# ndrwmlnk/critic-guided-segmentation-of-rewarding-objects-in-first-person-views

Measured on AMD Instinct MI355X. Metric: Hourglass+critic train images/sec, 64x64x3 batch=512, higher is better.
Workload: dtype f32

## Files before the change

critic-guided-segmentation-of-rewarding-objects-in-first-person-views_amd/_lib.py:

```python
import ctypes as C
import os

HERE = os.path.dirname(os.path.abspath(__file__))
LIB_PATH = os.environ.get("CGS_LIB_PATH") or os.path.join(HERE, "libcgs_hip.so")

OK, ERR_UNSUPPORTED, ERR_BADARG = 0, -1, -2
SRC_F32, SRC_U8, SRC_MIX = 0, 1, 2
ACT_NONE, ACT_RELU, ACT_LRELU, ACT_SIGMOID = 0, 1, 2, 3
H5_ENC1_FWD, H5_ENC1_BWD_DATA, H5_DEC0_FWD, H5_DEC0_BWD_SKIP, H5_DEC0_BWD_LOW = 1, 2, 3, 4, 5
H5_ENC1_BWD_DATA_POOLED = 6
H5_ENC2_FWD, H5_ENC2_BWD_DATA_POOLED, H5_DEC1_FWD, H5_DEC1_BWD_SKIP, H5_DEC1_BWD_LOW, H5_DEC1_FWD_F32B = 7, 8, 9, 10, 11, 12

vp = C.c_void_p
i32 = C.c_int32
i64 = C.c_int64
f32 = C.c_float


class Dropout(C.Structure):
    _fields_ = [("p", C.c_float), ("site", C.c_uint32), ("seed", C.c_uint64), ("step", C.c_void_p),
                ("base", C.c_uint32), ("reserved", C.c_uint32)]


class ConvDesc(C.Structure):
# ... 36 lines not shown
OBJ_TRACK_FIELDS, OBJ_TRACK_MAX_FRAMES = 8, 1 << 17
SALIENCY_SIDE, SALIENCY_MAX_T = 64, 1024
BOUNDARY_MAX_TOL, BOUNDARY_MAX_TOL_PX = 16, 128
FIT_SIDE, FIT_MAX_SIDE, FIT_RADIUS, FIT_MAP_F32, FIT_MAP_U8 = 64, 4096, 2, 0, 1
TEMPORAL_SIDE, TEMPORAL_MAX_RADIUS = 64, 8
OVERLAY_ONLY, OVERLAY_SIDE, OVERLAY_TRIPLE, OVERLAY_MAX_OUTLINE, OVERLAY_NONTEMPORAL = 1, 2, 3, 4, 1


class ReduceJob(C.Structure):
    _fields_ = [("slab", C.c_void_p), ("dst", C.c_void_p), ("nslab", i32), ("stride", i32), ("count", i32),
                ("accumulate", i32)]


SIGNATURES = {
    "cgs_conv3x3_fwd": (i32, [C.POINTER(ConvDesc), vp, vp, vp, vp, vp, vp, vp]),
    "cgs_conv3x3_bwd_data": (i32, [C.POINTER(ConvDesc), vp, vp, vp, vp, i32, vp, i32, vp, vp, vp]),
    "cgs_mask_infer_fwd": (i32, [i32, i32, vp, vp, vp, vp, vp, vp, vp, vp]),
    "cgs_mask_infer_fwd_packed": (i32, [i32, i32, vp, vp, vp, vp, vp, vp, vp, vp, vp]),
    "cgs_mask_infer_fwd_tile": (i32, [i32, i32, vp, vp, vp, vp, vp, vp, vp, vp]),
    "cgs_mask_infer_fwd_f16": (i32, [i32, i32, vp, vp, vp, vp, vp, vp, vp, vp]),
    "cgs_mask_infer_fwd_f16o": (i32, [i32, i32, vp, vp, vp, vp, vp, vp, vp, vp]),
    "cgs_f16_enc0_fwd": (i32, [i32, vp, vp, vp, vp, vp]),
    "cgs_f16_enc1_fwd": (i32, [i32, vp, vp, vp, vp, vp]),
    "cgs_f16_dec0_fwd": (i32, [i32, vp, vp, vp, vp, vp, vp]),
    "cgs_bf16_enc0_fwd": (i32, [i32, vp, i32, vp, vp, vp, vp, vp]),
    "cgs_bf16_mask0_fwd": (i32, [i32, vp, vp, vp, vp, vp, vp]),
    "cgs_bf16_mask2_fwd": (i32, [i32, vp, vp, vp, vp, vp]),
    "cgs_bf16_enc0_bwd_data": (i32, [i32, vp, vp, vp, vp]),
    "cgs_bf16_mask2_bwd_data": (i32, [i32, vp, vp, vp, vp, vp]),
    "cgs_bf16_enc0_bwd_data_pooled": (i32, [i32, vp, vp, vp, vp, vp, vp]),
    "cgs_bf16_enc0_bwd_mix": (i32, [i32, vp, vp, vp, vp, vp, vp, f32, f32, vp, vp]),
    "cgs_bf16_enc0_fwd_mix": (i32, [i32, vp, vp, vp, vp, vp, vp, vp, vp]),
    "cgs_bf16_hwgrad_pooled_mix": (i32, [i32, vp, vp, vp, vp, vp, vp, vp]),
    "cgs_bf16_mask0_bwd_data": (i32, [i32, vp, vp, vp, vp]),
    "cgs_bf16_h5conv": (i32, [i32, i32, vp, vp, vp, vp, vp, vp, vp]),
    "cgs_gen_enc0_fwd": (i32, [i32, i32, i32, vp, vp, vp, vp, vp, vp]),
    "cgs_gen_enc0_bwd_data": (i32, [i32, i32, vp, vp, vp, vp, vp]),
    "cgs_gen_enc0_bwd_weight_slabs": (i32, [i32, i32]),
    "cgs_gen_enc0_bwd_weight": (i32, [i32, i32, i32, vp, vp, vp, vp, vp]),
    "cgs_bn_rows": (i32, [i64, i32]),
    "cgs_bn_act_fwd": (i32, [i64, i32, vp, vp, vp, f32, i32, f32, i32, vp, vp, vp, vp, vp, f32, vp]),
    "cgs_bn_act_bwd": (i32, [i64, i32, vp, vp, vp, vp, i32, f32, i32, vp, vp, vp, vp, vp]),
    "cgs_bf16_hwgrad_slabs": (i32, [i32, i32, i32, i32, i32]),
    "cgs_bf16_hwgrad": (i32, [i32, i32, i32, i32, i32, i32, vp, vp, vp, vp, vp]),
    "cgs_bf16_hwgrad_pooled": (i32, [i32, i32, i32, i32, vp, vp, vp, vp, vp, vp]),
    "cgs_mask_train_fwd_partials": (i32, [i32]),
    "cgs_mask_train_fwd": (i32, [i32, i32, vp, vp, vp, vp, vp, vp, vp, vp, vp, vp]),
    "cgs_mask_train_fwd_packed": (i32, [i32, i32, vp, vp, vp, vp, vp, vp, vp, vp, vp, vp, vp]),
    "cgs_mask_head_bwd_slabs": (i32, [i32]),
    "cgs_mask_head_bwd": (i32, [i32, i32, vp, vp, vp, vp, vp, vp, vp, vp, vp, vp, vp]),
    "cgs_tail_enc_fwd": (i32, [i32, C.POINTER(TailEncWeights), vp, vp, vp, vp, vp, vp, vp, vp, vp, Dropout, Dropout, Dropout, vp]),
    "cgs_enc1_tail_fwd": (i32, [i32, C.POINTER(TailEncWeights), vp, vp, vp, vp, vp, vp, vp, vp, vp, vp, vp, vp, vp, Dropout, Dropout, Dropout, vp]),
    "cgs_critic_fwd_fused": (i32, [i32, C.POINTER(TailEncWeights), vp, i32] + [vp] * 16 + [Dropout, Dropout, Dropout, vp]),
    "cgs_tail_dec_fwd": (i32, [i32, C.POINTER(TailDecWeights), vp, vp, vp, vp, vp, vp, vp, vp]),
    "cgs_tail_enc_fwd_h16": (i32, [i32, C.POINTER(TailEncWeights), vp, vp, vp, vp, vp, vp, vp, vp, vp, vp]),
    "cgs_tail_dec_fwd_h16": (i32, [i32, C.POINTER(TailDecWeights), vp, vp, vp, vp, vp, vp, vp, vp]),
    "cgs_tail_infer_h16": (i32, [i32, C.POINTER(TailEncWeights), C.POINTER(TailDecWeights), vp, vp, vp, vp]),
    "cgs_f16_enc1_tail_infer": (i32, [i32, vp, vp, vp, C.POINTER(TailEncWeights), C.POINTER(TailDecWeights), vp, vp, vp]),
    "cgs_tail_dec_fwd_pack": (i32, [i32, C.POINTER(TailDecWeights), vp, vp, vp, vp, vp, vp, vp, vp, vp, vp]),
    "cgs_tail_enc_bwd_slabs": (i32, [i32]),
    "cgs_tail_enc_bwd": (i32, [i32, C.POINTER(TailEncWeights)] + [vp] * 10 + [f32, i32] + [vp] * 4 + [i32] + [vp] * 4 + [Dropout, Dropout, Dropout, vp]),
    "cgs_tail_enc_bwd_rider": (i32, [i32, C.POINTER(TailEncWeights)] + [vp] * 10 + [f32, i32] + [vp] * 4 + [i32] + [vp] * 4 + [Dropout, Dropout, Dropout, i32, vp, vp, vp, vp, i32, vp]),
    "cgs_tail_enc_bwd_enc1": (i32, [i32, C.POINTER(TailEncWeights)] + [vp] * 10 + [f32, i32] + [vp] * 4 + [i32] + [vp] * 4 + [Dropout, Dropout, Dropout, i32, vp, vp, vp, vp, i32, vp, vp, vp, i32, vp, vp, vp, i32, vp, vp, vp, vp]),
    "cgs_enc1_wgrad_rider_slabs": (i32, [i32]),
    "cgs_enc0_wgrad_u8_with_head_enc1": (i32, [i32, vp, vp, vp, vp, i32, vp, vp, vp, i32, i32, vp, vp, vp, i32, vp, vp, i32, vp, vp, vp, vp, i32, vp]),
    "cgs_enc0_bwd_mix_enc1": (i32, [i32, i32, vp, vp, vp, vp, vp, vp, vp, C.c_float, C.c_float, vp, vp, vp, vp, vp, vp, vp, vp]),
    "cgs_tail_head_wgrad_slabs": (i32, [i32]),
    "cgs_tail_head_wgrad": (i32, [i32, vp, vp, vp, i32, i32, vp, vp, vp, i32, vp, vp, vp]),
    "cgs_enc0_wgrad_u8_with_head": (i32, [i32, vp, vp, vp, vp, i32, vp, vp, vp, i32, i32, vp, vp, vp, i32, vp, vp, vp]),
    "cgs_reduce_adam": (i32, [vp, i32, i32, vp, vp, vp, vp, vp, f32, f32, f32, f32, vp, i32, vp, vp, vp, i32, f32, f32, f32, i32, i64, vp, vp]),
    "cgs_tail_dec_bwd_slabs": (i32, [i32]),
    "cgs_tail_dec_bwd": (i32, [i32, C.POINTER(TailDecWeights)] + [vp] * 14 + [vp]),
    "cgs_dec0_tail_dec_bwd": (i32, [i32, C.POINTER(TailDecWeights)] + [vp] * 17 + [vp]),
    "cgs_dec0_tail_dec_bwd_do3": (i32, [i32, C.POINTER(TailDecWeights)] + [vp] * 18 + [vp]),
    "cgs_dec3_wgrad_rider_slabs": (i32, [i32]),
    "cgs_enc0_wgrad_u8_with_head_riders": (i32, [i32, vp, vp, vp, vp, i32, vp, vp, vp, i32, i32, vp, vp, vp, i32, vp, vp, i32, vp, vp, vp, vp, i32, i32, vp, vp, vp, vp, vp]),
    "cgs_tail_dec_fwd_dec0": (i32, [i32, C.POINTER(TailDecWeights)] + [vp] * 13 + [vp]),
    "cgs_conv3x3_bwd_weight_slabs": (i32, [C.POINTER(ConvDesc)]),
    "cgs_conv3x3_bwd_weight": (i32, [C.POINTER(ConvDesc), vp, vp, vp, vp, vp, vp]),
    "cgs_conv3x3_bwd_both_slabs": (i32, [C.POINTER(ConvDesc)]),
    "cgs_conv3x3_bwd_both": (i32, [C.POINTER(ConvDesc), vp, vp, vp, vp, vp, vp, i32, vp, vp, vp, vp]),
    "cgs_reduce_slabs": (i32, [vp, i32, i32, vp, vp]),
    "cgs_head_fwd": (i32, [i32, vp, vp, vp, vp, vp, vp, vp, Dropout, Dropout, vp, vp, vp, vp, vp, vp, vp]),
    "cgs_enc0_bwd_mix_slabs": (i32, [i32]),
    "cgs_enc0_bwd_mix": (i32, [i32, i32, vp, vp, vp, vp, vp, vp, vp, C.c_float, C.c_float, vp, vp, vp, vp]),
    "cgs_head_bwd_slabs": (i32, [i32]),
    "cgs_head_bwd": (i32, [i32, vp, vp, vp, vp, vp, vp, vp, i32, vp, vp, vp, Dropout, Dropout, vp, vp, vp, vp, vp, vp]),
    "cgs_pointwise_fwd": (i32, [i32, i32, i32, vp, vp, vp, vp, vp]),
    "cgs_pointwise_bwd_slabs": (i32, [i32]),
    "cgs_pointwise_bwd": (i32, [i32, i32, i32, vp, vp, vp, vp, vp, vp]),
    "cgs_mix_fwd": (i32, [i32, i32, vp, vp, vp, i32, vp, vp, vp]),
    "cgs_mix_bwd": (i32, [i32, i32, vp, vp, vp, vp, i32, f32, f32, vp, vp]),
    "cgs_mix_bwd_weighted": (i32, [i32, i32, vp, vp, vp, vp, i32, f32, f32, vp, vp, vp]),
    "cgs_mix_fwd_partials": (i32, [i32, i32]),
    "cgs_phase2_losses": (i32, [i32, vp, vp, vp, i32, f32, f32, f32, i32, i64, vp, vp, vp]),
    "cgs_phase1_loss": (i32, [i32, vp, vp, i32, vp, vp, vp]),
    "cgs_adam_flat": (i32, [i64, vp, vp, vp, vp, vp, f32, f32, f32, f32, f32, vp]),
    "cgs_nchw_to_nhwc": (i32, [i32, i32, i32, vp, vp, vp]),
    "cgs_nhwc_to_nchw": (i32, [i32, i32, i32, vp, vp, vp]),
    "cgs_gen_conv_packed_floats": (i64, [i32, i32, i32]),
    "cgs_gen_conv_packed_floats_folded": (i64, [i32, i32, i32]),
    "cgs_gen_conv_packed_floats_up2": (i64, [i32, i32]),
    "cgs_gen_conv_pack_weights_up2": (i32, [i32, i32, i32, i32, vp, vp, vp]),
    "cgs_gen_conv3x3_bwd_data_up2": (i32, [i32, i32, i32, i32, vp, vp, vp, vp]),
    "cgs_gen_conv_pack_weights": (i32, [i32, i32, i32, i32, vp, vp, vp]),
    "cgs_gen_conv_pack_weights_window": (i32, [i32, i32, i32, i32, vp, vp, vp]),
    "cgs_gen_conv_pack_batch": (i32, [vp, i32, vp]),
    "cgs_gen_conv3x3_fwd": (i32, [i32, i32, i32, i32, i32, i32, i32, i32, f32, i32, vp, vp, vp, vp, vp, vp, vp]),
    "cgs_gen_conv3x3_fwd_folded": (i32, [i32, i32, i32, i32, i32, i32, i32, f32, vp, vp, vp, vp, vp, vp]),
    "cgs_gen_gemm": (i32, [i32, i32, i32, i32, f32, vp, vp, vp, vp, vp]),
    "cgs_gen_flip_weights": (i32, [i32, i32, vp, vp, vp]),
    "cgs_gen_conv3x3_bwd_data": (i32, [i32, i32, i32, i32, vp, vp, vp, vp, i32, vp, vp]),
    "cgs_gen_conv3x3_bwd_data_split": (i32, [i32, i32, i32, i32, i32, i32, vp, vp, vp, vp, vp]),
    "cgs_gen_conv3x3_bwd_weight_slabs": (i32, [i32, i32, i32, i32]),
    "cgs_gen_conv3x3_bwd_weight_folded_slabs": (i32, [i32, i32, i32, i32, i32]),
    "cgs_gen_conv3x3_bwd_weight_folded": (i32, [i32, i32, i32, i32, i32, i32, vp, vp, vp, vp, vp]),
    "cgs_gen_conv3x3_bwd_weight": (i32, [i32, i32, i32, i32, i32, i32, i32, vp, vp, vp, vp, vp, vp]),
    "cgs_gen_cat_split": (i32, [i32, i32, i32, i32, i32, vp, vp, vp, vp]),
    "cgs_gen_grad_fix": (i32, [i64, vp, vp, i32, f32, vp, i64, Dropout, vp]),
    "cgs_gen_dropout_fwd": (i32, [i64, vp, vp, Dropout, vp]),
    "cgs_gen_gemm_ex": (i32, [i32, i32, i32, vp, i64, i64, vp, i64, i64, vp, i32, f32, i32, vp, vp]),
    "cgs_gen_gemm_ex_splitk": (i32, [i32, i32, i32, vp, i64, i64, vp, i64, i64, i32, vp, vp]),
    "cgs_gen_u8_to_f32": (i32, [i64, vp, vp, vp]),
    "cgs_gen16_packed_weight_halves": (i64, [i32, i32, i32]),
    "cgs_gen16_pack_weights": (i32, [i32, i32, i32, vp, vp, vp]),
    "cgs_gen16_conv3x3_fwd": (i32, [i32, i32, i32, i32, i32, i32, i32, i32, f32, i32, i32, vp, vp, vp, vp, vp, vp]),
    "cgs_gen16_gemm": (i32, [i32, i32, i32, i32, f32, i32, i32, vp, vp, vp, vp, vp]),
    "cgs_genbf16_pack_weights": (i32, [i32, i32, i32, vp, vp, vp]),
    "cgs_genbf16_conv3x3_fwd": (i32, [i32, i32, i32, i32, i32, i32, i32, i32, f32, i32, i32, vp, vp, vp, vp, vp, vp]),
    "cgs_genbf16_gemm": (i32, [i32, i32, i32, i32, f32, i32, i32, vp, vp, vp, vp, vp]),
# ... 74 lines not shown
```

critic-guided-segmentation-of-rewarding-objects-in-first-person-views_amd/build.py:

```python
import os
import subprocess
import sys
from concurrent.futures import ThreadPoolExecutor

HERE = os.path.dirname(os.path.abspath(__file__))
REPO = os.path.dirname(HERE)
CSRC = os.path.join(HERE, "csrc")
LIB = os.path.join(HERE, "libcgs_hip.so")
SOURCES = ["conv_fwd.hip", "conv_wgrad.hip", "wgrad_dec0.hip", "conv_bwd_both.hip", "mconv.hip", "mask_head.hip", "mask_fwd.hip", "head.hip", "elementwise.hip", "tail.hip", "tail_infer.hip", "gen.hip", "gen4.hip", "gen_train.hip", "gen_f16.hip", "gen_bf16_train.hip", "hconv.hip", "hwgrad.hip", "bn.hip", "gen_enc0.hip", "crf.hip", "video.hip", "vis.hip", "sheet.hip", "metrics.hip", "objects.hip", "objects_match.hip", "objects_track.hip", "saliency.hip", "boundary.hip", "fit.hip", "temporal.hip", "overlay.hip"]
HEADERS = ["cgs_common.h", "head_wgrad.h", "conv_tile.h", "conv_body.h", "wgrad_body.h", "head_body.h", "tail_common.h", "tail4.h", "tail_h16.h", "gen_common.h", "gen4_common.h", "gen_wgrad_rows.h", "gen_wgrad_fold.h", "wgrad_dec0.h", "wgrad_sparse.h", os.path.join(REPO, "include", "cgs_hip.h")]
ARCH = "gfx950"
EXTRA_FLAGS = {"conv_fwd.hip": ["-fno-slp-vectorize"], "conv_bwd_both.hip": ["-fno-slp-vectorize"], "saliency.hip": ["-ffp-contract=off"]}


def _hipcc():
    for cand in (os.environ.get("HIPCC"), "/opt/rocm/bin/hipcc", "hipcc"):
        if cand and (os.path.isabs(cand) and os.path.exists(cand) or not os.path.isabs(cand)):
            return cand
    raise RuntimeError("hipcc not found")


def _stale():
    if not os.path.exists(LIB):
        return True
    t = os.path.getmtime(LIB)
    deps = [os.path.join(CSRC, s) for s in SOURCES] + [h if os.path.isabs(h) else os.path.join(CSRC, h) for h in HEADERS]
    return any(os.path.getmtime(d) > t for d in deps)


def build_library(force=False, verbose=True):
    if not force and not _stale():
        return LIB
    objdir = os.path.join(HERE, "build")
    os.makedirs(objdir, exist_ok=True)
    cc = _hipcc()
    flags = ["-O3", f"--offload-arch={ARCH}", "-std=c++17", "-fPIC", "-I", os.path.join(REPO, "include"), "-I", CSRC]

    def one(src):
        obj = os.path.join(objdir, src.replace(".hip", ".o"))
        extra = EXTRA_FLAGS.get(src, [])
        cmd = [cc] + flags + extra + ["-c", os.path.join(CSRC, src), "-o", obj]
        r = subprocess.run(cmd, capture_output=True, text=True)
        if r.returncode != 0:
            raise RuntimeError(f"hipcc failed for {src}:\n{r.stderr}")
        return obj

    with ThreadPoolExecutor(max_workers=6) as ex:
        objs = list(ex.map(one, SOURCES))
    r = subprocess.run([cc, "-shared", "-fPIC", f"--offload-arch={ARCH}", "-o", LIB] + objs, capture_output=True, text=True)
    if r.returncode != 0:
        raise RuntimeError(f"link failed:\n{r.stderr}")
    if verbose:
        print(f"built {LIB} ({os.path.getsize(LIB) // 1024} KiB) for {ARCH}", file=sys.stderr)
    return LIB


if __name__ == "__main__":
    build_library(force="--force" in sys.argv)
```

critic-guided-segmentation-of-rewarding-objects-in-first-person-views_amd/csrc/conv_body.h:

```cpp
#pragma once
#include "conv_tile.h"

#ifndef CGS_WHATIF_NO_POOL_EPI
#define CGS_WHATIF_NO_POOL_EPI 0
#endif
#ifndef CGS_POOL_EPI_MAX3
#define CGS_POOL_EPI_MAX3 2
#endif
#ifndef CGS_CONV_MFMA4
#define CGS_CONV_MFMA4 1
#endif

struct ConvParams {
    const void* src_a;
    const float* src_b;
    const uint32_t* amask_in;
    const float* w;
    const float* bias;
    float* out;
    float* out2;
    uint32_t* amask_out;
    const float* addend;
    const float* a_post;
    const float* w2;
// ... 521 lines not shown
    zero_halo_cols<G, PA>(ldsA, tid);
    auto pos = [&](int t, int& n0, int& row0) { const int b = bid0 + t; n0 = b / G::STRIPS; row0 = (b % G::STRIPS) * G::TH; };
    using RA = std::conditional_t<C::SRC == SRC_F32, FetchF32<G, PA>,
               std::conditional_t<C::SRC == SRC_U8C3, FetchU8<G>,
               std::conditional_t<C::SRC == SRC_MIXC3, FetchMix<G>,
               std::conditional_t<C::SRC == SRC_POOLEXP, FetchPool<G, PA, false>, FetchPool<G, PA, true>>>>>;
    RA ra;
    [[maybe_unused]] FetchBHalf<G, PB == 0 ? 1 : PB> rb;
    auto fetch = [&](int t) {
        int n0, row0;
        pos(t, n0, row0);
        if constexpr (C::SRC == SRC_F32) fetch_a_f32<G, PA>(ra, (const float4*)P.src_a, n0, row0, N, tid);
        else if constexpr (C::SRC == SRC_U8C3) fetch_a_u8c3<G>(ra, (const uint32_t*)P.src_a, n0, row0, N, tid);
        else if constexpr (C::SRC == SRC_MIXC3) fetch_a_mix<G>(ra, (const uint32_t*)P.mix_a, (const uint32_t*)P.mix_b, (const float4*)P.mix_z, P.mix_n_a, n0, row0, N, tid);
        else if constexpr (C::SRC == SRC_POOLEXP) fetch_poolexp<G, PA, false>(ra, (const float4*)P.src_a, P.amask_in, n0, 0, false, row0, N, tid);
        else fetch_poolexp<G, PA, true>(ra, (const float4*)P.src_a, P.amask_in, n0, P.mix_n_a, P.mix_inject != 0, row0, N, tid);
        if constexpr (PB > 0) fetch_b_half<G, PB>(rb, (const float4*)P.src_b, n0, row0, N, tid);
    };
    auto commit = [&](int t) {
        int n0, row0;
        pos(t, n0, row0);
        auto idx = [](int p, int img, int r, int x) { return ldsA_idx<G, PA>(p, img, r, x + 1); };
        if constexpr (C::SRC == SRC_F32) commit_a_f32<G, PA>(ra, ldsA, n0, row0, N, tid);
        else if constexpr (C::SRC == SRC_U8C3) commit_a_u8c3<G>(ra, ldsA, n0, row0, N, tid);
        else if constexpr (C::SRC == SRC_MIXC3) commit_a_mix<G>(ra, ldsA, P.mix_n_a, n0, row0, N, tid);
        else if constexpr (C::SRC == SRC_POOLEXP) commit_poolexp<G, PA, false>(ra, ldsA, n0, false, row0, N, tid, idx, L::DUMP);
        else commit_poolexp<G, PA, true>(ra, ldsA, n0, P.mix_inject != 0, row0, N, tid, idx, L::DUMP);
        if constexpr (PB > 0) commit_b_half<G, PB>(rb, ldsB, n0, row0, N, tid);
    };
    fetch(0);
#pragma unroll
    for (int t = 0; t < TPW; ++t) {
        commit(t);
        __syncthreads();
        if (t + 1 < TPW) fetch(t + 1);
        conv_compute<C, true>(P, bid0 + t, tid, smem, pool_lds);
        if (t + 1 < TPW) __syncthreads();
    }
}

template <class C>
__global__ void __launch_bounds__(C::THREADS * C::CW) conv3x3_pipe_kernel(ConvParams P) {
    extern __shared__ __attribute__((aligned(16))) float4 smem[];
    conv3x3_body_pipe<C>(P, blockIdx.x * tpw_of<C>::value, smem);
}

template <class C>
__global__ void __launch_bounds__(C::THREADS * C::CW) conv3x3_kernel(ConvParams P) {
    extern __shared__ __attribute__((aligned(16))) float4 smem[];
    conv3x3_body<C, false>(P, blockIdx.x, smem);
}

template <class C>
static size_t conv_lds_bytes() {
    using G = Geo<C::H, C::W, C::THREADS, C::CW>;
    constexpr int PA = (C::SRC == SRC_SCALAR) ? 1 : (C::CA + 3) / 4;
    constexpr int PB = C::CB / 4;
    size_t a = (C::SRC == SRC_SCALAR) ? (size_t)((G::IMGS * G::TRA * (G::W + 2) + 3) / 4) : (size_t)PA * G::IMGS * G::TRA * G::PWA;
    size_t b = PB == 0 ? 0 : (C::UPS == 2 ? (size_t)PB * G::IMGS * G::TRB * G::PWB : (size_t)PB * G::IMGS);
    size_t w = (size_t)(9 * C::WCI * C::WCO + 3) / 4;
    size_t dz = (C::SRC == SRC_DH) ? (size_t)((G::TRA + 2) * (G::W + 4) + 3) / 4 : 0;
    return (a + b + 1 + w + dz) * sizeof(float4);
}

#define CGS_FWD_CFG(NAME, HW, THR, SRC_, CA_, CB_, UPS_, CO_, EPI_, ACT_, OCB_, CW_)                   \
    struct NAME {                                                                                      \
        static constexpr int H = HW, W = HW, THREADS = THR, SRC = SRC_, CA = CA_, CB = CB_, UPS = UPS_; \
        static constexpr int WT = 0, WCI = CA_ + CB_, WCO = CO_, OC0 = 0, OC = CO_, OCB = OCB_, CW = CW_; \
        static constexpr int EPI = EPI_, ACT = ACT_, OUT_A = 0, POST_ACT = CGS_ACT_NONE;                \
        static constexpr bool DROP = (HW == 8 && CB_ == 0);   \
    };
#define CGS_DG_CFG(NAME, HW, THR, SRC_, DYC, LCI, LCO, UPS_, OC0_, OC_, OCB_, OUTA, PACT, CW_)         \
    struct NAME {                                                                                      \
        static constexpr int H = HW, W = HW, THREADS = THR, SRC = SRC_, CA = DYC, CB = 0, UPS = UPS_;   \
        static constexpr int WT = 1, WCI = LCI, WCO = LCO, OC0 = OC0_, OC = OC_, OCB = OCB_, CW = CW_;  \
        static constexpr int EPI = EPI_DGRAD, ACT = CGS_ACT_NONE, OUT_A = OUTA, POST_ACT = PACT;        \
        static constexpr bool DROP = (HW == 8 && SRC_ == SRC_POOLEXP);                                   \
    };

CGS_FWD_CFG(FEnc0U8, 64, 256, SRC_U8C3, 3, 0, 2, 8, EPI_POOL, CGS_ACT_RELU, 8, 1)
CGS_FWD_CFG(FEnc0F32, 64, 256, SRC_F32C3, 3, 0, 2, 8, EPI_POOL, CGS_ACT_RELU, 8, 1)
CGS_FWD_CFG(FEnc0Mix, 64, 256, SRC_MIXC3, 3, 0, 2, 8, EPI_POOL, CGS_ACT_RELU, 8, 1)
CGS_FWD_CFG(FEnc1, 32, 128, SRC_F32, 8, 0, 2, 8, EPI_POOL, CGS_ACT_RELU, 4, 2)
CGS_FWD_CFG(FEnc2, 16, 128, SRC_F32, 8, 0, 2, 8, EPI_POOL, CGS_ACT_RELU, 4, 2)
CGS_FWD_CFG(FEnc3, 8, 64, SRC_F32, 8, 0, 2, 16, EPI_POOL, CGS_ACT_RELU, 4, 4)
CGS_FWD_CFG(FDec3, 4, 64, SRC_F32, 16, 32, 4, 16, EPI_PLAIN, CGS_ACT_NONE, 4, 4)
CGS_FWD_CFG(FDec2, 8, 64, SRC_F32, 8, 16, 2, 8, EPI_PLAIN, CGS_ACT_NONE, 2, 4)
CGS_FWD_CFG(FDec1, 16, 64, SRC_F32, 8, 8, 2, 8, EPI_PLAIN, CGS_ACT_NONE, 4, 2)
CGS_FWD_CFG(FDec0, 32, 128, SRC_F32, 8, 8, 2, 8, EPI_PLAIN, CGS_ACT_NONE, 4, 2)
CGS_FWD_CFG(FMask0U8, 64, 128, SRC_U8C3, 3, 8, 2, 16, EPI_PLAIN, CGS_ACT_LRELU, 8, 2)
CGS_FWD_CFG(FMask0F32, 64, 128, SRC_F32C3, 3, 8, 2, 16, EPI_PLAIN, CGS_ACT_LRELU, 8, 2)
CGS_FWD_CFG(FMask2, 64, 256, SRC_F32, 16, 0, 2, 1, EPI_PLAIN, CGS_ACT_SIGMOID, 1, 1)

CGS_DG_CFG(DEnc0, 64, 256, SRC_POOLEXP, 8, 3, 8, 2, 0, 3, 3, 3, CGS_ACT_NONE, 1)
CGS_DG_CFG(DEnc1, 32, 128, SRC_POOLEXP, 8, 8, 8, 2, 0, 8, 4, 8, CGS_ACT_NONE, 2)
CGS_DG_CFG(DEnc2, 16, 128, SRC_POOLEXP, 8, 8, 8, 2, 0, 8, 4, 8, CGS_ACT_NONE, 2)
CGS_DG_CFG(DEnc3, 8, 64, SRC_POOLEXP, 16, 8, 16, 2, 0, 8, 4, 8, CGS_ACT_NONE, 2)
CGS_DG_CFG(DDec3, 4, 64, SRC_F32, 16, 48, 16, 4, 0, 48, 8, 16, CGS_ACT_NONE, 6)
CGS_DG_CFG(DDec2, 8, 64, SRC_F32, 8, 24, 8, 2, 0, 24, 8, 8, CGS_ACT_NONE, 3)
CGS_DG_CFG(DDec1, 16, 64, SRC_F32, 8, 16, 8, 2, 0, 16, 4, 8, CGS_ACT_NONE, 4)
CGS_DG_CFG(DDec0, 32, 128, SRC_F32, 8, 16, 8, 2, 0, 16, 8, 8, CGS_ACT_NONE, 2)
CGS_DG_CFG(DMask0, 64, 128, SRC_F32, 16, 11, 16, 2, 3, 8, 4, 3, CGS_ACT_NONE, 2)
CGS_DG_CFG(DMask2, 64, 128, SRC_SCALAR, 1, 16, 1, 2, 0, 16, 8, 16, CGS_ACT_LRELU, 2)
CGS_DG_CFG(DMaskHead, 64, 128, SRC_DH, 16, 11, 16, 2, 3, 8, 4, 3, CGS_ACT_NONE, 2)

#ifndef CGS_CONV_PIPE
#define CGS_CONV_PIPE 1
// ... 8 lines not shown
```

critic-guided-segmentation-of-rewarding-objects-in-first-person-views_amd/csrc/mask_fwd.hip:

```cpp
#include "conv_tile.h"

struct MaskFwdParams {
    const void* img; const float* o0;
    const float* w0; const float* b0; const float* w2; const float* b2;
    float* h; float* z; float* zpart;
    int n;
    unsigned long long* dbg;
    const float* w0_pack;
};

namespace {
using MG = Geo<64, 64, 256, 1>;
constexpr int kPSlots = 9;
constexpr int kWinPitch = 33;
unsigned long long* g_maskfwd_stamps = nullptr;
}

#define MF_STAMP(k) do { if (CGS_STAMP_PTR(P.dbg) && tid == 0) CGS_STAMP_PTR(P.dbg)[(size_t)blockIdx.x * 64 + (k)] = __builtin_amdgcn_s_memtime(); } while (0)
#ifdef CGS_DEBUG_STAMPS
extern "C" int dbg_maskfwd_stamps(unsigned long long* stamps) { g_maskfwd_stamps = stamps; return CGS_OK; }
#endif

template <int SRC>
__global__ void __launch_bounds__(256, SRC == SRC_U8C3 ? 2 : 1) mask_fwd_kernel(MaskFwdParams P) {
    if (CGS_KARG_PREFETCH) cgs_kernarg_prefetch<sizeof(MaskFwdParams)>();
    using G = MG;
    constexpr int A4 = (G::TRA * G::PWA + 1 + 3) / 4 * 4, B4 = 2 * G::TRB * G::PWB;
    static_assert(A4 + B4 <= 2048, "tiles fit the 32 KB staging area");
    __shared__ __attribute__((aligned(16))) float4 stage4[2048];
    float4* const ldsA = stage4;
    float4* const ldsB = stage4 + A4;
    __shared__ float win[kPSlots * 16 * kWinPitch];
    __shared__ float zred[8];
    const int tid = threadIdx.x, lane = tid & 63, wave = tid >> 6;
    const int n = blockIdx.x, N = P.n;
    const int lb = lane >> 2, li = lane & 3;
    MF_STAMP(0);

    constexpr int GW = G::W / 4, EA = G::TRA * GW, ITA = (EA + 255) / 256;
    constexpr int EB = G::TRB * G::PWB * 2, ITB = (EB + 255) / 256;
    uint32_t ra[ITA][(SRC == SRC_U8C3) ? 3 : 12];
    float4 rb[ITB];
    auto fetch = [&](int row0) {
#pragma unroll
        for (int it = 0; it < ITA; ++it) {
            int e = tid + 256 * it; e = e < EA ? e : EA - 1;
            const int g = e % GW, r = e / GW, y = row0 + r - 1;
            const bool in = y >= 0 && y < G::H;
            const int gi = in ? ((n * G::H + y) * G::W + g * 4) * 3 / 4 : 0;
            if constexpr (SRC == SRC_U8C3) {
                const uint32_t* src = (const uint32_t*)P.img;
                ra[it][0] = src[gi]; ra[it][1] = src[gi + 1]; ra[it][2] = src[gi + 2];
            } else {
                const float4* src = (const float4*)P.img;
#pragma unroll
                for (int k = 0; k < 3; ++k) {
                    const float4 v = src[gi + k];
                    ra[it][4 * k] = __float_as_uint(v.x); ra[it][4 * k + 1] = __float_as_uint(v.y);
                    ra[it][4 * k + 2] = __float_as_uint(v.z); ra[it][4 * k + 3] = __float_as_uint(v.w);
                }
            }
        }
        const int sy0 = row0 / 2;
#pragma unroll
        for (int it = 0; it < ITB; ++it) {
            int e = tid + 256 * it; e = e < EB ? e : EB - 1;
            const int p = e % 2, c = (e / 2) % G::PWB, r = e / (2 * G::PWB);
            const int sy = sy0 + r - 1, sx = c - 1;
            const bool in = sy >= 0 && sy < G::QH && sx >= 0 && sx < G::QW;
            rb[it] = ((const float4*)P.o0)[in ? ((n * G::QH + sy) * G::QW + sx) * 2 + p : 0];
        }
    };
    auto commit = [&](int row0) {
        const float sc = 1.f / 255.f;
#pragma unroll
        for (int it = 0; it < ITA; ++it) {
            int e = tid + 256 * it; e = e < EA ? e : EA - 1;
            const int g = e % GW, r = e / GW, y = row0 + r - 1;
            const bool in = y >= 0 && y < G::H;
            float4 p0, p1, p2, p3;
            if constexpr (SRC == SRC_U8C3) {
                const uint32_t d0 = ra[it][0], d1 = ra[it][1], d2 = ra[it][2];
                p0 = make_float4((d0 & 255) * sc, ((d0 >> 8) & 255) * sc, ((d0 >> 16) & 255) * sc, 0.f);
                p1 = make_float4((d0 >> 24) * sc, (d1 & 255) * sc, ((d1 >> 8) & 255) * sc, 0.f);
                p2 = make_float4(((d1 >> 16) & 255) * sc, (d1 >> 24) * sc, (d2 & 255) * sc, 0.f);
                p3 = make_float4(((d2 >> 8) & 255) * sc, ((d2 >> 16) & 255) * sc, (d2 >> 24) * sc, 0.f);
            } else {
                auto f = [&](int k) { return __uint_as_float(ra[it][k]); };
                p0 = make_float4(f(0), f(1), f(2), 0.f); p1 = make_float4(f(3), f(4), f(5), 0.f);
                p2 = make_float4(f(6), f(7), f(8), 0.f); p3 = make_float4(f(9), f(10), f(11), 0.f);
            }
            const int base = r * G::PWA;
            ldsA[base + G::pc(g * 4 + 1)] = in ? p0 : f4zero();
            ldsA[base + G::pc(g * 4 + 2)] = in ? p1 : f4zero();
            ldsA[base + G::pc(g * 4 + 3)] = in ? p2 : f4zero();
            ldsA[base + G::pc(g * 4 + 4)] = in ? p3 : f4zero();
        }
        zero_halo_cols<G, 1>(ldsA, tid);
        const int sy0 = row0 / 2;
#pragma unroll
        for (int it = 0; it < ITB; ++it) {
            int e = tid + 256 * it; e = e < EB ? e : EB - 1;
            const int p = e % 2, c = (e / 2) % G::PWB, r = e / (2 * G::PWB);
            const int sy = sy0 + r - 1, sx = c - 1;
            const bool in = sy >= 0 && sy < G::QH && sx >= 0 && sx < G::QW;
            ldsB[(p * G::TRB + r) * G::PWB + c] = in ? rb[it] : f4zero();
        }
    };
    fetch(0);
    float wimg[4][2];
    float wups[4][4][2];
    if (P.w0_pack) {
        const float* wp = P.w0_pack + lane;
#pragma unroll
        for (int g = 0; g < 4; ++g) {
#pragma unroll
            for (int k = 0; k < 2; ++k) wimg[g][k] = wp[(g * 2 + k) * 64];
#pragma unroll
            for (int pos = 0; pos < 4; ++pos)
#pragma unroll
                for (int ry = 0; ry < 2; ++ry) wups[pos][g][ry] = wp[(8 + (pos * 4 + g) * 2 + ry) * 64];
        }
    } else {
    float* wst = (float*)ldsA;
    for (int e = tid; e < 9 * 11 * 16; e += 256) wst[e] = P.w0[e];
    __syncthreads();
#pragma unroll
    for (int g = 0; g < 4; ++g) {
#pragma unroll
        for (int k = 0; k < 2; ++k) {
            const int step = 16 * k + lb;
            wimg[g][k] = step < 27 ? wst[((step / 3) * 11 + step % 3) * 16 + 4 * g + li] : 0.f;
        }
#pragma unroll
        for (int pos = 0; pos < 4; ++pos) {
            const int oy = pos >> 1, ox = pos & 1;
#pragma unroll
            for (int ry = 0; ry < 2; ++ry) {
                const int rx = lb >> 3, ci = lb & 7;
                const int ky0 = (oy == 0) ? (ry == 0 ? 0 : 1) : (ry == 0 ? 0 : 2), ky1 = (oy == 0) ? (ry == 0 ? 0 : 2) : (ry == 0 ? 1 : 2);
                const int kx0 = (ox == 0) ? (rx == 0 ? 0 : 1) : (rx == 0 ? 0 : 2), kx1 = (ox == 0) ? (rx == 0 ? 0 : 2) : (rx == 0 ? 1 : 2);
                auto wv = [&](int ky, int kx) { return wst[((ky * 3 + kx) * 11 + 3 + ci) * 16 + 4 * g + li]; };
                const float w00 = wv(ky0, kx0), w01 = wv(ky0, kx1), w10 = wv(ky1, kx0), w11 = wv(ky1, kx1);
                const bool my = ky1 > ky0, mx = kx1 > kx0;
                float s = w00;
                s += mx ? w01 : 0.f;
                s += my ? w10 : 0.f;
                s += (mx && my) ? w11 : 0.f;
                wups[pos][g][ry] = s;
            }
            __builtin_amdgcn_sched_barrier(0);
        }
    }
    }
    float w2r[3];
#pragma unroll
    for (int g = 0; g < 3; ++g) w2r[g] = (4 * g + li < 9) ? P.w2[(4 * g + li) * 16 + lb] : 0.f;
    const cgs_cptr b0c = cgs_to_const(P.b0);
    const float b2v = cgs_to_const(P.b2)[0];
    __syncthreads();

    MF_STAMP(1);
    const QuadPos q0 = quad_pos<G>(tid, 0);
    const int qy_l = q0.qy_l, qx = q0.qx;
    int pcx[4];
#pragma unroll
    for (int dx = 0; dx < 4; ++dx) pcx[dx] = G::pc(2 * qx + dx);
    float zs1 = 0.f, zs2 = 0.f;

#pragma unroll 1
    for (int strip = 0; strip < G::STRIPS; ++strip) {
        const int row0 = strip * G::TH;
        QuadPos q = q0;
        q.n = n; q.row0 = row0;
        MF_STAMP(2 + 10 * strip);
        commit(row0);
        __syncthreads();
        MF_STAMP(3 + 10 * strip);
        if (strip + 1 < G::STRIPS) fetch(row0 + G::TH);

        frag4 acc[4][4];
#pragma unroll
        for (int i = 0; i < 4; ++i)
#pragma unroll
            for (int g = 0; g < 4; ++g) acc[i][g] = frag4{b0c[4 * g], b0c[4 * g + 1], b0c[4 * g + 2], b0c[4 * g + 3]};
        {
            float4 pt[4][4];
            read_patch_a<G>(pt, ldsA, 0, q, pcx);
            mfma_plane<4, 3, 3, 0, 2>(acc, pt, wimg);
        }
        MF_STAMP(4 + 10 * strip);
        static_for<2>([&](auto PL) {
            constexpr int p = decltype(PL)::value;
            float4 s[3][3];
            const int base = (p * G::TRB + qy_l) * G::PWB + qx;
#pragma unroll
            for (int j = 0; j < 3; ++j)
#pragma unroll
                for (int i = 0; i < 3; ++i) s[j][i] = ldsB[base + j * G::PWB + i];
            static_for<16>([&](auto T) {
                constexpr int t = decltype(T)::value, ry = t >> 3, rx = (t >> 2) & 1, c = t & 3;
                constexpr int abid = rx * 8 + 4 * p + c;
#pragma unroll
                for (int pos = 0; pos < 4; ++pos) {
                    const float x = f4get(s[(pos >> 1) + ry][(pos & 1) + rx], c);
#pragma unroll
                    for (int g = 0; g < 4; ++g)
                        acc[pos][g] = __builtin_amdgcn_mfma_f32_4x4x1f32(wups[pos][g][ry], x, acc[pos][g], 4, abid, 0);
                }
            });
        });

        float hv[4][16];
        const int y0 = row0 + 2 * qy_l, x0 = 2 * qx;
#pragma unroll
        for (int pos = 0; pos < 4; ++pos)
#pragma unroll
            for (int c = 0; c < 16; ++c) { const float v = acc[pos][c >> 2][c & 3]; hv[pos][c] = fmaxf(v, 0.01f * v); }
        MF_STAMP(5 + 10 * strip);
        __syncthreads();
        MF_STAMP(6 + 10 * strip);
        if (P.h) {
            float4* sw4 = stage4 + wave * 512;
            const int pp = lane;
#pragma unroll
            for (int oy = 0; oy < 2; ++oy) {
#pragma unroll
                for (int j = 0; j < 8; ++j) {
                    const int pos = oy * 2 + (j >> 2), c0 = 4 * (j & 3);
                    sw4[pp * 8 + (j ^ (pp & 7))] = make_float4(hv[pos][c0], hv[pos][c0 + 1], hv[pos][c0 + 2], hv[pos][c0 + 3]);
                }
#pragma unroll
                for (int k = 0; k < 8; ++k) {
                    const int i = lane + 64 * k, rp = i >> 3, j = i & 7;
                    const float4 v = sw4[rp * 8 + (j ^ (rp & 7))];
                    const int y = row0 + 2 * (2 * wave + (k >> 2)) + oy;
                    ((float4*)P.h)[((size_t)(n * 64 + y) * 64) * 4 + (rp & 31) * 8 + j] = v;
                }
            }
        }
        MF_STAMP(7 + 10 * strip);
        frag4 c2[4][3];
#pragma unroll
        for (int i = 0; i < 4; ++i)
#pragma unroll
            for (int g = 0; g < 3; ++g) c2[i][g] = frag4{0.f, 0.f, 0.f, 0.f};
        static_for<16>([&](auto CH) {
            constexpr int ch = decltype(CH)::value;
#pragma unroll
            for (int pos = 0; pos < 4; ++pos)
#pragma unroll
                for (int g = 0; g < 3; ++g)
                    c2[pos][g] = __builtin_amdgcn_mfma_f32_4x4x1f32(w2r[g], hv[pos][ch], c2[pos][g], 4, ch, 0);
        });
        MF_STAMP(8 + 10 * strip);
        float sw[4][4];
#pragma unroll
        for (int wy = -1; wy <= 2; ++wy)
#pragma unroll
            for (int wx = -1; wx <= 2; ++wx) {
                float s = 0.f;
#pragma unroll
                for (int oy = 0; oy < 2; ++oy)
#pragma unroll
                    for (int ox = 0; ox < 2; ++ox) {
                        const int ky = oy - wy + 1, kx = ox - wx + 1;
                        if (ky >= 0 && ky <= 2 && kx >= 0 && kx <= 2) {
                            const int tap = ky * 3 + kx;
                            s += c2[oy * 2 + ox][tap >> 2][tap & 3];
                        }
                    }
                sw[wy + 1][wx + 1] = s;
            }
        float* wown = win + (qy_l + 1) * 16 * kWinPitch + qx;
#pragma unroll
        for (int e = 0; e < 16; ++e) wown[e * kWinPitch] = sw[e >> 2][e & 3];
        __syncthreads();
        MF_STAMP(9 + 10 * strip);
        const bool has_top = strip > 0 || qy_l > 0;
        const float* wtop = win + qy_l * 16 * kWinPitch + qx;
        float zz[3][2];
#pragma unroll
        for (int wy = -1; wy <= 1; ++wy) {
#pragma unroll
            for (int wx = 0; wx <= 1; ++wx) {
                const bool has_side = wx == 0 ? qx > 0 : qx < 31;
                const int side = has_side ? (wx == 0 ? -1 : 1) : 0;
                const int wxs = wx == 0 ? 2 : -1;
                float s = sw[wy + 1][wx + 1];
                const float a = wown[((wy + 1) * 4 + wxs + 1) * kWinPitch + side];
                s += has_side ? a : 0.f;
                if (wy <= 0) {
                    const float b = wtop[((wy + 3) * 4 + wx + 1) * kWinPitch];
                    const float c = wtop[((wy + 3) * 4 + wxs + 1) * kWinPitch + side];
                    s += has_top ? b : 0.f;
                    s += (has_top && has_side) ? c : 0.f;
                }
                zz[wy + 1][wx] = act_fwd<CGS_ACT_SIGMOID>(s + b2v);
            }
        }
        const bool last_row = strip == G::STRIPS - 1 && qy_l == 7;
#pragma unroll
        for (int wy = -1; wy <= 1; ++wy) {
            const int y = y0 + wy;
            if (wy == 1 ? last_row : y >= 0) {
                *(float2*)(P.z + (size_t)(n * 64 + y) * 64 + x0) = make_float2(zz[wy + 1][0], zz[wy + 1][1]);
                zs1 += fabsf(zz[wy + 1][0]) + fabsf(zz[wy + 1][1]);
                zs2 += zz[wy + 1][0] * zz[wy + 1][0] + zz[wy + 1][1] * zz[wy + 1][1];
            }
        }
        MF_STAMP(10 + 10 * strip);
        __syncthreads();
        MF_STAMP(11 + 10 * strip);
        if (qy_l == 7) {
#pragma unroll
            for (int e = 0; e < 16; ++e) win[e * kWinPitch + qx] = sw[e >> 2][e & 3];
        }
    }
    if (P.zpart) {
        zs1 = wave_sum(zs1); zs2 = wave_sum(zs2);
        if (lane == 0) { zred[2 * wave] = zs1; zred[2 * wave + 1] = zs2; }
        __syncthreads();
        if (tid == 0) {
            P.zpart[2 * n] = (zred[0] + zred[2]) + (zred[4] + zred[6]);
            P.zpart[2 * n + 1] = (zred[1] + zred[3]) + (zred[5] + zred[7]);
        }
    }
}

int mask_train_partials(int n) { return n; }
int mask_train_launch(int n, int img_kind, const void* img, const float* o0, const float* w0, const float* b0, const float* w2,
                      const float* b2, float* h, float* z, float* zpart, const float* w0_pack, hipStream_t st) {
    if (n <= 0) return CGS_OK;
    MaskFwdParams P{img, o0, w0, b0, w2, b2, h, z, zpart, n, g_maskfwd_stamps, w0_pack};
    if (img_kind == CGS_SRC_U8) hipLaunchKernelGGL(mask_fwd_kernel<SRC_U8C3>, dim3(n), dim3(256), 0, st, P);
    else hipLaunchKernelGGL(mask_fwd_kernel<SRC_F32C3>, dim3(n), dim3(256), 0, st, P);
    CGS_HIP_CHECK_LAUNCH();
    return CGS_OK;
}
```

critic-guided-segmentation-of-rewarding-objects-in-first-person-views_amd/csrc/tail.hip:

```cpp
#include "tail4.h"
#include "tail_h16.h"
#include "head_wgrad.h"
#include "wgrad_dec0.h"
#include "conv_body.h"
#include "wgrad_sparse.h"

namespace {

using T16x8 = Tile<16, 16, 8>;
using T8x8 = Tile<8, 8, 8>;
using T8x16 = Tile<8, 8, 16>;
using T16x16 = Tile<16, 16, 16>;
using T8x24 = Tile<8, 8, 24>;
using T4x48 = Tile<4, 4, 48>;
using T4x16 = Tile<4, 4, 20>;

__device__ __forceinline__ float4 nib_select4(const float4& v, uint32_t nib16, uint32_t pos) {
    float4 r;
    r.x = ((nib16 & 15u) == pos) ? v.x : 0.f;
    r.y = (((nib16 >> 4) & 15u) == pos) ? v.y : 0.f;
    r.z = (((nib16 >> 8) & 15u) == pos) ? v.z : 0.f;
    r.w = (((nib16 >> 12) & 15u) == pos) ? v.w : 0.f;
    return r;
}

__device__ __forceinline__ float drop1(const DropCtx& dc, uint32_t i) {
    return dc.on ? f4get(drop_mult4(dc, i >> 2), i & 3) : 1.f;
}

int tail_blocks(int n, int cap) { return n < cap ? n : cap; }
int tail_fwd_cap() { return 1024; }
#ifndef CGS_TAIL_DEC_FWD_CAP
#define CGS_TAIL_DEC_FWD_CAP 768
#endif
int tail_dec_fwd_cap() { return CGS_TAIL_DEC_FWD_CAP; }
int tail_bwd_cap() { return 512; }
#ifndef CGS_TAIL_ENC_BWD_CAP
#define CGS_TAIL_ENC_BWD_CAP 768
#endif
int tail_enc_bwd_cap() { return CGS_TAIL_ENC_BWD_CAP; }

unsigned long long* g_tail_stamps = nullptr;

}

#ifdef CGS_DEBUG_STAMPS
extern "C" int dbg_tail_stamps(unsigned long long* stamps) { g_tail_stamps = stamps; return CGS_OK; }
#endif
#define TAIL_STAMP(k)                                                                                     \
    do {                                                                                                  \
        if (CGS_STAMP_PTR(P.dbg) && tid == 0 && img == (int)blockIdx.x) CGS_STAMP_PTR(P.dbg)[(size_t)blockIdx.x * 16 + (k)] = __builtin_amdgcn_s_memtime(); \
    } while (0)

#ifndef CGS_TAIL_STAGGER
#define CGS_TAIL_STAGGER 0
#endif
#ifndef CGS_STAGGER_ENC_FWD
#define CGS_STAGGER_ENC_FWD CGS_TAIL_STAGGER
#endif
#ifndef CGS_STAGGER_DEC_FWD
#define CGS_STAGGER_DEC_FWD CGS_TAIL_STAGGER
#endif
#ifndef CGS_STAGGER_DEC_BWD
#define CGS_STAGGER_DEC_BWD CGS_TAIL_STAGGER
#endif
struct TailEncFwdParams {
    cgs_tail_enc_weights w;
    const float* e1;
    float* e2; uint32_t* am2; float* e3; uint32_t* am3; float* e4; float* h1; float* pred; float* o4;
    cgs_dropout drop_e2, drop_e3, drop_h1;
    int n;
    int nblocks;
    unsigned long long* dbg;
};

using X1P = TileP<16, 16, 8, 8, 148>;
using X2P = TileP<8, 8, 8, 8, 84>;

template <bool FUSED, int ENC0 = 0, bool H16 = false>
__global__ void __launch_bounds__(256) __attribute__((amdgpu_waves_per_eu(H16 ? 3 : 4, H16 ? 3 : 4))) tail_enc_fwd_kernel(TailEncFwdParams P, ConvParams PC, ConvParams PC0) {
    static_assert(!H16 || (!FUSED && ENC0 == 0), "fp16 operands: the stand-alone inference form");
    extern __shared__ __attribute__((aligned(16))) float4 conv_smem[];
    __shared__ __attribute__((aligned(16))) float x1[X1P::FLOATS];
    __shared__ __attribute__((aligned(16))) float x2[X2P::FLOATS];
    __shared__ __attribute__((aligned(16))) float xs[256];
    __shared__ __attribute__((aligned(16))) float red[8][32];
    __shared__ float es[32], hs[32];
    if (CGS_KARG_PREFETCH) cgs_kernarg_prefetch<sizeof(TailEncFwdParams) + 2 * sizeof(ConvParams)>();
    const int tid = threadIdx.x, lane = tid & 63, wave = tid >> 6;
    if (CGS_STAMP_PTR(P.dbg) && tid == 0) CGS_STAMP_PTR(P.dbg)[(size_t)blockIdx.x * 16] = __builtin_amdgcn_s_memtime();
    const int o = tid & 31, kg = tid >> 5;
    int img = blockIdx.x;
    float4 pe[2] = {f4zero(), f4zero()};
    if constexpr (!FUSED) {
        if (img < P.n) { pe[0] = ((const float4*)P.e1)[(size_t)img * 512 + tid]; pe[1] = ((const float4*)P.e1)[(size_t)img * 512 + tid + 256]; }
    }
#if CGS_DROPCTX3
    DropCtx d2, d3, dh;
    drop_ctx3(P.drop_e2, P.drop_e3, P.drop_h1, P.w.b6, d2, d3, dh);
#else
    const DropCtx d2 = drop_ctx(P.drop_e2, P.w.b6), d3 = drop_ctx(P.drop_e3, P.w.b6), dh = drop_ctx(P.drop_h1, P.w.b6);
#endif

    tilep_zero<X1P>(x1, tid);
    tilep_zero<X2P>(x2, tid);
    if constexpr (FUSED) {
        cgs_stagger<8, CGS_STAGGER_ENC_FWD>();
        if constexpr (ENC0 == 1) { conv3x3_body_pipe<FEnc0U8P>(PC0, 4 * (int)blockIdx.x, conv_smem); __syncthreads(); }
        if constexpr (ENC0 == 2) { conv3x3_body_pipe<FEnc0MixP>(PC0, 4 * (int)blockIdx.x, conv_smem); __syncthreads(); }
        conv3x3_body_pipe<FEnc1P>(PC, 2 * (int)blockIdx.x, conv_smem, PoolLds{x1, X1P::PITCH, X1P::PS});
    }
    if (CGS_STAMP_PTR(P.dbg) && tid == 0) CGS_STAMP_PTR(P.dbg)[(size_t)blockIdx.x * 16 + 12] = __builtin_amdgcn_s_memtime();
    [[maybe_unused]] float wr6[H16 ? 1 : 2][5], wr10[1][5];
    [[maybe_unused]] th4_t w6h[5], w10h[5];
    [[maybe_unused]] int off6[5], off10[5];
    if constexpr (H16) {
        const int l15w = lane & 15;
        h16_fill_w<8, 5, 1>(w6h, lane, 0, l15w < 8, [&](int tap, int c) { return P.w.w6[(tap * 8 + c) * 8 + (l15w & 7)]; });
        h16_fill_w<8, 5, 1>(w10h, lane, 0, true, [&](int tap, int c) { return P.w.w10[(tap * 8 + c) * 16 + l15w]; });
        h16_fill_off<X1P, 8, 5, 1>(off6, lane, 0);
        h16_fill_off<X2P, 8, 5, 1>(off10, lane, 0);
    } else {
        fill_wreg<2, 5, 72>(wr6, lane, [&](int step, int co) { return P.w.w6[step * 8 + co]; });
        fill_wreg<1, 5, 72>(wr10, lane, [&](int step, int co) { return P.w.w10[step * 16 + 4 * wave + co]; });
    }
    if (CGS_STAMP_PTR(P.dbg) && tid == 0) CGS_STAMP_PTR(P.dbg)[(size_t)blockIdx.x * 16 + 13] = __builtin_amdgcn_s_memtime();
    float w1r[4], wpr[4];
#pragma unroll
    for (int j = 0; j < 4; ++j) {
        w1r[j] = P.w.wl1[(kg * 4 + j) * 32 + o];
        wpr[j] = P.o4 ? P.w.wpw[(kg * 4 + j) * 32 + o] : 0.f;
    }
    const cgs_cptr b6c = cgs_to_const(P.w.b6), b10c = cgs_to_const(P.w.b10);
    const float b14 = P.w.b14[o], bl1 = P.w.bl1[o], wl2 = P.w.wl2[o], bl2 = P.w.bl2[0], bpw = P.o4 ? P.w.bpw[o] : 0.f;
    const PxPos pa = px16(wave, lane), pb = px8(lane);
    if (CGS_STAMP_PTR(P.dbg) && tid == 0) CGS_STAMP_PTR(P.dbg)[(size_t)blockIdx.x * 16 + 14] = __builtin_amdgcn_s_memtime();
    __syncthreads();

    for (; img < P.n; img += P.nblocks) {
        TAIL_STAMP(1);
        if constexpr (!FUSED) {
#pragma unroll
// ... 152 lines not shown
                for (int m = 16; m >= 1; m >>= 1) t += __shfl_xor(t, m, 64);
                if (o == 0) P.pred[img] = 1.f / (1.f + expf(-(t + bl2)));
            }
        }
        __syncthreads();
        TAIL_STAMP(11);
    }
    if (CGS_STAMP_PTR(P.dbg) && tid == 0) CGS_STAMP_PTR(P.dbg)[(size_t)blockIdx.x * 16 + 15] = __builtin_amdgcn_s_memtime();
}

extern "C" int cgs_tail_enc_fwd(int32_t n, const cgs_tail_enc_weights* w, const float* e1, float* e2, uint32_t* am2, float* e3,
                                uint32_t* am3, float* e4, float* h1, float* pred, float* o4, cgs_dropout drop_e2,
                                cgs_dropout drop_e3, cgs_dropout drop_h1, cgs_stream_t stream) {
    if (n < 0 || !w || !e1 || !e2 || !am2 || !e3 || !am3 || !e4 || !h1 || !pred) return CGS_ERR_BADARG;
    if (!w->w6 || !w->b6 || !w->w10 || !w->b10 || !w->w14 || !w->b14 || !w->wl1 || !w->bl1 || !w->wl2 || !w->bl2) return CGS_ERR_BADARG;
    if (o4 && (!w->wpw || !w->bpw)) return CGS_ERR_BADARG;
    if (n == 0) return CGS_OK;
    TailEncFwdParams P{*w, e1, e2, am2, e3, am3, e4, h1, pred, o4, drop_e2, drop_e3, drop_h1, n, tail_blocks(n, tail_fwd_cap()), g_tail_stamps ? g_tail_stamps + 0 * 2048 * 16 : nullptr};
    const int blocks = P.nblocks;
    hipLaunchKernelGGL((tail_enc_fwd_kernel<false, 0>), dim3(blocks), dim3(256), 0, (hipStream_t)stream, P, ConvParams{}, ConvParams{});
    CGS_HIP_CHECK_LAUNCH();
    return CGS_OK;
}

extern "C" int cgs_tail_enc_fwd_h16(int32_t n, const cgs_tail_enc_weights* w, const float* e1, float* e2, uint32_t* am2, float* e3,
                                    uint32_t* am3, float* e4, float* h1, float* pred, float* o4, cgs_stream_t stream) {
    if (n < 0 || !w || !e1 || !e2 || !am2 || !e3 || !am3 || !e4 || !h1 || !pred) return CGS_ERR_BADARG;
    if (!w->w6 || !w->b6 || !w->w10 || !w->b10 || !w->w14 || !w->b14 || !w->wl1 || !w->bl1 || !w->wl2 || !w->bl2) return CGS_ERR_BADARG;
    if (o4 && (!w->wpw || !w->bpw)) return CGS_ERR_BADARG;
    if (n == 0) return CGS_OK;
    const cgs_dropout nd{};
    TailEncFwdParams P{*w, e1, e2, am2, e3, am3, e4, h1, pred, o4, nd, nd, nd, n, tail_blocks(n, 768), nullptr};
    hipLaunchKernelGGL((tail_enc_fwd_kernel<false, 0, true>), dim3(P.nblocks), dim3(256), 0, (hipStream_t)stream, P, ConvParams{}, ConvParams{});
    CGS_HIP_CHECK_LAUNCH();
    return CGS_OK;
}

extern "C" int cgs_enc1_tail_fwd(int32_t n, const cgs_tail_enc_weights* w, const float* e0, const float* w3, const float* b3, float* e1,
                                 uint32_t* am1, float* e2, uint32_t* am2, float* e3, uint32_t* am3, float* e4, float* h1, float* pred, float* o4,
                                 cgs_dropout drop_e2, cgs_dropout drop_e3, cgs_dropout drop_h1, cgs_stream_t stream) {
    if (n < 0 || !w || !e0 || !w3 || !b3 || !e1 || !am1 || !e2 || !am2 || !e3 || !am3 || !e4 || !h1 || !pred) return CGS_ERR_BADARG;
    if (!w->w6 || !w->b6 || !w->w10 || !w->b10 || !w->w14 || !w->b14 || !w->wl1 || !w->bl1 || !w->wl2 || !w->bl2) return CGS_ERR_BADARG;
    if (o4 && (!w->wpw || !w->bpw)) return CGS_ERR_BADARG;
    if (n == 0) return CGS_OK;
    TailEncFwdParams P{*w, e1, e2, am2, e3, am3, e4, h1, pred, o4, drop_e2, drop_e3, drop_h1, n, n, g_tail_stamps ? g_tail_stamps + 0 * 2048 * 16 : nullptr};
    ConvParams PC{};
    PC.src_a = e0; PC.w = w3; PC.bias = b3; PC.out = e1; PC.amask_out = am1; PC.n = n;
    const size_t lds = conv_lds_bytes<FEnc1P>();
    hipLaunchKernelGGL((tail_enc_fwd_kernel<true, 0>), dim3(n), dim3(256), lds, (hipStream_t)stream, P, PC, ConvParams{});
    CGS_HIP_CHECK_LAUNCH();
    return CGS_OK;
}

extern "C" int cgs_critic_fwd_fused(int32_t n, const cgs_tail_enc_weights* w, const void* x, int32_t x_is_mix, const float* w0, const float* b0,
                                    float* e0, uint32_t* am0, const float* w3, const float* b3, float* e1, uint32_t* am1, float* e2, uint32_t* am2,
                                    float* e3, uint32_t* am3, float* e4, float* h1, float* pred, float* o4, cgs_dropout drop_e2,
                                    cgs_dropout drop_e3, cgs_dropout drop_h1, cgs_stream_t stream) {
    if (n < 0 || !w || !x || !w0 || !b0 || !e0 || !am0 || !w3 || !b3 || !e1 || !am1 || !e2 || !am2 || !e3 || !am3 || !e4 || !h1 || !pred) return CGS_ERR_BADARG;
    if (!w->w6 || !w->b6 || !w->w10 || !w->b10 || !w->w14 || !w->b14 || !w->wl1 || !w->bl1 || !w->wl2 || !w->bl2) return CGS_ERR_BADARG;
    if (o4 && (!w->wpw || !w->bpw)) return CGS_ERR_BADARG;
    if (n == 0) return CGS_OK;
    TailEncFwdParams P{*w, e1, e2, am2, e3, am3, e4, h1, pred, o4, drop_e2, drop_e3, drop_h1, n, n, g_tail_stamps ? g_tail_stamps + 0 * 2048 * 16 : nullptr};
    ConvParams PC{}, PC0{};
    PC.src_a = e0; PC.w = w3; PC.bias = b3; PC.out = e1; PC.amask_out = am1; PC.n = n;
    PC0.w = w0; PC0.bias = b0; PC0.out = e0; PC0.amask_out = am0; PC0.n = n;
    size_t lds = conv_lds_bytes<FEnc1P>();
    if (x_is_mix) {
        const cgs_mix_src* m = (const cgs_mix_src*)x;
        if (!m->a || !m->b || !m->z || m->n_a <= 0 || n > 2 * m->n_a) return CGS_ERR_BADARG;
        PC0.mix_a = m->a; PC0.mix_b = m->b; PC0.mix_z = m->z; PC0.mix_n_a = m->n_a;
        if (conv_lds_bytes<FEnc0MixP>() > lds) lds = conv_lds_bytes<FEnc0MixP>();
        hipLaunchKernelGGL((tail_enc_fwd_kernel<true, 2>), dim3(n), dim3(256), lds, (hipStream_t)stream, P, PC, PC0);
    } else {
        PC0.src_a = x;
        if (conv_lds_bytes<FEnc0U8P>() > lds) lds = conv_lds_bytes<FEnc0U8P>();
        hipLaunchKernelGGL((tail_enc_fwd_kernel<true, 1>), dim3(n), dim3(256), lds, (hipStream_t)stream, P, PC, PC0);
    }
    CGS_HIP_CHECK_LAUNCH();
    return CGS_OK;
}

struct TailDecFwdParams {
    cgs_tail_dec_weights w;
    const float* e1; const float* e2; const float* e3; const float* o4;
    float* o3; float* o2; float* o1;
    int n;
    int nblocks;
    unsigned long long* dbg;
    const float* m0_w; float* m0_pack;
};

__device__ __forceinline__ void mask0_pack_weights(const float* __restrict__ w0, float* __restrict__ pack, int lane) {
    const int lb = lane >> 2, li = lane & 3;
#pragma unroll
    for (int g = 0; g < 4; ++g) {
#pragma unroll
        for (int k = 0; k < 2; ++k) {
            const int step = 16 * k + lb;
            pack[(g * 2 + k) * 64 + lane] = step < 27 ? w0[((step / 3) * 11 + step % 3) * 16 + 4 * g + li] : 0.f;
        }
#pragma unroll
        for (int pos = 0; pos < 4; ++pos) {
            const int oy = pos >> 1, ox = pos & 1;
#pragma unroll
            for (int ry = 0; ry < 2; ++ry) {
                const int rx = lb >> 3, ci = lb & 7;
                const int ky0 = (oy == 0) ? (ry == 0 ? 0 : 1) : (ry == 0 ? 0 : 2), ky1 = (oy == 0) ? (ry == 0 ? 0 : 2) : (ry == 0 ? 1 : 2);
                const int kx0 = (ox == 0) ? (rx == 0 ? 0 : 1) : (rx == 0 ? 0 : 2), kx1 = (ox == 0) ? (rx == 0 ? 0 : 2) : (rx == 0 ? 1 : 2);
                auto wv = [&](int ky, int kx) { return w0[((ky * 3 + kx) * 11 + 3 + ci) * 16 + 4 * g + li]; };
                const float w00 = wv(ky0, kx0), w01 = wv(ky0, kx1), w10 = wv(ky1, kx0), w11 = wv(ky1, kx1);
                const bool my = ky1 > ky0, mx = kx1 > kx0;
                float sum = w00;
                sum += mx ? w01 : 0.f;
                sum += my ? w10 : 0.f;
                sum += (mx && my) ? w11 : 0.f;
                pack[(8 + (pos * 4 + g) * 2 + ry) * 64 + lane] = sum;
            }
        }
    }
}

using T1F = TileP<16, 16, 16, 16, 292>;

template <bool FUSED, bool H16 = false>
__global__ void __launch_bounds__(256) __attribute__((amdgpu_waves_per_eu(3, 3))) tail_dec_fwd_kernel(TailDecFwdParams P, ConvParams PC) {
    static_assert(!H16 || !FUSED, "fp16 operands: the stand-alone inference form");
    if (CGS_KARG_PREFETCH) cgs_kernarg_prefetch<sizeof(TailDecFwdParams) + sizeof(ConvParams)>();
    extern __shared__ __attribute__((aligned(16))) float4 dec_conv_smem[];
    __shared__ __attribute__((aligned(16))) float t1[T1F::FLOATS];
    __shared__ __attribute__((aligned(16))) float t2[T8x24::FLOATS];
    __shared__ __attribute__((aligned(16))) float t3[T4x48::FLOATS];
    __shared__ __attribute__((aligned(16))) float w2s[14 * 64 * 2];
    static_assert(14 * 64 * 2 >= 216 * 8, "either form fits");
    __shared__ float part[4][16][16];
    const int tid = threadIdx.x, lane = tid & 63, wave = tid >> 6;
    if ((int)blockIdx.x == P.nblocks) {
        if (wave == 0) mask0_pack_weights(P.m0_w, P.m0_pack, lane);
        return;
    }
    if constexpr (FUSED) cgs_stagger<8, CGS_STAGGER_DEC_FWD>();
    if (CGS_STAMP_PTR(P.dbg) && tid == 0) CGS_STAMP_PTR(P.dbg)[(size_t)blockIdx.x * 16] = __builtin_amdgcn_s_memtime();
    const int l15 = lane & 15, kq = lane >> 4;
    int img = blockIdx.x;
    float4 pe1a = f4zero(), pe1b = f4zero(), pe2 = f4zero(), pe3 = f4zero(), po4 = f4zero();
#define DEC_FWD_FETCH(im)                                                                                         \
    do {                                                                                                          \
        pe1a = ((const float4*)P.e1)[(size_t)(im) * 512 + tid]; pe1b = ((const float4*)P.e1)[(size_t)(im) * 512 + tid + 256]; \
        pe2 = ((const float4*)P.e2)[(size_t)(im) * 128 + (tid & 127)];                                            \
        pe3 = ((const float4*)P.e3)[(size_t)(im) * 64 + (tid & 63)];                                              \
        po4 = ((const float4*)P.o4)[(size_t)(im) * 8 + (tid & 7)];                                                \
    } while (0)
    if (img < P.n) DEC_FWD_FETCH(img);

    const float4 w2a = ((const float4*)P.w.w2)[tid], w2b = ((const float4*)P.w.w2)[tid + 256 < 216 * 8 / 4 ? tid + 256 : 0];
    [[maybe_unused]] float wr1[2][H16 ? 1 : 9];
    [[maybe_unused]] th4_t w3h[7], w1h[9];
    [[maybe_unused]] int off2[14];
    [[maybe_unused]] th4_t w2t[H16 ? 4 : 1];
    if constexpr (H16) {
        h16_fill_w<48, 7, 4>(w3h, lane, wave, true, [&](int tap, int c) { return P.w.w3[(tap * 48 + c) * 16 + l15]; });
        h16_fill_w<16, 9, 1>(w1h, lane, 0, l15 < 8, [&](int tap, int c) { return P.w.w1[(tap * 16 + c) * 8 + (l15 & 7)]; });
#pragma unroll
        for (int r = 0; r < 4; ++r) {
            const int e = tid + 256 * r, i = e >> 6, ln = e & 63;
            w2t[r] = h16_w1<24>(i, ln >> 4, (ln & 15) < 8, [&](int tap, int c) { return P.w.w2[(tap * 24 + c) * 8 + (ln & 7)]; });
        }
        h16_fill_off<T8x24, 24, 14, 1>(off2, lane, 0);
    } else {
        fill_wreg<2, 9, 144>(wr1, lane, [&](int step, int co) { return P.w.w1[step * 8 + co]; });
    }
    const float b2 = P.w.b2[l15 & 7];
    [[maybe_unused]] const float b1v = P.w.b1[l15 & 7];
    __builtin_amdgcn_sched_barrier(0);
    tilep_zero<T1F>(t1, tid);
    tile_zero<T8x24>(t2, tid);
    tile_zero<T4x48>(t3, tid);
    if constexpr (H16) {
#pragma unroll
        for (int r = 0; r < 4; ++r)
            if (tid + 256 * r < 14 * 64) ((th4_t*)w2s)[tid + 256 * r] = w2t[r];
    } else {
        ((float4*)w2s)[tid] = w2a;
        if (tid + 256 < 216 * 8 / 4) ((float4*)w2s)[tid + 256] = w2b;
    }
    const PxPos pa = px16(wave, lane);
    const cgs_cptr b1c = cgs_to_const(P.w.b1);
    __syncthreads();

    for (; img < P.n; img += P.nblocks) {
        TAIL_STAMP(1);
        int lz = 0;
        asm volatile("" : "+v"(lz));
        const int lane_i = lane + lz;
// ... 53 lines not shown
        auto epi2 = [&](int q, const frag4 (&acc)[1]) {
            if (l15 < 8) {
                const int qy = q >> 2, qx = q & 3;
#pragma unroll
                for (int j = 0; j < 4; ++j) {
                    const int y = 2 * qy + (j >> 1), x = 2 * qx + (j & 1);
                    const float v = acc[0][j] + b2;
                    P.o2[((size_t)img * 64 + y * 8 + x) * 8 + l15] = v;
#pragma unroll
                    for (int d = 0; d < 4; ++d) t1[T1F::at(2 * y + (d >> 1), 2 * x + (d & 1)) + 8 + l15] = v;
                }
            }
        };
        if constexpr (H16) {
            int y, x;
            h16_tile_px<8>(wave, l15, y, x);
            const frag4 acc[1] = {h16_conv_f<14>(t2 + T8x24::at(y - 1, x - 1), [&](int n) { return off2[n]; },
                                               [&](int n) { return ((const th4_t*)w2s)[n * 64 + lane_i]; }, frag4{0.f, 0.f, 0.f, 0.f})};
            epi2(4 * wave + kq, acc);
        } else {
            conv_tiles<T8x24, 0, 24, 1>(t2, [&](int tap, int c, int) { return w2s[(tap * 24 + c) * 8 + (l15 & 7)]; }, epi2, wave, lane_i);
        }
        __syncthreads();
        TAIL_STAMP(5);
        if constexpr (H16) {
#pragma unroll 1
            for (int u = 0; u < 4; ++u) {
                const int t = wave + 4 * u;
                int y, x;
                h16_tile_px<16>(t, l15, y, x);
                const frag4 acc = h16_conv_f<9>(t1 + T1F::at(y - 1, x - 1) + 4 * kq, [&](int n) { return h16_off<T1F, 16>(n, 0); },
                                                 [&](int n) { return w1h[n]; }, frag4{b1v, b1v, b1v, b1v});
                if (l15 < 8) {
                    const int q = 4 * t + kq, qy = q >> 3, qx = q & 7;
#pragma unroll
                    for (int j = 0; j < 4; ++j)
                        P.o1[((size_t)img * 256 + (2 * qy + (j >> 1)) * 16 + 2 * qx + (j & 1)) * 8 + l15] = acc[j];
                }
            }
        } else {
            frag4 a[2] = {frag4{b1c[0], b1c[1], b1c[2], b1c[3]}, frag4{b1c[4], b1c[5], b1c[6], b1c[7]}};
            conv_px<T1F, 0, 16, 16, 0, 2, 9, false, true>(a, t1, pa.y, pa.x, wr1);
            float4* dst = (float4*)(P.o1 + ((size_t)img * 256 + pa.y * 16 + pa.x) * 8);
            dst[0] = make_float4(a[0][0], a[0][1], a[0][2], a[0][3]);
            dst[1] = make_float4(a[1][0], a[1][1], a[1][2], a[1][3]);
        }
        __syncthreads();
        TAIL_STAMP(6);
    }
    if constexpr (FUSED) {
        conv3x3_body_pipe<FDec0P>(PC, 2 * (int)blockIdx.x, dec_conv_smem);
    }
    if (CGS_STAMP_PTR(P.dbg) && tid == 0) CGS_STAMP_PTR(P.dbg)[(size_t)blockIdx.x * 16 + 15] = __builtin_amdgcn_s_memtime();
}

extern "C" int cgs_tail_dec_fwd_pack(int32_t n, const cgs_tail_dec_weights* w, const float* e1, const float* e2, const float* e3,
                                     const float* o4, float* o3, float* o2, float* o1, const float* w_m0, float* m0_pack,
                                     cgs_stream_t stream) {
    if (n < 0 || !w || !e1 || !e2 || !e3 || !o4 || !o3 || !o2 || !o1 || (m0_pack && !w_m0)) return CGS_ERR_BADARG;
    if (!w->w3 || !w->b3 || !w->w2 || !w->b2 || !w->w1 || !w->b1) return CGS_ERR_BADARG;
    if (n == 0) return CGS_OK;
    TailDecFwdParams P{*w, e1, e2, e3, o4, o3, o2, o1, n, tail_blocks(n, tail_dec_fwd_cap()), g_tail_stamps ? g_tail_stamps + 1 * 2048 * 16 : nullptr,
                       w_m0, m0_pack};
    const int blocks = tail_blocks(n, tail_dec_fwd_cap());
    hipLaunchKernelGGL(tail_dec_fwd_kernel<false>, dim3(blocks + (m0_pack ? 1 : 0)), dim3(256), 0, (hipStream_t)stream, P, ConvParams{});
    CGS_HIP_CHECK_LAUNCH();
    return CGS_OK;
}

extern "C" int cgs_tail_dec_fwd_dec0(int32_t n, const cgs_tail_dec_weights* w, const float* e0, const float* e1, const float* e2, const float* e3,
                                     const float* o4, float* o3, float* o2, float* o1, const float* w0, const float* b0, float* o0,
                                     const float* w_m0, float* m0_pack, cgs_stream_t stream) {
    if (n < 0 || !w || !e0 || !e1 || !e2 || !e3 || !o4 || !o3 || !o2 || !o1 || !w0 || !b0 || !o0 || (m0_pack && !w_m0)) return CGS_ERR_BADARG;
    if (!w->w3 || !w->b3 || !w->w2 || !w->b2 || !w->w1 || !w->b1) return CGS_ERR_BADARG;
    if (n == 0) return CGS_OK;
    if (n > tail_fwd_cap()) return CGS_ERR_UNSUPPORTED;
    TailDecFwdParams P{*w, e1, e2, e3, o4, o3, o2, o1, n, n, g_tail_stamps ? g_tail_stamps + 1 * 2048 * 16 : nullptr, w_m0, m0_pack};
    ConvParams PC{};
    PC.src_a = e0; PC.src_b = o1; PC.w = w0; PC.bias = b0; PC.out = o0; PC.n = n;
    const size_t lds = conv_lds_bytes<FDec0P>();
    static hipError_t attr = hipFuncSetAttribute(reinterpret_cast<const void*>(&tail_dec_fwd_kernel<true>),
                                                 hipFuncAttributeMaxDynamicSharedMemorySize, (int)(conv_lds_bytes<FDec0P>()));
    if (attr != hipSuccess) return (int)attr;
    hipLaunchKernelGGL(tail_dec_fwd_kernel<true>, dim3(n + (m0_pack ? 1 : 0)), dim3(256), lds, (hipStream_t)stream, P, PC);
    CGS_HIP_CHECK_LAUNCH();
    return CGS_OK;
}

extern "C" int cgs_tail_dec_fwd_h16(int32_t n, const cgs_tail_dec_weights* w, const float* e1, const float* e2, const float* e3,
                                    const float* o4, float* o3, float* o2, float* o1, cgs_stream_t stream) {
    if (n < 0 || !w || !e1 || !e2 || !e3 || !o4 || !o3 || !o2 || !o1) return CGS_ERR_BADARG;
    if (!w->w3 || !w->b3 || !w->w2 || !w->b2 || !w->w1 || !w->b1) return CGS_ERR_BADARG;
    if (n == 0) return CGS_OK;
    const int blocks = tail_blocks(n, tail_dec_fwd_cap());
    TailDecFwdParams P{*w, e1, e2, e3, o4, o3, o2, o1, n, blocks, nullptr, nullptr, nullptr};
    hipLaunchKernelGGL((tail_dec_fwd_kernel<false, true>), dim3(blocks), dim3(256), 0, (hipStream_t)stream, P, ConvParams{});
    CGS_HIP_CHECK_LAUNCH();
    return CGS_OK;
}

extern "C" int cgs_tail_dec_fwd(int32_t n, const cgs_tail_dec_weights* w, const float* e1, const float* e2, const float* e3,
                                const float* o4, float* o3, float* o2, float* o1, cgs_stream_t stream) {
    return cgs_tail_dec_fwd_pack(n, w, e1, e2, e3, o4, o3, o2, o1, nullptr, nullptr, stream);
}

static constexpr int kTailSlab10 = 1168, kTailSlab6 = 584;
using DY2P = TileP<16, 16, 8, 8, 148>;
using DY3P = TileP<8, 8, 16, 16, 164>;
static constexpr int kTailEncBwdTileFloats = T16x8::FLOATS + T8x8::FLOATS + DY2P::FLOATS + DY3P::FLOATS;
static constexpr int kTailEncBwdOwnFloats = ((kTailEncBwdTileFloats + 3) & ~3) + 72 * 8 + 72 * 16 + 256 + 512 + 512 + 2048 + 64 + 32;
static constexpr int kTailEncBwdLdsFloats = kTailEncBwdOwnFloats > kWD0LdsFloats ? kTailEncBwdOwnFloats : kWD0LdsFloats;

struct TailEncBwdParams {
    cgs_tail_enc_weights w;
    const float* e1; const float* e2; const uint32_t* am2; const float* e3; const uint32_t* am3;
    const float* e4; const float* h1; const float* pred; const float* dpred;
    const float* target; float loss_scale; int bce;
    const float* dE1; const float* dE2; const float* dE3; const float* d_o4; int n_add;
    float* de1;
    float* hvec; float* slab10; float* slab6;
    cgs_dropout drop_e2, drop_e3, drop_h1;
    int n;
    int nblocks;
    unsigned long long* dbg;
    WDec0Params rider;
};

#ifndef CGS_ENC1_STAGGER
#define CGS_ENC1_STAGGER 64
#endif
#ifndef CGS_DROPCTX_SPLIT
#define CGS_DROPCTX_SPLIT 0
#endif
#ifndef CGS_ENC1_WGRAD_STAGES
#define CGS_ENC1_WGRAD_STAGES 1
#endif
template <int MODE>
// ... 609 lines not shown
```

critic-guided-segmentation-of-rewarding-objects-in-first-person-views_amd/engine.py:

```python
import os
import ctypes as C
from typing import Dict, Optional

import torch

from . import _lib
from . import hourglass as hg
from . import parallel
from .spec import ENC_LAYERS, critic_layout, masker_layout

_P = hg._p
_S = hg._stream


def _align4(x):
    return (x + 3) // 4 * 4


GATHER_ONE_LAUNCH = os.environ.get("CGS_GATHER_ONE_LAUNCH", "1") != "0"
PHASE1_FUSED_TAIL = os.environ.get("CGS_PHASE1_FUSED_TAIL", "1") != "0"
F16_TAILS = os.environ.get("CGS_F16_TAILS", "fused")


class HourglassEngine:
# ... 108 lines not shown
        return {k: t[a:b] for k, t in self.cbuf.items()}

    def _slab_views(self, tag: str, n_first: int, n_second: int):
        lib = _lib.load()
        out1, out2 = {}, {}
        nd = _lib.Dropout(0.0, 0, 0, None, 0, 0)
        tail = hg.TAIL_BWD
        specs = [] if tail else [("slab_head", lambda n, first: lib.cgs_head_bwd_slabs(n), hg.HEAD_SLAB)]
        for i, (key, hw, ca, cb, co, ups, act, pool, site) in enumerate(ENC_LAYERS):
            def f(n, first, i=i, hw=hw, ca=ca, cb=cb, co=co, ups=ups, act=act, pool=pool):
                d = hg.conv_desc(n, hw, ca, cb, co, False, ups, act, pool, nd)
                in_tail1 = hg.enc1_tail_bwd_fused(n) and hg.ENC1_WGRAD_IN_TAIL and 1 in hg.BOTH_ENC
                if tail and (i >= 2 or (i == 1 and in_tail1) or (i == 0 and in_tail1 and tag == "p2" and hg.enc0_in_tail(first, not first, None))):
                    return lib.cgs_tail_enc_bwd_slabs(n)
                if i in hg.BOTH_ENC and (i > 0 or first):
                    return lib.cgs_conv3x3_bwd_both_slabs(C.byref(d))
                return lib.cgs_conv3x3_bwd_weight_slabs(C.byref(d))
            specs.append((f"slab_enc{i}", f, 9 * ca * co + co))
        for name, fn, cnt in specs:
            a, b = (fn(n_first, True) if n_first else 0), (fn(n_second, False) if n_second else 0)
            big = torch.zeros((a + b, cnt), device=self.dev)
            self._ws.setdefault("slabs_" + tag, []).append(big)
            out1[name], out2[name] = big[:a], big[a:]
        return out1, out2

    def _opt_range(self):
        return (0, self.total) if self.live else (self.off_m, self.total - self.off_m)

    def _adam(self, tag="p2"):
        if self.fused_tail and not self.dp and tag == "p2":
            return
        lo, cnt = self._opt_range()
        _lib.call("cgs_adam_flat", cnt, C.c_void_p(self.flat.data_ptr() + 4 * lo), C.c_void_p(self.grad.data_ptr() + 4 * lo),
                  C.c_void_p(self.m.data_ptr() + 4 * lo), C.c_void_p(self.v.data_ptr() + 4 * lo), _P(self.step_t),
                  self.lr, self.b1, self.b2, self.eps, 1.0 / self.world, _S())

    def _allreduce(self):
        if self.dp:
            lo, cnt = self._opt_range()
            parallel.allreduce_sum_(self.grad[lo:lo + cnt], self.pg)

    def _phase2_fwd_bwd(self):
        n = self.n
        nmix = 2 * n if self.inject else n
        drop = self.drop
        A = self.ab[n:]
        B = self.ab[:n]
        if getattr(self, "_o4_full", None) is None:
            self._o4_full = torch.empty((2 * n, 32), device=self.dev, dtype=torch.float32)
            self.mbuf["o4"] = self._o4_full[n:]
        fm_ptr = self.fm.data_ptr()
        pw = (C.c_void_p(fm_ptr + 4 * self.lm.off("dec_model.4.weight")), C.c_void_p(fm_ptr + 4 * self.lm.off("dec_model.4.bias")),
              self._o4_full)
        hg.critic_forward(self.fc, self.lc, self.ab, 2 * n, drop.shifted(0), out=self._cview(0, 2 * n),
                          pw=None if self.separate else pw)
        sa = self._cview(n, 2 * n)
        if self.separate:
            pws = (pw[0], pw[1], self.mbuf["o4"])
            hg.critic_forward(self.fs, self.lc, A, n, drop.shifted(4 * n), out=self.sbuf, pw=pws)
            embeds = [self.sbuf[f"e{i}"] for i in range(5)]
        else:
            embeds = [sa[f"e{i}"] for i in range(5)]
        hg.masker_forward(self.fm, self.lm, A, embeds, n, out=self.mbuf, o4_done=True,
                          zpart=self.zsum if hg.ENC0_MIX_FUSED else None)
        if hg.ENC0_MIX_FUSED:
            mixsrc = hg.MixInput(A, B, self.mbuf["Z"])
            hg.critic_forward(self.fc, self.lc, mixsrc, nmix, drop.shifted(2 * n), out=self._cview(2 * n, 2 * n + nmix))
        else:
            mixsrc = self.mixed[:nmix]
            _lib.call("cgs_mix_fwd", n, 4096, _P(A), _P(B), _P(self.mbuf["Z"]), int(self.inject), _P(self.mixed), _P(self.zsum), _S())
            hg.critic_forward(self.fc, self.lc, mixsrc, nmix, drop.shifted(2 * n), out=self._cview(2 * n, 2 * n + nmix))
        flags = (1 if self.live else 0) | (2 if self.inject else 0) | (4 if self.bce else 0) | (0 if self.staticnorm else 8)
        ft = self.fused_tail
        if not ft:
            _lib.call("cgs_phase2_losses", n, _P(self.cbuf["pred"]), _P(self.y), _P(self.zsum), self.nzpart, self.lfak, self.L1, self.L2,
                      flags, n * 4096, _P(self.losses), _P(self.dpred), _S())
        loss_mix = (self.cbuf["pred"][:nmix], 1.0 / n, False) if ft else None
        loss_a = (self.y, self.lfak / n, self.bce) if ft else None
        plan = self._plans.get("p2")
        first = plan is None
        if first:
            plan = hg.SlabPlan()
            self._sl_mix, self._sl_a = self._slab_views("p2", nmix, n if self.live else 0)
            self._ws["cb_mix"].update(self._sl_mix)
            self._ws["cb_a"].update(self._sl_a)
        pc = plan if first else hg.SlabPlan()
        sink_c = [] if hg.TAIL_BWD else None
        nz = float(n * 4096)
        if hg.ENC0_MIX_FUSED:
            hg.critic_backward(self.fc, self.lc, mixsrc, nmix, self._cview(2 * n, 2 * n + nmix),
                               None if ft else self.dpred[2 * n:2 * n + nmix], pc, drop.shifted(2 * n), dx=None, dx_from=0,
                               ws=self._ws["cb_mix"], side=self.side, need_wgrad=self.live, loss=loss_mix, head_sink=sink_c,
                               mix_bwd=(A, B, self.mbuf["Z"], self.inject, self.L1 / nz, self.L2 / nz, self.dzpre,
                                        None if self.staticnorm else sa["pred"]))
        else:
            hg.critic_backward(self.fc, self.lc, self.mixed[:nmix], nmix, self._cview(2 * n, 2 * n + nmix),
                               self.dpred[2 * n:2 * n + nmix], pc, drop.shifted(2 * n), dx=self.dmixed[:nmix], dx_from=0,
                               ws=self._ws["cb_mix"], side=self.side, need_wgrad=self.live)
            _lib.call("cgs_mix_bwd", n, 4096, _P(A), _P(B), _P(self.mbuf["Z"]), _P(self.dmixed), int(self.inject),
                      self.L1 / nz, self.L2 / nz, _P(self.dzpre), _S())
        pm = hg.SlabPlan()
        defer = [] if (self.live and not self.separate and hg.TAIL_BWD) else None
        d_emb = hg.masker_backward(self.fm, self.lm, A, embeds, n, self.mbuf, self.dzpre, pm, ws=self._ws["mb"], side=self.side,
                                   pw_in_head=self.live or self.separate, defer_dec0=defer)
        rider = next((d for d in (defer or []) if not isinstance(d, dict)), None)
        dec3 = next((d["dec3"] for d in (defer or []) if isinstance(d, dict)), None)
        ps = hg.SlabPlan()
        if self.separate:
            d_o4, d_emb[4] = d_emb[4], None
            hg.critic_backward(self.fs, self.lc, A, n, self.sbuf, None if ft else self._zero_dpred, ps, drop.shifted(4 * n), d_embeds=d_emb,
                               n_add=n, ws=self._ws["cb_sep"], side=self.side,
                               pw_bwd=(d_o4, pw[0], pm, self.lm.off("dec_model.4.weight")))
            if self.live:
                hg.critic_backward(self.fc, self.lc, A, n, sa, None if ft else self.dpred[n:2 * n], pc, drop.shifted(n),
                                   ws=self._ws["cb_a"], side=self.side, loss=loss_a, head_sink=sink_c)
        elif self.live:
            d_o4, d_emb[4] = d_emb[4], None
# ... 296 lines not shown
```

critic-guided-segmentation-of-rewarding-objects-in-first-person-views_amd/hourglass.py:

```python
import os
import ctypes as C
from typing import Dict, List, Optional

import torch

from . import _lib
from .spec import (DEC_LAYERS, DROP_SITE_E2, DROP_SITE_E3, DROP_SITE_H1, ENC_LAYERS, Layout)

_ACT = {"none": _lib.ACT_NONE, "relu": _lib.ACT_RELU, "lrelu": _lib.ACT_LRELU, "sigmoid": _lib.ACT_SIGMOID}
HEAD_SLAB = 8192 + 32 + 1024 + 32 + 32 + 1
BWD_BOTH = True
MASK_INFER_FUSED = True
ENC0_MIX_FUSED = True
MASK_HEAD_FUSED = True
MASK_TRAIN_FUSED = True
MASK_TRAIN_FUSED_MIN_N = int(os.environ.get("CGS_MASK_TRAIN_FUSED_MIN_N", "160"))
TAIL_FWD = True
TAIL_BWD = True
ENC1_TAIL_FUSED = True
CRITIC_FWD_FUSED = True
DEC0_TAIL_BWD_FUSED = True
DEC_TAIL_DEC0_FUSED = True
ENC1_TAIL_BWD_FUSED = os.environ.get("CGS_ENC1_TAIL_BWD_FUSED", "1") != "0"
ENC1_TAIL_BWD_FUSED_MIN_N = int(os.environ.get("CGS_ENC1_TAIL_BWD_FUSED_MIN_N", "224"))


def mask_train_fused(n: int) -> bool:
    return MASK_TRAIN_FUSED and n >= MASK_TRAIN_FUSED_MIN_N


def enc1_tail_bwd_fused(n: int) -> bool:
    return ENC1_TAIL_BWD_FUSED and n >= ENC1_TAIL_BWD_FUSED_MIN_N
ENC1_WGRAD_IN_TAIL = os.environ.get("CGS_ENC1_WGRAD_IN_TAIL", "1") != "0"
ENC0_WGRAD_IN_TAIL = os.environ.get("CGS_ENC0_WGRAD_IN_TAIL", "")
DEC0_WGRAD_RIDER = True
DEC0_RIDERS = 256
DEC3_WGRAD_RIDER = os.environ.get("CGS_DEC3_WGRAD_RIDER", "0") != "0"
_both = "c3,c2,c1,c0,d3,d2,d1"
BOTH_ENC = {int(t[1]) for t in _both.split(",") if t.startswith("c")} if BWD_BOTH else set()
BOTH_DEC = {t for t in _both.split(",") if t[0] in "dm"} if BWD_BOTH else set()
_DEC_TAG = {0: "d3", 1: "d2", 2: "d1", 3: "d0", 4: "m0", 5: "m2"}
PW_SLAB = 32 * 32 + 32


def _stream():
    return C.c_void_p(torch.cuda.current_stream().cuda_stream)


def _p(t: Optional[torch.Tensor]):
    return C.c_void_p(t.data_ptr()) if t is not None else C.c_void_p(0)


def _chk(t: torch.Tensor, dtype, what: str):
    if not t.is_cuda:
        raise _lib.CgsError(f"{what}: HIP kernels need a device tensor (got {t.device}); there is no CPU fallback")
    if t.dtype != dtype or not t.is_contiguous():
        raise _lib.CgsError(f"{what}: expected contiguous {dtype}, got {t.dtype} contiguous={t.is_contiguous()}")
    return t


def _chk_img(x, n: int, what: str):
    shp = tuple(x.shape) if not isinstance(x, MixInput) else (x.n_a, 64, 64, 3)
    if len(shp) != 4 or shp[1:] != (64, 64, 3) or (not isinstance(x, MixInput) and shp[0] < n):
        raise _lib.CgsError(f"{what}: expected an NHWC image batch [>={n},64,64,3], got {shp}")


class DropState:

    def __init__(self, p: float, seed: int, step: Optional[torch.Tensor], img_off: int = 0):
        self.p, self.seed, self.step, self.img_off = float(p), int(seed), step, int(img_off)

    def shifted(self, img_off: int) -> "DropState":
        return DropState(self.p, self.seed, self.step, img_off)

    def desc(self, site: int, active: bool = True, per_img4: int = 0) -> _lib.Dropout:
        if not active or self.p <= 0.0:
            return _lib.Dropout(0.0, 0, 0, None, 0, 0)
        return _lib.Dropout(self.p, site, self.seed, self.step.data_ptr(), self.img_off * per_img4, 0)


NO_DROP = DropState(0.0, 0, None)
# ... 49 lines not shown
        self.device = A_u8.device
        self.dtype = torch.float32
        self.src = _lib.MixSrc(A_u8.data_ptr(), B_u8.data_ptr(), Z.data_ptr(), self.n_a, 0)

    def ptr(self):
        return C.cast(C.pointer(self.src), C.c_void_p)


class SlabPlan:

    def __init__(self):
        self.jobs = []
        self._table = None
        self._keep = None
        self._extra = []

    def add(self, slab: torch.Tensor, nslab: int, count: int, dst_off: int):
        for i, (s0, n0, c0, o0) in enumerate(self.jobs):
            if o0 == dst_off and c0 == count:
                if slab.data_ptr() != s0.data_ptr() + 4 * n0 * c0:
                    raise _lib.CgsError("slabs of passes that share a destination must be adjacent in memory")
                self.jobs[i] = (s0, n0 + nslab, c0, o0)
                self._extra.append(slab)
                return
        self.jobs.append((slab, nslab, count, dst_off))

    def build(self, grad_flat: torch.Tensor, accumulate: bool = False):
        CH = 1024
        rows = []
        for slab, nslab, count, off in self.jobs:
            for c0 in range(0, count, CH):
                rows.append((slab.data_ptr() + 4 * c0, grad_flat.data_ptr() + 4 * (off + c0), nslab, count, min(CH, count - c0)))
        arr = (_lib.ReduceJob * len(rows))()
        for i, (sp, dp, nslab, stride, cnt) in enumerate(rows):
            arr[i] = _lib.ReduceJob(sp, dp, nslab, stride, cnt, int(accumulate))
        host = torch.frombuffer(bytearray(bytes(arr)), dtype=torch.uint8)
        self._table = host.to(grad_flat.device)
        self._keep = grad_flat
        self._njobs = len(rows)
        self._max = max(r[4] for r in rows)
        return self

    def run(self, step: Optional[torch.Tensor] = None):
        _lib.call("cgs_reduce_slabs", _p(self._table), self._njobs, self._max, _p(step), _stream())

    def run_adam(self, step, param, grad, m, v, lr, b1, b2, eps, ticket, loss=None):
        ls = loss if loss is not None else (0, None, None, None, 0, 0.0, 0.0, 0.0, 0, 0, None)
        _lib.call("cgs_reduce_adam", _p(self._table), self._njobs, self._max, _p(step), _p(param), _p(grad), _p(m), _p(v),
                  float(lr), float(b1), float(b2), float(eps), _p(ticket), int(ls[0]), _p(ls[1]), _p(ls[2]), _p(ls[3]), int(ls[4]),
                  float(ls[5]), float(ls[6]), float(ls[7]), int(ls[8]), int(ls[9]), _p(ls[10]), _stream())


def critic_forward(flat: torch.Tensor, lay: Layout, x: torch.Tensor, n: int, drop: DropState = NO_DROP,
                   out: Optional[Dict[str, torch.Tensor]] = None, pw=None) -> Dict[str, torch.Tensor]:
    mixin = isinstance(x, MixInput)
    u8 = (not mixin) and x.dtype == torch.uint8
    if not mixin:
        _chk(x, torch.uint8 if u8 else torch.float32, "critic input")
    _chk_img(x, n, "critic input")
    dev = x.device
    o = out if out is not None else {}
    src = x
    whole = TAIL_FWD and ENC1_TAIL_FUSED and CRITIC_FWD_FUSED and (mixin or u8)
    for i, (key, hw, ca, cb, co, ups, act, pool, site) in enumerate(ENC_LAYERS):
        e = o.get(f"e{i}")
        if e is None:
            e = o[f"e{i}"] = torch.empty((n, hw // 2, hw // 2, co), device=dev, dtype=torch.float32)
        am = o.get(f"am{i}")
        if am is None:
            am = o[f"am{i}"] = torch.empty((n, hw // 2, hw // 2, co // 8), device=dev, dtype=torch.int32)
        if TAIL_FWD and (i >= 2 or (i == 1 and ENC1_TAIL_FUSED) or (i == 0 and whole)):
            src = e
            continue
        d = conv_desc(n, hw, ca, cb, co, u8 and i == 0, ups, act, pool, drop.desc(DROP_SITE_E2, site is not None, 128))
        if mixin and i == 0:
            d.src_a = _lib.SRC_MIX
        _lib.call("cgs_conv3x3_fwd", C.byref(d), src.ptr() if (mixin and i == 0) else _p(src), None,
                  C.c_void_p(flat.data_ptr() + 4 * lay.off(key + ".weight")),
                  C.c_void_p(flat.data_ptr() + 4 * lay.off(key + ".bias")), _p(e), _p(am), _stream())
        src = e
    for k, shape in (("e4", (n, 32)), ("h1", (n, 32)), ("pred", (n,))):
        if o.get(k) is None:
            o[k] = torch.empty(shape, device=dev, dtype=torch.float32)
    if TAIL_FWD:
        pwp = (pw[0], pw[1]) if pw else None
        tw = tail_enc_weights(flat, lay, (pwp[0].value, pwp[1].value) if pwp else None)
        if whole:
            k0, k3 = ENC_LAYERS[0][0], ENC_LAYERS[1][0]
            wp_ = lambda k: C.c_void_p(flat.data_ptr() + 4 * lay.off(k))
            _lib.call("cgs_critic_fwd_fused", n, C.byref(tw), x.ptr() if mixin else _p(x), int(mixin), wp_(k0 + ".weight"), wp_(k0 + ".bias"),
                      _p(o["e0"]), _p(o["am0"]), wp_(k3 + ".weight"), wp_(k3 + ".bias"), _p(o["e1"]), _p(o["am1"]), _p(o["e2"]), _p(o["am2"]),
                      _p(o["e3"]), _p(o["am3"]), _p(o["e4"]), _p(o["h1"]), _p(o["pred"]), _p(pw[2]) if pw else None,
                      drop.desc(DROP_SITE_E2, True, 128), drop.desc(DROP_SITE_E3, True, 64), drop.desc(DROP_SITE_H1, True, 8), _stream())
            return o
        if ENC1_TAIL_FUSED:
            k3 = ENC_LAYERS[1][0]
            _lib.call("cgs_enc1_tail_fwd", n, C.byref(tw), _p(o["e0"]), C.c_void_p(flat.data_ptr() + 4 * lay.off(k3 + ".weight")),
                      C.c_void_p(flat.data_ptr() + 4 * lay.off(k3 + ".bias")), _p(o["e1"]), _p(o["am1"]), _p(o["e2"]), _p(o["am2"]), _p(o["e3"]),
                      _p(o["am3"]), _p(o["e4"]), _p(o["h1"]), _p(o["pred"]), _p(pw[2]) if pw else None, drop.desc(DROP_SITE_E2, True, 128),
                      drop.desc(DROP_SITE_E3, True, 64), drop.desc(DROP_SITE_H1, True, 8), _stream())
            return o
        _lib.call("cgs_tail_enc_fwd", n, C.byref(tw), _p(o["e1"]), _p(o["e2"]), _p(o["am2"]), _p(o["e3"]), _p(o["am3"]),
                  _p(o["e4"]), _p(o["h1"]), _p(o["pred"]), _p(pw[2]) if pw else None, drop.desc(DROP_SITE_E2, True, 128),
                  drop.desc(DROP_SITE_E3, True, 64), drop.desc(DROP_SITE_H1, True, 8), _stream())
        return o
    fp = flat.data_ptr()
    _lib.call("cgs_head_fwd", n, _p(o["e3"]), C.c_void_p(fp + 4 * lay.off("features.14.weight")),
              C.c_void_p(fp + 4 * lay.off("features.14.bias")), C.c_void_p(fp + 4 * lay.off("crit.1.weight")),
              C.c_void_p(fp + 4 * lay.off("crit.1.bias")), C.c_void_p(fp + 4 * lay.off("crit.4.weight")),
              C.c_void_p(fp + 4 * lay.off("crit.4.bias")), drop.desc(DROP_SITE_E3, True, 64), drop.desc(DROP_SITE_H1, True, 8),
              _p(o["e4"]), _p(o["h1"]), _p(o["pred"]), pw[0] if pw else None, pw[1] if pw else None,
              _p(pw[2]) if pw else None, _stream())
    return o


def enc0_in_tail(mixin: bool, u8: bool, dx) -> bool:
    if mixin:
        return ENC0_WGRAD_IN_TAIL in ("both", "mix")
    return u8 and dx is None and ENC0_WGRAD_IN_TAIL in ("both", "A")


def head_wgrad(ranges, plan: "SlabPlan", lay: Layout, ws: Dict[str, torch.Tensor]):
    enc0 = next((r["enc0"] for r in ranges if isinstance(r, dict)), None)
    ranges = [r for r in ranges if not isinstance(r, dict)]
    if not ranges:
        if enc0 is not None:
            raise _lib.CgsError("head_wgrad: a deferred features.0 weight gradient needs a head range to ride with")
        return
    assert len(ranges) <= 2
    lib = _lib.load()
    total = sum(r[3] for r in ranges)
    nsl = lib.cgs_tail_head_wgrad_slabs(total)
    dev = ranges[0][0].device
    key = f"slab_head_{total}"
    if ws.get(key) is None:
        ws[key] = torch.empty((nsl, HEAD_SLAB), device=dev, dtype=torch.float32)
    pwb = next((r[5] for r in ranges if r[5] is not None), None)
    if pwb is not None and ws.get(key + "_pw") is None:
        ws[key + "_pw"] = torch.empty((nsl, PW_SLAB), device=dev, dtype=torch.float32)
    sl, slpw = ws[key], (ws[key + "_pw"] if pwb is not None else None)
    r0 = ranges[0]
    r1 = ranges[1] if len(ranges) > 1 else (None, None, None, 0, 0, None)
    if enc0 is not None:
        n_e, x_e, dy_e, am_e, slab_e = enc0[:5]
        e1w = enc0[5] if len(enc0) > 5 else None
        d3 = enc0[6] if len(enc0) > 6 else None
# ... 143 lines not shown
            if need_wgrad and not enc0_done:
                nsl = lib.cgs_enc0_bwd_mix_slabs(n)
                slab = buf("slab_enc0", (nsl, cnt))
                plan.add(slab, nsl, cnt, lay.off(key + ".weight"))
            e1w = enc1_wgrad if enc1_wgrad is not None else (0, None, None, None, None, 0)
            _lib.call("cgs_enc0_bwd_mix_enc1", A8.shape[0], int(bool(inj)), _p(src) if (need_wgrad and not mixin) else None, _p(d_cur),
                      _p(saved["am0"]), wptr, _p(A8), _p(B8), _p(Zm), float(l1s), float(l2s), _p(vfp), _p(dzp), _p(slab),
                      _p(e1w[1]), _p(e1w[2]), _p(e1w[3]), _p(e1w[4]), _stream())
            return None
        if need_wgrad and i in BOTH_ENC and (i > 0 or (dx is not None and dx_from == 0 and not u8)):
            nsl = lib.cgs_conv3x3_bwd_both_slabs(C.byref(d))
            if nsl < 0:
                _lib.check(nsl, "cgs_conv3x3_bwd_both_slabs")
            slab = buf(f"slab_enc{i}", (nsl, cnt))
            nxt = buf(f"de{i - 1}", (n, hw, hw, ca)) if i > 0 else dx
            _lib.call("cgs_conv3x3_bwd_both", C.byref(d), _p(src), None, _p(d_cur), _p(saved[f"am{i}"]), wptr,
                      _p(d_embeds[i - 1]) if (has_add and i > 0) else None, n_add if (has_add and i > 0) else 0, _p(nxt), None,
                      _p(slab), _stream())
            plan.add(slab, nsl, cnt, lay.off(key + ".weight"))
            d_cur = nxt
            continue
        nsl = lib.cgs_conv3x3_bwd_weight_slabs(C.byref(d))
        if nsl < 0:
            _lib.check(nsl, "cgs_conv3x3_bwd_weight_slabs")
        if need_wgrad and not (i == 0 and enc0_done):
            slab = buf(f"slab_enc{i}", (nsl, cnt))
            if i == 0 and head_sink is not None and u8:
                head_sink.append({"enc0": (n, src, d_cur, saved["am0"], slab, enc1_wgrad, dec3_rider)})
                enc1_wgrad, dec3_rider = None, None
            else:
                with side.fork():
                    _lib.call("cgs_conv3x3_bwd_weight", C.byref(d), _p(src), None, _p(d_cur), _p(saved[f"am{i}"]), _p(slab), _stream())
            plan.add(slab, nsl, cnt, lay.off(key + ".weight"))
        if i > 0:
            nxt = buf(f"de{i - 1}", (n, hw, hw, ca))
            _lib.call("cgs_conv3x3_bwd_data", C.byref(d), _p(d_cur), _p(saved[f"am{i}"]), wptr, None, _lib.ACT_NONE,
                      _p(d_embeds[i - 1]) if has_add else None, n_add if has_add else 0, _p(nxt), None, _stream())
            d_cur = nxt
        elif dx is not None and n - dx_from > 0:
            m = n - dx_from
            dd = conv_desc(m, hw, ca, cb, co, False, ups, act, pool, _lib.Dropout(0.0, 0, 0, None))
            _lib.call("cgs_conv3x3_bwd_data", C.byref(dd), _p(d_cur[dx_from:]), _p(saved["am0"][dx_from:]), wptr, None,
                      _lib.ACT_NONE, None, 0, _p(dx), None, _stream())
    if enc1_wgrad is not None:
        raise _lib.CgsError("critic_backward: features.3's deferred weight gradient found no features.0 launch to ride with")
    if dec3_rider is not None:
        raise _lib.CgsError("critic_backward: dec_model.3's deferred weight gradient found no features.0 launch to ride with")
    return dx


def masker_forward(flat: torch.Tensor, lay: Layout, x: torch.Tensor, embeds: List[torch.Tensor], n: int,
                   out: Optional[Dict[str, torch.Tensor]] = None, o4_done: bool = False,
                   keep_hm: bool = True, fp16_mask_head: bool = False,
                   zpart: Optional[torch.Tensor] = None) -> Dict[str, torch.Tensor]:
    u8 = x.dtype == torch.uint8
    _chk(x, torch.uint8 if u8 else torch.float32, "masker image input")
    _chk_img(x, n, "masker image input")
    dev = x.device
    fp = flat.data_ptr()
    o = out if out is not None else {}
    if o4_done:
        assert o.get("o4") is not None, "o4_done: the caller's head kernel already produced out['o4']"
    else:
        if o.get("o4") is None:
            o["o4"] = torch.empty((n, 32), device=dev, dtype=torch.float32)
        _lib.call("cgs_pointwise_fwd", n, 32, 32, _p(embeds[4]), C.c_void_p(fp + 4 * lay.off("dec_model.4.weight")),
                  C.c_void_p(fp + 4 * lay.off("dec_model.4.bias")), _p(o["o4"]), _stream())
    names = ("o3", "o2", "o1", "o0", "hm", "Z")
    srcs_a = (embeds[3], embeds[2], embeds[1], embeds[0], x, None)
    prev = o["o4"]
    if fp16_mask_head and (keep_hm or not MASK_INFER_FUSED):
        raise _lib.CgsError("fp16_mask_head is an inference-only option of the one-kernel mask head (keep_hm=False)")
    if TAIL_FWD:
        for nm, shp in (("o3", (n, 4, 4, 16)), ("o2", (n, 8, 8, 8)), ("o1", (n, 16, 16, 8))):
            if o.get(nm) is None:
                o[nm] = torch.empty(shp, device=dev, dtype=torch.float32)
        tw = tail_dec_weights(flat, lay)
        m0pack = None
        if (keep_hm and mask_train_fused(n) and zpart is not None) or (not keep_hm and MASK_INFER_FUSED and not fp16_mask_head):
            m0pack = o.get("m0pack")
            if m0pack is None:
                m0pack = o["m0pack"] = torch.empty(40 * 64, device=dev, dtype=torch.float32)
        dec0_done = False
        if DEC_TAIL_DEC0_FUSED:
            if o.get("o0") is None:
                o["o0"] = torch.empty((n, 32, 32, 8), device=dev, dtype=torch.float32)
            rc = _lib.load().cgs_tail_dec_fwd_dec0(n, C.byref(tw), _p(embeds[0]), _p(embeds[1]), _p(embeds[2]), _p(embeds[3]), _p(o["o4"]),
                                                   _p(o["o3"]), _p(o["o2"]), _p(o["o1"]), C.c_void_p(fp + 4 * lay.off("dec_model.0.weight")),
                                                   C.c_void_p(fp + 4 * lay.off("dec_model.0.bias")), _p(o["o0"]),
                                                   C.c_void_p(fp + 4 * lay.off("masker.0.weight")), _p(m0pack), _stream())
            if rc == 0:
                dec0_done = True
            elif rc != _lib.ERR_UNSUPPORTED:
                _lib.check(rc, "cgs_tail_dec_fwd_dec0")
        if not dec0_done:
            _lib.call("cgs_tail_dec_fwd_pack", n, C.byref(tw), _p(embeds[1]), _p(embeds[2]), _p(embeds[3]), _p(o["o4"]),
                      _p(o["o3"]), _p(o["o2"]), _p(o["o1"]), C.c_void_p(fp + 4 * lay.off("masker.0.weight")), _p(m0pack), _stream())
        prev = o["o0"] if dec0_done else o["o1"]
    for name, sa, (key, hw, ca, cb, co, ups, act, pool, _s) in zip(names, srcs_a, DEC_LAYERS):
        if TAIL_FWD and (name in ("o3", "o2", "o1") or (name == "o0" and dec0_done)):
            continue
        if name == "hm" and not keep_hm and MASK_INFER_FUSED:
            if o.get("Z") is None:
                o["Z"] = torch.empty((n, 64, 64), device=dev, dtype=torch.float32)
            margs = (n, _lib.SRC_U8 if u8 else _lib.SRC_F32, _p(x), _p(prev),
                     C.c_void_p(fp + 4 * lay.off("masker.0.weight")), C.c_void_p(fp + 4 * lay.off("masker.0.bias")),
                     C.c_void_p(fp + 4 * lay.off("masker.2.weight")), C.c_void_p(fp + 4 * lay.off("masker.2.bias")), _p(o["Z"]))
            if fp16_mask_head:
                rc = _lib.load().cgs_mask_infer_fwd_f16(*margs, _stream())
            else:
                rc = _lib.load().cgs_mask_infer_fwd_packed(*margs, _p(o.get("m0pack")) if TAIL_FWD else None, _stream())
            if rc == 0:
                return o
            if rc != _lib.ERR_UNSUPPORTED:
                _lib.check(rc, "cgs_mask_infer_fwd")
        if name == "hm" and keep_hm and mask_train_fused(n) and zpart is not None:
            for k, shp in (("hm", (n, 64, 64, 16)), ("Z", (n, 64, 64))):
                if o.get(k) is None:
                    o[k] = torch.empty(shp, device=dev, dtype=torch.float32)
            _lib.call("cgs_mask_train_fwd_packed", n, _lib.SRC_U8 if u8 else _lib.SRC_F32, _p(x), _p(prev),
                      C.c_void_p(fp + 4 * lay.off("masker.0.weight")), C.c_void_p(fp + 4 * lay.off("masker.0.bias")),
                      C.c_void_p(fp + 4 * lay.off("masker.2.weight")), C.c_void_p(fp + 4 * lay.off("masker.2.bias")),
                      _p(o["hm"]), _p(o["Z"]), _p(zpart), _p(o.get("m0pack")) if TAIL_FWD else None, _stream())
            return o
        shape = (n, hw, hw) if co == 1 else (n, hw, hw, co)
        if o.get(name) is None:
            o[name] = torch.empty(shape, device=dev, dtype=torch.float32)
        a = sa if sa is not None else prev
        b = prev if cb > 0 else None
        d = conv_desc(n, hw, ca, cb, co, u8 and name == "hm", ups, act, pool, _lib.Dropout(0.0, 0, 0, None))
        _lib.call("cgs_conv3x3_fwd", C.byref(d), _p(a), _p(b), C.c_void_p(fp + 4 * lay.off(key + ".weight")),
                  C.c_void_p(fp + 4 * lay.off(key + ".bias")), _p(o[name]), _p(zpart) if name == "Z" else None, _stream())
        prev = o[name]
    return o

# ... 151 lines not shown
```

include/cgs_hip.h:

```cpp
#ifndef CGS_HIP_H
#define CGS_HIP_H

#include <stdint.h>

#ifdef __cplusplus
extern "C" {
#endif

typedef void* cgs_stream_t;

enum { CGS_OK = 0, CGS_ERR_UNSUPPORTED = -1, CGS_ERR_BADARG = -2 };
enum { CGS_SRC_F32 = 0, CGS_SRC_U8 = 1, CGS_SRC_MIX = 2 };

typedef struct {
    const uint8_t* a;
    const uint8_t* b;
    const float* z;
    int32_t n_a;
    int32_t reserved;
} cgs_mix_src;
enum { CGS_ACT_NONE = 0, CGS_ACT_RELU = 1, CGS_ACT_LRELU = 2, CGS_ACT_SIGMOID = 3 };

typedef struct {
    float p;
// ... 59 lines not shown
int cgs_mask_infer_fwd_f16o(int32_t n, int32_t src_a, const void* x, const void* o0_f16, const float* w_m0_hwio, const float* b_m0,
                            const float* w_m2_hwio, const float* b_m2, float* z, cgs_stream_t stream);
int cgs_bf16_enc0_fwd(int32_t n, const void* x, int32_t x_is_f32, const float* w_hwio, const float* bias, void* e0_bf16, uint8_t* codes,
                      cgs_stream_t stream);
int cgs_bf16_mask0_fwd(int32_t n, const uint8_t* x_u8, const void* o0_bf16, const float* w_hwio, const float* bias, void* hm_bf16,
                       cgs_stream_t stream);
int cgs_bf16_mask2_fwd(int32_t n, const void* hm_bf16, const float* w_hwio, const float* bias, float* z, cgs_stream_t stream);
int cgs_bf16_enc0_bwd_data(int32_t n, const void* dy_bf16, const float* w_hwio, float* dx, cgs_stream_t stream);
int cgs_bf16_enc0_bwd_data_pooled(int32_t n, const void* dp_bf16, const void* addend_bf16, const uint8_t* codes, const float* w_hwio, float* dx,
                                  cgs_stream_t stream);
int cgs_bf16_enc0_fwd_mix(int32_t n, const uint8_t* a_u8, const uint8_t* b_u8, const float* z, const float* w_hwio, const float* bias, void* e0_bf16,
                          uint8_t* codes, cgs_stream_t stream);
int cgs_bf16_hwgrad_pooled_mix(int32_t n, const uint8_t* a_u8, const uint8_t* b_u8, const float* z, const void* dp, const uint8_t* codes, float* slab,
                               cgs_stream_t stream);
int cgs_bf16_enc0_bwd_mix(int32_t n, const void* dp_bf16, const uint8_t* codes, const float* w_hwio, const uint8_t* a_u8, const uint8_t* b_u8,
                          const float* z, float l1s, float l2s, float* dzpre, cgs_stream_t stream);
int cgs_bf16_mask2_bwd_data(int32_t n, const float* dz, const void* hm_bf16, const float* w_hwio, void* dhm_bf16, cgs_stream_t stream);
int cgs_bf16_mask0_bwd_data(int32_t n, const void* dhm_bf16, const float* w_hwio, void* do0_bf16, cgs_stream_t stream);
enum { CGS_H5_ENC1_FWD = 1, CGS_H5_ENC1_BWD_DATA = 2, CGS_H5_DEC0_FWD = 3, CGS_H5_DEC0_BWD_SKIP = 4, CGS_H5_DEC0_BWD_LOW = 5,
       CGS_H5_ENC1_BWD_DATA_POOLED = 6,
       CGS_H5_ENC2_FWD = 7, CGS_H5_ENC2_BWD_DATA_POOLED = 8, CGS_H5_DEC1_FWD = 9, CGS_H5_DEC1_BWD_SKIP = 10, CGS_H5_DEC1_BWD_LOW = 11,
       CGS_H5_DEC1_FWD_F32B = 12  };
int cgs_bf16_h5conv(int32_t which, int32_t n, const void* src_a, const void* src_b, const float* w_hwio, const float* bias, void* out,
                    uint8_t* codes, cgs_stream_t stream);
int cgs_bf16_hwgrad_slabs(int32_t n, int32_t hw, int32_t ca, int32_t cb, int32_t co);
int cgs_bf16_hwgrad(int32_t n, int32_t hw, int32_t ca, int32_t cb, int32_t co, int32_t a_kind, const void* src_a, const void* src_b,
                    const void* dy, float* slab, cgs_stream_t stream);
int cgs_bf16_hwgrad_pooled(int32_t n, int32_t hw, int32_t ca, int32_t a_kind, const void* src_a, const void* dp, const void* addend,
                           const uint8_t* codes, float* slab, cgs_stream_t stream);

typedef struct {
    const float *w6, *b6;
    const float *w10, *b10;
    const float *w14, *b14;
    const float *wl1, *bl1;
    const float *wl2, *bl2;
    const float *wpw, *bpw;
} cgs_tail_enc_weights;
typedef struct {
    const float *w3, *b3;
    const float *w2, *b2;
    const float *w1, *b1;
} cgs_tail_dec_weights;
int cgs_tail_enc_fwd(int32_t n, const cgs_tail_enc_weights* w, const float* e1, float* e2, uint32_t* am2, float* e3,
                     uint32_t* am3, float* e4, float* h1, float* pred, float* o4, cgs_dropout drop_e2,
                     cgs_dropout drop_e3, cgs_dropout drop_h1, cgs_stream_t stream);
int cgs_enc1_tail_fwd(int32_t n, const cgs_tail_enc_weights* w, const float* e0, const float* w3, const float* b3, float* e1,
                      uint32_t* am1, float* e2, uint32_t* am2, float* e3, uint32_t* am3, float* e4, float* h1, float* pred, float* o4,
                      cgs_dropout drop_e2, cgs_dropout drop_e3, cgs_dropout drop_h1, cgs_stream_t stream);
int cgs_critic_fwd_fused(int32_t n, const cgs_tail_enc_weights* w, const void* x, int32_t x_is_mix, const float* w0, const float* b0,
                         float* e0, uint32_t* am0, const float* w3, const float* b3, float* e1, uint32_t* am1, float* e2, uint32_t* am2,
                         float* e3, uint32_t* am3, float* e4, float* h1, float* pred, float* o4, cgs_dropout drop_e2, cgs_dropout drop_e3,
                         cgs_dropout drop_h1, cgs_stream_t stream);
int cgs_tail_dec_fwd(int32_t n, const cgs_tail_dec_weights* w, const float* e1, const float* e2, const float* e3,
                     const float* o4, float* o3, float* o2, float* o1, cgs_stream_t stream);
int cgs_tail_enc_fwd_h16(int32_t n, const cgs_tail_enc_weights* w, const float* e1, float* e2, uint32_t* am2, float* e3,
                         uint32_t* am3, float* e4, float* h1, float* pred, float* o4, cgs_stream_t stream);
int cgs_tail_dec_fwd_h16(int32_t n, const cgs_tail_dec_weights* w, const float* e1, const float* e2, const float* e3,
                         const float* o4, float* o3, float* o2, float* o1, cgs_stream_t stream);
int cgs_tail_infer_h16(int32_t n, const cgs_tail_enc_weights* we, const cgs_tail_dec_weights* wd, const float* e1, float* pred, float* o1,
                       cgs_stream_t stream);
int cgs_f16_enc1_tail_infer(int32_t n, const void* e0_f16, const float* w3, const float* b3, const cgs_tail_enc_weights* we,
                            const cgs_tail_dec_weights* wd, float* pred, float* o1, cgs_stream_t stream);
int cgs_tail_dec_fwd_pack(int32_t n, const cgs_tail_dec_weights* w, const float* e1, const float* e2, const float* e3,
                          const float* o4, float* o3, float* o2, float* o1, const float* w_m0, float* m0_pack, cgs_stream_t stream);

int cgs_tail_enc_bwd_slabs(int32_t n);
int cgs_tail_enc_bwd(int32_t n, const cgs_tail_enc_weights* w, const float* e1, const float* e2, const uint32_t* am2,
                     const float* e3, const uint32_t* am3, const float* e4, const float* h1, const float* pred,
                     const float* dpred, const float* target, float loss_scale, int32_t bce, const float* dE1, const float* dE2, const float* dE3, const float* d_o4,
                     int32_t n_add, float* de1, float* hvec, float* slab10, float* slab6,
                     cgs_dropout drop_e2, cgs_dropout drop_e3, cgs_dropout drop_h1, cgs_stream_t stream);
int cgs_tail_enc_bwd_rider(int32_t n, const cgs_tail_enc_weights* w, const float* e1, const float* e2, const uint32_t* am2,
                           const float* e3, const uint32_t* am3, const float* e4, const float* h1, const float* pred,
                           const float* dpred, const float* target, float loss_scale, int32_t bce, const float* dE1, const float* dE2,
                           const float* dE3, const float* d_o4, int32_t n_add, float* de1, float* hvec, float* slab10, float* slab6,
                           cgs_dropout drop_e2, cgs_dropout drop_e3, cgs_dropout drop_h1,
                           int32_t n_r, const float* e0_r, const float* o1_r, const float* dy_r, float* slab_r, int32_t nslab_r,
                           cgs_stream_t stream);
int cgs_tail_enc_bwd_enc1(int32_t n, const cgs_tail_enc_weights* w, const float* e1, const float* e2, const uint32_t* am2,
                          const float* e3, const uint32_t* am3, const float* e4, const float* h1, const float* pred,
                          const float* dpred, const float* target, float loss_scale, int32_t bce, const float* dE1, const float* dE2,
                          const float* dE3, const float* d_o4, int32_t n_add, float* de1, float* hvec, float* slab10, float* slab6,
                          cgs_dropout drop_e2, cgs_dropout drop_e3, cgs_dropout drop_h1,
                          int32_t n_r, const float* e0_r, const float* o1_r, const float* dy_r, float* slab_r, int32_t nslab_r,
                          const uint32_t* am1, const float* w_enc1, const float* addend0, int32_t n_addend, float* de0,
                          const float* e0, float* slab1,
                          int32_t x_kind, const void* x, const uint32_t* am0, float* slab0, cgs_stream_t stream);
int cgs_tail_head_wgrad_slabs(int32_t n_total);
int cgs_tail_head_wgrad(int32_t n0, const float* hvec0, const float* e4_0, const float* d_o4_0, int32_t n_o4_0, int32_t n1,
                        const float* hvec1, const float* e4_1, const float* d_o4_1, int32_t n_o4_1, float* slab_head,
                        float* slab_pw, cgs_stream_t stream);
int cgs_enc0_wgrad_u8_with_head(int32_t n, const uint8_t* x_u8, const float* dy, const uint32_t* amask, float* slab,
                                int32_t n0, const float* hvec0, const float* e4_0, const float* d_o4_0, int32_t n_o4_0,
                                int32_t n1, const float* hvec1, const float* e4_1, const float* d_o4_1, int32_t n_o4_1,
                                float* slab_head, float* slab_pw, cgs_stream_t stream);
int cgs_enc1_wgrad_rider_slabs(int32_t n);
int cgs_enc0_wgrad_u8_with_head_enc1(int32_t n, const uint8_t* x_u8, const float* dy, const uint32_t* amask, float* slab,
                                     int32_t n0, const float* hvec0, const float* e4_0, const float* d_o4_0, int32_t n_o4_0,
                                     int32_t n1, const float* hvec1, const float* e4_1, const float* d_o4_1, int32_t n_o4_1,
                                     float* slab_head, float* slab_pw,
                                     int32_t n1w, const float* e0_1, const float* dy1, const uint32_t* am1, float* slab1, int32_t nslab1,
                                     cgs_stream_t stream);
int cgs_dec3_wgrad_rider_slabs(int32_t n);
int cgs_enc0_wgrad_u8_with_head_riders(int32_t n, const uint8_t* x_u8, const float* dy, const uint32_t* amask, float* slab,
                                       int32_t n0, const float* hvec0, const float* e4_0, const float* d_o4_0, int32_t n_o4_0,
                                       int32_t n1, const float* hvec1, const float* e4_1, const float* d_o4_1, int32_t n_o4_1,
                                       float* slab_head, float* slab_pw,
                                       int32_t n1w, const float* e0_1, const float* dy1, const uint32_t* am1, float* slab1, int32_t nslab1,
                                       int32_t n3, const float* e3, const float* o4, const float* do3, float* slab3, cgs_stream_t stream);
int cgs_tail_dec_bwd_slabs(int32_t n);
int cgs_tail_dec_bwd(int32_t n, const cgs_tail_dec_weights* w, const float* e1, const float* e2, const float* e3,
                     const float* o4, const float* o3, const float* o2, const float* do1, float* dE1, float* dE2,
                     float* dE3, float* d_o4, float* slab3, float* slab2, float* slab1, cgs_stream_t stream);
int cgs_dec0_tail_dec_bwd(int32_t n, const cgs_tail_dec_weights* w, const float* dy_o0, const float* w0_hwio, float* dE0, const float* e1,
                          const float* e2, const float* e3, const float* o4, const float* o3, const float* o2, float* do1, float* dE1,
                          float* dE2, float* dE3, float* d_o4, float* slab3, float* slab2, float* slab1, cgs_stream_t stream);
int cgs_dec0_tail_dec_bwd_do3(int32_t n, const cgs_tail_dec_weights* w, const float* dy_o0, const float* w0, float* dE0, const float* e1,
                              const float* e2, const float* e3, const float* o4, const float* o3, const float* o2, float* do1,
                              float* dE1, float* dE2, float* dE3, float* d_o4, float* slab3, float* slab2, float* slab1, float* do3,
                              cgs_stream_t stream);
int cgs_tail_dec_fwd_dec0(int32_t n, const cgs_tail_dec_weights* w, const float* e0, const float* e1, const float* e2, const float* e3,
                          const float* o4, float* o3, float* o2, float* o1, const float* w0_hwio, const float* b0, float* o0,
                          const float* w_m0, float* m0_pack, cgs_stream_t stream);

int cgs_conv3x3_bwd_weight_slabs(const cgs_conv_desc* d);
int cgs_conv3x3_bwd_weight(const cgs_conv_desc* d, const void* src_a, const float* src_b,
                           const float* dy, const uint32_t* amask, float* slab,
                           cgs_stream_t stream);

int cgs_conv3x3_bwd_both_slabs(const cgs_conv_desc* d);
int cgs_conv3x3_bwd_both(const cgs_conv_desc* d, const void* src_a, const float* src_b, const float* dy,
                         const uint32_t* amask, const float* w_hwio, const float* addend, int32_t n_addend,
                         float* d_a, float* d_b, float* slab, cgs_stream_t stream);

typedef struct {
    const float* slab;
    float* dst;
    int32_t nslab, stride, count;
    int32_t accumulate;
} cgs_reduce_job;
int cgs_reduce_slabs(const cgs_reduce_job* jobs, int32_t njobs, int32_t max_count,
                     uint64_t* step, cgs_stream_t stream);

int cgs_reduce_adam(const cgs_reduce_job* jobs, int32_t njobs, int32_t max_count, uint64_t* step, float* param,
                    const float* grad_base, float* m, float* v, float lr, float beta1, float beta2, float eps,
                    uint32_t* ticket, int32_t n, const float* pred, const float* y, const float* zpart, int32_t nzpart,
                    float lfak, float l1, float l2, int32_t flags, int64_t nz, float* losses, cgs_stream_t stream);

int cgs_enc0_bwd_mix_slabs(int32_t n_mix);
int cgs_enc0_bwd_mix(int32_t n_a, int32_t inject, const float* mixed, const float* dy, const uint32_t* amask,
                     const float* w_hwio, const uint8_t* a, const uint8_t* b, const float* z, float l1_scale,
                     float l2_scale, const float* valuefak_pred, float* dzpre, float* slab, cgs_stream_t stream);
int cgs_enc0_bwd_mix_enc1(int32_t n_a, int32_t inject, const float* mixed, const float* dy, const uint32_t* amask,
                          const float* w_hwio, const uint8_t* a, const uint8_t* b, const float* z, float l1_scale,
                          float l2_scale, const float* valuefak_pred, float* dzpre, float* slab,
                          const float* e0_1, const float* dy1, const uint32_t* am1, float* slab1, cgs_stream_t stream);

int cgs_head_fwd(int32_t n, const float* e3, const float* w4, const float* b4, const float* w1,
                 const float* b1, const float* w2, const float* b2, cgs_dropout drop_in,
                 cgs_dropout drop_h, float* e4, float* h1, float* pred, const float* w_pw,
                 const float* b_pw, float* o4, cgs_stream_t stream);
int cgs_head_bwd_slabs(int32_t n);
int cgs_head_bwd(int32_t n, const float* e3, const float* e4, const float* h1, const float* pred,
                 const float* dpred, const float* d_e4_extra, const float* d_e3_extra, int32_t n_extra,
                 const float* w4,
                 const float* w1, const float* w2, cgs_dropout drop_in, cgs_dropout drop_h,
                 float* d_e3, float* slab, const float* d_o4, const float* w_pw, float* slab_pw,
                 cgs_stream_t stream);

int cgs_pointwise_fwd(int32_t n, int32_t ci, int32_t co, const float* x, const float* w,
                      const float* b, float* y, cgs_stream_t stream);
int cgs_pointwise_bwd_slabs(int32_t n);
int cgs_pointwise_bwd(int32_t n, int32_t ci, int32_t co, const float* x, const float* dy,
                      const float* w, float* dx, float* slab, cgs_stream_t stream);

int cgs_mix_fwd_partials(int32_t n, int32_t hw);
// ... 212 lines not shown
```

Baseline: 1.001 million.

## Fuse decoder tail and mask-head forward into one launch; pack mask weights in critic launch

Adds a combined kernel that runs the decoder tail, dec0 and the mask-head forward (h, Z, zpart) in one launch, and moves the mask-head weight packing into the critic's fused forward launch. The mask forward body is factored into a shared header so both kernels can reuse it. The aim is to cut kernel launches and the intermediate round trips between the decoder and mask stages. In exchange the fused kernel carries more registers and LDS, which may lower occupancy, and it falls back to the old path when it reports unsupported.

```diff
diff --git a/critic-guided-segmentation-of-rewarding-objects-in-first-person-views_amd/_lib.py b/critic-guided-segmentation-of-rewarding-objects-in-first-person-views_amd/_lib.py
--- a/critic-guided-segmentation-of-rewarding-objects-in-first-person-views_amd/_lib.py
+++ b/critic-guided-segmentation-of-rewarding-objects-in-first-person-views_amd/_lib.py
@@ -112,6 +112,7 @@
     "cgs_tail_enc_fwd": (i32, [i32, C.POINTER(TailEncWeights), vp, vp, vp, vp, vp, vp, vp, vp, vp, Dropout, Dropout, Dropout, vp]),
     "cgs_enc1_tail_fwd": (i32, [i32, C.POINTER(TailEncWeights), vp, vp, vp, vp, vp, vp, vp, vp, vp, vp, vp, vp, vp, Dropout, Dropout, Dropout, vp]),
     "cgs_critic_fwd_fused": (i32, [i32, C.POINTER(TailEncWeights), vp, i32] + [vp] * 16 + [Dropout, Dropout, Dropout, vp]),
+    "cgs_critic_fwd_fused_pack": (i32, [i32, C.POINTER(TailEncWeights), vp, i32] + [vp] * 16 + [Dropout, Dropout, Dropout, vp, vp, vp]),
     "cgs_tail_dec_fwd": (i32, [i32, C.POINTER(TailDecWeights), vp, vp, vp, vp, vp, vp, vp, vp]),
     "cgs_tail_enc_fwd_h16": (i32, [i32, C.POINTER(TailEncWeights), vp, vp, vp, vp, vp, vp, vp, vp, vp, vp]),
     "cgs_tail_dec_fwd_h16": (i32, [i32, C.POINTER(TailDecWeights), vp, vp, vp, vp, vp, vp, vp, vp]),
@@ -136,6 +137,7 @@
     "cgs_dec3_wgrad_rider_slabs": (i32, [i32]),
     "cgs_enc0_wgrad_u8_with_head_riders": (i32, [i32, vp, vp, vp, vp, i32, vp, vp, vp, i32, i32, vp, vp, vp, i32, vp, vp, i32, vp, vp, vp, vp, i32, i32, vp, vp, vp, vp, vp]),
     "cgs_tail_dec_fwd_dec0": (i32, [i32, C.POINTER(TailDecWeights)] + [vp] * 13 + [vp]),
+    "cgs_dec_mask_fwd": (i32, [i32, C.POINTER(TailDecWeights)] + [vp] * 11 + [i32] + [vp] * 8 + [vp]),
     "cgs_conv3x3_bwd_weight_slabs": (i32, [C.POINTER(ConvDesc)]),
     "cgs_conv3x3_bwd_weight": (i32, [C.POINTER(ConvDesc), vp, vp, vp, vp, vp, vp]),
     "cgs_conv3x3_bwd_both_slabs": (i32, [C.POINTER(ConvDesc)]),
diff --git a/critic-guided-segmentation-of-rewarding-objects-in-first-person-views_amd/build.py b/critic-guided-segmentation-of-rewarding-objects-in-first-person-views_amd/build.py
--- a/critic-guided-segmentation-of-rewarding-objects-in-first-person-views_amd/build.py
+++ b/critic-guided-segmentation-of-rewarding-objects-in-first-person-views_amd/build.py
@@ -8,7 +8,7 @@
 CSRC = os.path.join(HERE, "csrc")
 LIB = os.path.join(HERE, "libcgs_hip.so")
 SOURCES = ["conv_fwd.hip", "conv_wgrad.hip", "wgrad_dec0.hip", "conv_bwd_both.hip", "mconv.hip", "mask_head.hip", "mask_fwd.hip", "head.hip", "elementwise.hip", "tail.hip", "tail_infer.hip", "gen.hip", "gen4.hip", "gen_train.hip", "gen_f16.hip", "gen_bf16_train.hip", "hconv.hip", "hwgrad.hip", "bn.hip", "gen_enc0.hip", "crf.hip", "video.hip", "vis.hip", "sheet.hip", "metrics.hip", "objects.hip", "objects_match.hip", "objects_track.hip", "saliency.hip", "boundary.hip", "fit.hip", "temporal.hip", "overlay.hip"]
-HEADERS = ["cgs_common.h", "head_wgrad.h", "conv_tile.h", "conv_body.h", "wgrad_body.h", "head_body.h", "tail_common.h", "tail4.h", "tail_h16.h", "gen_common.h", "gen4_common.h", "gen_wgrad_rows.h", "gen_wgrad_fold.h", "wgrad_dec0.h", "wgrad_sparse.h", os.path.join(REPO, "include", "cgs_hip.h")]
+HEADERS = ["cgs_common.h", "head_wgrad.h", "conv_tile.h", "conv_body.h", "wgrad_body.h", "head_body.h", "mask_fwd_body.h", "tail_common.h", "tail4.h", "tail_h16.h", "gen_common.h", "gen4_common.h", "gen_wgrad_rows.h", "gen_wgrad_fold.h", "wgrad_dec0.h", "wgrad_sparse.h", os.path.join(REPO, "include", "cgs_hip.h")]
 ARCH = "gfx950"
 EXTRA_FLAGS = {"conv_fwd.hip": ["-fno-slp-vectorize"], "conv_bwd_both.hip": ["-fno-slp-vectorize"], "saliency.hip": ["-ffp-contract=off"]}
 
diff --git a/critic-guided-segmentation-of-rewarding-objects-in-first-person-views_amd/csrc/conv_body.h b/critic-guided-segmentation-of-rewarding-objects-in-first-person-views_amd/csrc/conv_body.h
--- a/critic-guided-segmentation-of-rewarding-objects-in-first-person-views_amd/csrc/conv_body.h
+++ b/critic-guided-segmentation-of-rewarding-objects-in-first-person-views_amd/csrc/conv_body.h
@@ -597,7 +597,7 @@
 }
 
 template <class C>
-static size_t conv_lds_bytes() {
+static constexpr size_t conv_lds_bytes() {
     using G = Geo<C::H, C::W, C::THREADS, C::CW>;
     constexpr int PA = (C::SRC == SRC_SCALAR) ? 1 : (C::CA + 3) / 4;
     constexpr int PB = C::CB / 4;
diff --git a/critic-guided-segmentation-of-rewarding-objects-in-first-person-views_amd/csrc/mask_fwd.hip b/critic-guided-segmentation-of-rewarding-objects-in-first-person-views_amd/csrc/mask_fwd.hip
--- a/critic-guided-segmentation-of-rewarding-objects-in-first-person-views_amd/csrc/mask_fwd.hip
+++ b/critic-guided-segmentation-of-rewarding-objects-in-first-person-views_amd/csrc/mask_fwd.hip
@@ -1,22 +1,9 @@
-#include "conv_tile.h"
-
-struct MaskFwdParams {
-    const void* img; const float* o0;
-    const float* w0; const float* b0; const float* w2; const float* b2;
-    float* h; float* z; float* zpart;
-    int n;
-    unsigned long long* dbg;
-    const float* w0_pack;
-};
+#include "mask_fwd_body.h"
 
 namespace {
-using MG = Geo<64, 64, 256, 1>;
-constexpr int kPSlots = 9;
-constexpr int kWinPitch = 33;
 unsigned long long* g_maskfwd_stamps = nullptr;
 }
 
-#define MF_STAMP(k) do { if (CGS_STAMP_PTR(P.dbg) && tid == 0) CGS_STAMP_PTR(P.dbg)[(size_t)blockIdx.x * 64 + (k)] = __builtin_amdgcn_s_memtime(); } while (0)
 #ifdef CGS_DEBUG_STAMPS
 extern "C" int dbg_maskfwd_stamps(unsigned long long* stamps) { g_maskfwd_stamps = stamps; return CGS_OK; }
 #endif
@@ -24,308 +11,10 @@
 template <int SRC>
 __global__ void __launch_bounds__(256, SRC == SRC_U8C3 ? 2 : 1) mask_fwd_kernel(MaskFwdParams P) {
     if (CGS_KARG_PREFETCH) cgs_kernarg_prefetch<sizeof(MaskFwdParams)>();
-    using G = MG;
-    constexpr int A4 = (G::TRA * G::PWA + 1 + 3) / 4 * 4, B4 = 2 * G::TRB * G::PWB;
-    static_assert(A4 + B4 <= 2048, "tiles fit the 32 KB staging area");
-    __shared__ __attribute__((aligned(16))) float4 stage4[2048];
-    float4* const ldsA = stage4;
-    float4* const ldsB = stage4 + A4;
-    __shared__ float win[kPSlots * 16 * kWinPitch];
+    __shared__ __attribute__((aligned(16))) float4 stage4[kMaskStageF4];
+    __shared__ float win[kMaskWinFloats];
     __shared__ float zred[8];
-    const int tid = threadIdx.x, lane = tid & 63, wave = tid >> 6;
-    const int n = blockIdx.x, N = P.n;
-    const int lb = lane >> 2, li = lane & 3;
-    MF_STAMP(0);
-
-    constexpr int GW = G::W / 4, EA = G::TRA * GW, ITA = (EA + 255) / 256;
-    constexpr int EB = G::TRB * G::PWB * 2, ITB = (EB + 255) / 256;
-    uint32_t ra[ITA][(SRC == SRC_U8C3) ? 3 : 12];
-    float4 rb[ITB];
-    auto fetch = [&](int row0) {
-#pragma unroll
-        for (int it = 0; it < ITA; ++it) {
-            int e = tid + 256 * it; e = e < EA ? e : EA - 1;
-            const int g = e % GW, r = e / GW, y = row0 + r - 1;
-            const bool in = y >= 0 && y < G::H;
-            const int gi = in ? ((n * G::H + y) * G::W + g * 4) * 3 / 4 : 0;
-            if constexpr (SRC == SRC_U8C3) {
-                const uint32_t* src = (const uint32_t*)P.img;
-                ra[it][0] = src[gi]; ra[it][1] = src[gi + 1]; ra[it][2] = src[gi + 2];
-            } else {
-                const float4* src = (const float4*)P.img;
-#pragma unroll
-                for (int k = 0; k < 3; ++k) {
-                    const float4 v = src[gi + k];
-                    ra[it][4 * k] = __float_as_uint(v.x); ra[it][4 * k + 1] = __float_as_uint(v.y);
-                    ra[it][4 * k + 2] = __float_as_uint(v.z); ra[it][4 * k + 3] = __float_as_uint(v.w);
-                }
-            }
-        }
-        const int sy0 = row0 / 2;
-#pragma unroll
-        for (int it = 0; it < ITB; ++it) {
-            int e = tid + 256 * it; e = e < EB ? e : EB - 1;
-            const int p = e % 2, c = (e / 2) % G::PWB, r = e / (2 * G::PWB);
-            const int sy = sy0 + r - 1, sx = c - 1;
-            const bool in = sy >= 0 && sy < G::QH && sx >= 0 && sx < G::QW;
-            rb[it] = ((const float4*)P.o0)[in ? ((n * G::QH + sy) * G::QW + sx) * 2 + p : 0];
-        }
-    };
-    auto commit = [&](int row0) {
-        const float sc = 1.f / 255.f;
-#pragma unroll
-        for (int it = 0; it < ITA; ++it) {
-            int e = tid + 256 * it; e = e < EA ? e : EA - 1;
-            const int g = e % GW, r = e / GW, y = row0 + r - 1;
-            const bool in = y >= 0 && y < G::H;
-            float4 p0, p1, p2, p3;
-            if constexpr (SRC == SRC_U8C3) {
-                const uint32_t d0 = ra[it][0], d1 = ra[it][1], d2 = ra[it][2];
-                p0 = make_float4((d0 & 255) * sc, ((d0 >> 8) & 255) * sc, ((d0 >> 16) & 255) * sc, 0.f);
-                p1 = make_float4((d0 >> 24) * sc, (d1 & 255) * sc, ((d1 >> 8) & 255) * sc, 0.f);
-                p2 = make_float4(((d1 >> 16) & 255) * sc, (d1 >> 24) * sc, (d2 & 255) * sc, 0.f);
-                p3 = make_float4(((d2 >> 8) & 255) * sc, ((d2 >> 16) & 255) * sc, (d2 >> 24) * sc, 0.f);
-            } else {
-                auto f = [&](int k) { return __uint_as_float(ra[it][k]); };
-                p0 = make_float4(f(0), f(1), f(2), 0.f); p1 = make_float4(f(3), f(4), f(5), 0.f);
-                p2 = make_float4(f(6), f(7), f(8), 0.f); p3 = make_float4(f(9), f(10), f(11), 0.f);
-            }
-            const int base = r * G::PWA;
-            ldsA[base + G::pc(g * 4 + 1)] = in ? p0 : f4zero();
-            ldsA[base + G::pc(g * 4 + 2)] = in ? p1 : f4zero();
-            ldsA[base + G::pc(g * 4 + 3)] = in ? p2 : f4zero();
-            ldsA[base + G::pc(g * 4 + 4)] = in ? p3 : f4zero();
-        }
-        zero_halo_cols<G, 1>(ldsA, tid);
-        const int sy0 = row0 / 2;
-#pragma unroll
-        for (int it = 0; it < ITB; ++it) {
-            int e = tid + 256 * it; e = e < EB ? e : EB - 1;
-            const int p = e % 2, c = (e / 2) % G::PWB, r = e / (2 * G::PWB);
-            const int sy = sy0 + r - 1, sx = c - 1;
-            const bool in = sy >= 0 && sy < G::QH && sx >= 0 && sx < G::QW;
-            ldsB[(p * G::TRB + r) * G::PWB + c] = in ? rb[it] : f4zero();
-        }
-    };
-    fetch(0);
-    float wimg[4][2];
-    float wups[4][4][2];
-    if (P.w0_pack) {
-        const float* wp = P.w0_pack + lane;
-#pragma unroll
-        for (int g = 0; g < 4; ++g) {
-#pragma unroll
-            for (int k = 0; k < 2; ++k) wimg[g][k] = wp[(g * 2 + k) * 64];
-#pragma unroll
-            for (int pos = 0; pos < 4; ++pos)
-#pragma unroll
-                for (int ry = 0; ry < 2; ++ry) wups[pos][g][ry] = wp[(8 + (pos * 4 + g) * 2 + ry) * 64];
-        }
-    } else {
-    float* wst = (float*)ldsA;
-    for (int e = tid; e < 9 * 11 * 16; e += 256) wst[e] = P.w0[e];
-    __syncthreads();
-#pragma unroll
-    for (int g = 0; g < 4; ++g) {
-#pragma unroll
-        for (int k = 0; k < 2; ++k) {
-            const int step = 16 * k + lb;
-            wimg[g][k] = step < 27 ? wst[((step / 3) * 11 + step % 3) * 16 + 4 * g + li] : 0.f;
-        }
-#pragma unroll
-        for (int pos = 0; pos < 4; ++pos) {
-            const int oy = pos >> 1, ox = pos & 1;
-#pragma unroll
-            for (int ry = 0; ry < 2; ++ry) {
-                const int rx = lb >> 3, ci = lb & 7;
-                const int ky0 = (oy == 0) ? (ry == 0 ? 0 : 1) : (ry == 0 ? 0 : 2), ky1 = (oy == 0) ? (ry == 0 ? 0 : 2) : (ry == 0 ? 1 : 2);
-                const int kx0 = (ox == 0) ? (rx == 0 ? 0 : 1) : (rx == 0 ? 0 : 2), kx1 = (ox == 0) ? (rx == 0 ? 0 : 2) : (rx == 0 ? 1 : 2);
-                auto wv = [&](int ky, int kx) { return wst[((ky * 3 + kx) * 11 + 3 + ci) * 16 + 4 * g + li]; };
-                const float w00 = wv(ky0, kx0), w01 = wv(ky0, kx1), w10 = wv(ky1, kx0), w11 = wv(ky1, kx1);
-                const bool my = ky1 > ky0, mx = kx1 > kx0;
-                float s = w00;
-                s += mx ? w01 : 0.f;
-                s += my ? w10 : 0.f;
-                s += (mx && my) ? w11 : 0.f;
-                wups[pos][g][ry] = s;
-            }
-            __builtin_amdgcn_sched_barrier(0);
-        }
-    }
-    }
-    float w2r[3];
-#pragma unroll
-    for (int g = 0; g < 3; ++g) w2r[g] = (4 * g + li < 9) ? P.w2[(4 * g + li) * 16 + lb] : 0.f;
-    const cgs_cptr b0c = cgs_to_const(P.b0);
-    const float b2v = cgs_to_const(P.b2)[0];
-    __syncthreads();
-
-    MF_STAMP(1);
-    const QuadPos q0 = quad_pos<G>(tid, 0);
-    const int qy_l = q0.qy_l, qx = q0.qx;
-    int pcx[4];
-#pragma unroll
-    for (int dx = 0; dx < 4; ++dx) pcx[dx] = G::pc(2 * qx + dx);
-    float zs1 = 0.f, zs2 = 0.f;
-
-#pragma unroll 1
-    for (int strip = 0; strip < G::STRIPS; ++strip) {
-        const int row0 = strip * G::TH;
-        QuadPos q = q0;
-        q.n = n; q.row0 = row0;
-        MF_STAMP(2 + 10 * strip);
-        commit(row0);
-        __syncthreads();
-        MF_STAMP(3 + 10 * strip);
-        if (strip + 1 < G::STRIPS) fetch(row0 + G::TH);
-
-        frag4 acc[4][4];
-#pragma unroll
-        for (int i = 0; i < 4; ++i)
-#pragma unroll
-            for (int g = 0; g < 4; ++g) acc[i][g] = frag4{b0c[4 * g], b0c[4 * g + 1], b0c[4 * g + 2], b0c[4 * g + 3]};
-        {
-            float4 pt[4][4];
-            read_patch_a<G>(pt, ldsA, 0, q, pcx);
-            mfma_plane<4, 3, 3, 0, 2>(acc, pt, wimg);
-        }
-        MF_STAMP(4 + 10 * strip);
-        static_for<2>([&](auto PL) {
-            constexpr int p = decltype(PL)::value;
-            float4 s[3][3];
-            const int base = (p * G::TRB + qy_l) * G::PWB + qx;
-#pragma unroll
-            for (int j = 0; j < 3; ++j)
-#pragma unroll
-                for (int i = 0; i < 3; ++i) s[j][i] = ldsB[base + j * G::PWB + i];
-            static_for<16>([&](auto T) {
-                constexpr int t = decltype(T)::value, ry = t >> 3, rx = (t >> 2) & 1, c = t & 3;
-                constexpr int abid = rx * 8 + 4 * p + c;
-#pragma unroll
-                for (int pos = 0; pos < 4; ++pos) {
-                    const float x = f4get(s[(pos >> 1) + ry][(pos & 1) + rx], c);
-#pragma unroll
-                    for (int g = 0; g < 4; ++g)
-                        acc[pos][g] = __builtin_amdgcn_mfma_f32_4x4x1f32(wups[pos][g][ry], x, acc[pos][g], 4, abid, 0);
-                }
-            });
-        });
-
-        float hv[4][16];
-        const int y0 = row0 + 2 * qy_l, x0 = 2 * qx;
-#pragma unroll
-        for (int pos = 0; pos < 4; ++pos)
-#pragma unroll
-            for (int c = 0; c < 16; ++c) { const float v = acc[pos][c >> 2][c & 3]; hv[pos][c] = fmaxf(v, 0.01f * v); }
-        MF_STAMP(5 + 10 * strip);
-        __syncthreads();
-        MF_STAMP(6 + 10 * strip);
-        if (P.h) {
-            float4* sw4 = stage4 + wave * 512;
-            const int pp = lane;
-#pragma unroll
-            for (int oy = 0; oy < 2; ++oy) {
-#pragma unroll
-                for (int j = 0; j < 8; ++j) {
-                    const int pos = oy * 2 + (j >> 2), c0 = 4 * (j & 3);
-                    sw4[pp * 8 + (j ^ (pp & 7))] = make_float4(hv[pos][c0], hv[pos][c0 + 1], hv[pos][c0 + 2], hv[pos][c0 + 3]);
-                }
-#pragma unroll
-                for (int k = 0; k < 8; ++k) {
-                    const int i = lane + 64 * k, rp = i >> 3, j = i & 7;
-                    const float4 v = sw4[rp * 8 + (j ^ (rp & 7))];
-                    const int y = row0 + 2 * (2 * wave + (k >> 2)) + oy;
-                    ((float4*)P.h)[((size_t)(n * 64 + y) * 64) * 4 + (rp & 31) * 8 + j] = v;
-                }
-            }
-        }
-        MF_STAMP(7 + 10 * strip);
-        frag4 c2[4][3];
-#pragma unroll
-        for (int i = 0; i < 4; ++i)
-#pragma unroll
-            for (int g = 0; g < 3; ++g) c2[i][g] = frag4{0.f, 0.f, 0.f, 0.f};
-        static_for<16>([&](auto CH) {
-            constexpr int ch = decltype(CH)::value;
-#pragma unroll
-            for (int pos = 0; pos < 4; ++pos)
-#pragma unroll
-                for (int g = 0; g < 3; ++g)
-                    c2[pos][g] = __builtin_amdgcn_mfma_f32_4x4x1f32(w2r[g], hv[pos][ch], c2[pos][g], 4, ch, 0);
-        });
-        MF_STAMP(8 + 10 * strip);
-        float sw[4][4];
-#pragma unroll
-        for (int wy = -1; wy <= 2; ++wy)
-#pragma unroll
-            for (int wx = -1; wx <= 2; ++wx) {
-                float s = 0.f;
-#pragma unroll
-                for (int oy = 0; oy < 2; ++oy)
-#pragma unroll
-                    for (int ox = 0; ox < 2; ++ox) {
-                        const int ky = oy - wy + 1, kx = ox - wx + 1;
-                        if (ky >= 0 && ky <= 2 && kx >= 0 && kx <= 2) {
-                            const int tap = ky * 3 + kx;
-                            s += c2[oy * 2 + ox][tap >> 2][tap & 3];
-                        }
-                    }
-                sw[wy + 1][wx + 1] = s;
-            }
-        float* wown = win + (qy_l + 1) * 16 * kWinPitch + qx;
-#pragma unroll
-        for (int e = 0; e < 16; ++e) wown[e * kWinPitch] = sw[e >> 2][e & 3];
-        __syncthreads();
-        MF_STAMP(9 + 10 * strip);
-        const bool has_top = strip > 0 || qy_l > 0;
-        const float* wtop = win + qy_l * 16 * kWinPitch + qx;
-        float zz[3][2];
-#pragma unroll
-        for (int wy = -1; wy <= 1; ++wy) {
-#pragma unroll
-            for (int wx = 0; wx <= 1; ++wx) {
-                const bool has_side = wx == 0 ? qx > 0 : qx < 31;
-                const int side = has_side ? (wx == 0 ? -1 : 1) : 0;
-                const int wxs = wx == 0 ? 2 : -1;
-                float s = sw[wy + 1][wx + 1];
-                const float a = wown[((wy + 1) * 4 + wxs + 1) * kWinPitch + side];
-                s += has_side ? a : 0.f;
-                if (wy <= 0) {
-                    const float b = wtop[((wy + 3) * 4 + wx + 1) * kWinPitch];
-                    const float c = wtop[((wy + 3) * 4 + wxs + 1) * kWinPitch + side];
-                    s += has_top ? b : 0.f;
-                    s += (has_top && has_side) ? c : 0.f;
-                }
-                zz[wy + 1][wx] = act_fwd<CGS_ACT_SIGMOID>(s + b2v);
-            }
-        }
-        const bool last_row = strip == G::STRIPS - 1 && qy_l == 7;
-#pragma unroll
-        for (int wy = -1; wy <= 1; ++wy) {
-            const int y = y0 + wy;
-            if (wy == 1 ? last_row : y >= 0) {
-                *(float2*)(P.z + (size_t)(n * 64 + y) * 64 + x0) = make_float2(zz[wy + 1][0], zz[wy + 1][1]);
-                zs1 += fabsf(zz[wy + 1][0]) + fabsf(zz[wy + 1][1]);
-                zs2 += zz[wy + 1][0] * zz[wy + 1][0] + zz[wy + 1][1] * zz[wy + 1][1];
-            }
-        }
-        MF_STAMP(10 + 10 * strip);
-        __syncthreads();
-        MF_STAMP(11 + 10 * strip);
-        if (qy_l == 7) {
-#pragma unroll
-            for (int e = 0; e < 16; ++e) win[e * kWinPitch + qx] = sw[e >> 2][e & 3];
-        }
-    }
-    if (P.zpart) {
-        zs1 = wave_sum(zs1); zs2 = wave_sum(zs2);
-        if (lane == 0) { zred[2 * wave] = zs1; zred[2 * wave + 1] = zs2; }
-        __syncthreads();
-        if (tid == 0) {
-            P.zpart[2 * n] = (zred[0] + zred[2]) + (zred[4] + zred[6]);
-            P.zpart[2 * n + 1] = (zred[1] + zred[3]) + (zred[5] + zred[7]);
-        }
-    }
+    mask_fwd_body<SRC, false, false>(P, stage4, win, zred, [] {});
 }
 
 int mask_train_partials(int n) { return n; }
diff --git a/critic-guided-segmentation-of-rewarding-objects-in-first-person-views_amd/csrc/mask_fwd_body.h b/critic-guided-segmentation-of-rewarding-objects-in-first-person-views_amd/csrc/mask_fwd_body.h
--- /dev/null
+++ b/critic-guided-segmentation-of-rewarding-objects-in-first-person-views_amd/csrc/mask_fwd_body.h
@@ -0,0 +1,332 @@
+#pragma once
+#include "conv_tile.h"
+
+struct MaskFwdParams {
+    const void* img; const float* o0;
+    const float* w0; const float* b0; const float* w2; const float* b2;
+    float* h; float* z; float* zpart;
+    int n;
+    unsigned long long* dbg;
+    const float* w0_pack;
+};
+
+namespace {
+using MG = Geo<64, 64, 256, 1>;
+constexpr int kPSlots = 9;
+constexpr int kWinPitch = 33;
+constexpr int kMaskStageF4 = 2048;
+constexpr int kMaskWinFloats = kPSlots * 16 * kWinPitch;
+}
+
+#define MF_STAMP(k) do { if (CGS_STAMP_PTR(P.dbg) && tid == 0) CGS_STAMP_PTR(P.dbg)[(size_t)blockIdx.x * 64 + (k)] = __builtin_amdgcn_s_memtime(); } while (0)
+
+template <int SRC, bool HOIST, bool PACKED, class Mid>
+__device__ __forceinline__ void mask_fwd_body(const MaskFwdParams& P, float4* const stage4, float* const win, float* const zred, Mid&& mid) {
+    using G = MG;
+    constexpr int A4 = (G::TRA * G::PWA + 1 + 3) / 4 * 4, B4 = 2 * G::TRB * G::PWB;
+    static_assert(A4 + B4 <= 2048, "tiles fit the 32 KB staging area");
+    float4* const ldsA = stage4;
+    float4* const ldsB = stage4 + A4;
+    const int tid = threadIdx.x, lane = tid & 63, wave = tid >> 6;
+    const int n = blockIdx.x, N = P.n;
+    const int lb = lane >> 2, li = lane & 3;
+    MF_STAMP(0);
+
+    constexpr int GW = G::W / 4, EA = G::TRA * GW, ITA = (EA + 255) / 256;
+    constexpr int EB = G::TRB * G::PWB * 2, ITB = (EB + 255) / 256;
+    uint32_t ra[ITA][(SRC == SRC_U8C3) ? 3 : 12];
+    float4 rb[ITB];
+    auto fetch_a = [&](int row0) {
+#pragma unroll
+        for (int it = 0; it < ITA; ++it) {
+            int e = tid + 256 * it; e = e < EA ? e : EA - 1;
+            const int g = e % GW, r = e / GW, y = row0 + r - 1;
+            const bool in = y >= 0 && y < G::H;
+            const int gi = in ? ((n * G::H + y) * G::W + g * 4) * 3 / 4 : 0;
+            if constexpr (SRC == SRC_U8C3) {
+                const uint32_t* src = (const uint32_t*)P.img;
+                ra[it][0] = src[gi]; ra[it][1] = src[gi + 1]; ra[it][2] = src[gi + 2];
+            } else {
+                const float4* src = (const float4*)P.img;
+#pragma unroll
+                for (int k = 0; k < 3; ++k) {
+                    const float4 v = src[gi + k];
+                    ra[it][4 * k] = __float_as_uint(v.x); ra[it][4 * k + 1] = __float_as_uint(v.y);
+                    ra[it][4 * k + 2] = __float_as_uint(v.z); ra[it][4 * k + 3] = __float_as_uint(v.w);
+                }
+            }
+        }
+    };
+    auto fetch_b = [&](int row0) {
+        const int sy0 = row0 / 2;
+#pragma unroll
+        for (int it = 0; it < ITB; ++it) {
+            int e = tid + 256 * it; e = e < EB ? e : EB - 1;
+            const int p = e % 2, c = (e / 2) % G::PWB, r = e / (2 * G::PWB);
+            const int sy = sy0 + r - 1, sx = c - 1;
+            const bool in = sy >= 0 && sy < G::QH && sx >= 0 && sx < G::QW;
+            rb[it] = ((const float4*)P.o0)[in ? ((n * G::QH + sy) * G::QW + sx) * 2 + p : 0];
+        }
+    };
+    auto fetch = [&](int row0) { fetch_a(row0); fetch_b(row0); };
+    auto commit = [&](int row0) {
+        const float sc = 1.f / 255.f;
+#pragma unroll
+        for (int it = 0; it < ITA; ++it) {
+            int e = tid + 256 * it; e = e < EA ? e : EA - 1;
+            const int g = e % GW, r = e / GW, y = row0 + r - 1;
+            const bool in = y >= 0 && y < G::H;
+            float4 p0, p1, p2, p3;
+            if constexpr (SRC == SRC_U8C3) {
+                const uint32_t d0 = ra[it][0], d1 = ra[it][1], d2 = ra[it][2];
+                p0 = make_float4((d0 & 255) * sc, ((d0 >> 8) & 255) * sc, ((d0 >> 16) & 255) * sc, 0.f);
+                p1 = make_float4((d0 >> 24) * sc, (d1 & 255) * sc, ((d1 >> 8) & 255) * sc, 0.f);
+                p2 = make_float4(((d1 >> 16) & 255) * sc, (d1 >> 24) * sc, (d2 & 255) * sc, 0.f);
+                p3 = make_float4(((d2 >> 8) & 255) * sc, ((d2 >> 16) & 255) * sc, (d2 >> 24) * sc, 0.f);
+            } else {
+                auto f = [&](int k) { return __uint_as_float(ra[it][k]); };
+                p0 = make_float4(f(0), f(1), f(2), 0.f); p1 = make_float4(f(3), f(4), f(5), 0.f);
+                p2 = make_float4(f(6), f(7), f(8), 0.f); p3 = make_float4(f(9), f(10), f(11), 0.f);
+            }
+            const int base = r * G::PWA;
+            ldsA[base + G::pc(g * 4 + 1)] = in ? p0 : f4zero();
+            ldsA[base + G::pc(g * 4 + 2)] = in ? p1 : f4zero();
+            ldsA[base + G::pc(g * 4 + 3)] = in ? p2 : f4zero();
+            ldsA[base + G::pc(g * 4 + 4)] = in ? p3 : f4zero();
+        }
+        zero_halo_cols<G, 1>(ldsA, tid);
+        const int sy0 = row0 / 2;
+#pragma unroll
+        for (int it = 0; it < ITB; ++it) {
+            int e = tid + 256 * it; e = e < EB ? e : EB - 1;
+            const int p = e % 2, c = (e / 2) % G::PWB, r = e / (2 * G::PWB);
+            const int sy = sy0 + r - 1, sx = c - 1;
+            const bool in = sy >= 0 && sy < G::QH && sx >= 0 && sx < G::QW;
+            ldsB[(p * G::TRB + r) * G::PWB + c] = in ? rb[it] : f4zero();
+        }
+    };
+    if constexpr (HOIST) fetch_a(0); else fetch(0);
+    float wimg[4][2];
+    float wups[4][4][2];
+    if (PACKED || P.w0_pack) {
+        const float* wp = P.w0_pack + lane;
+#pragma unroll
+        for (int g = 0; g < 4; ++g) {
+#pragma unroll
+            for (int k = 0; k < 2; ++k) wimg[g][k] = wp[(g * 2 + k) * 64];
+#pragma unroll
+            for (int pos = 0; pos < 4; ++pos)
+#pragma unroll
+                for (int ry = 0; ry < 2; ++ry) wups[pos][g][ry] = wp[(8 + (pos * 4 + g) * 2 + ry) * 64];
+        }
+    } else if constexpr (!PACKED) {
+    float* wst = (float*)ldsA;
+    for (int e = tid; e < 9 * 11 * 16; e += 256) wst[e] = P.w0[e];
+    __syncthreads();
+#pragma unroll
+    for (int g = 0; g < 4; ++g) {
+#pragma unroll
+        for (int k = 0; k < 2; ++k) {
+            const int step = 16 * k + lb;
+            wimg[g][k] = step < 27 ? wst[((step / 3) * 11 + step % 3) * 16 + 4 * g + li] : 0.f;
+        }
+#pragma unroll
+        for (int pos = 0; pos < 4; ++pos) {
+            const int oy = pos >> 1, ox = pos & 1;
+#pragma unroll
+            for (int ry = 0; ry < 2; ++ry) {
+                const int rx = lb >> 3, ci = lb & 7;
+                const int ky0 = (oy == 0) ? (ry == 0 ? 0 : 1) : (ry == 0 ? 0 : 2), ky1 = (oy == 0) ? (ry == 0 ? 0 : 2) : (ry == 0 ? 1 : 2);
+                const int kx0 = (ox == 0) ? (rx == 0 ? 0 : 1) : (rx == 0 ? 0 : 2), kx1 = (ox == 0) ? (rx == 0 ? 0 : 2) : (rx == 0 ? 1 : 2);
+                auto wv = [&](int ky, int kx) { return wst[((ky * 3 + kx) * 11 + 3 + ci) * 16 + 4 * g + li]; };
+                const float w00 = wv(ky0, kx0), w01 = wv(ky0, kx1), w10 = wv(ky1, kx0), w11 = wv(ky1, kx1);
+                const bool my = ky1 > ky0, mx = kx1 > kx0;
+                float s = w00;
+                s += mx ? w01 : 0.f;
+                s += my ? w10 : 0.f;
+                s += (mx && my) ? w11 : 0.f;
+                wups[pos][g][ry] = s;
+            }
+            __builtin_amdgcn_sched_barrier(0);
+        }
+    }
+    }
+    float w2r[3];
+#pragma unroll
+    for (int g = 0; g < 3; ++g) w2r[g] = (4 * g + li < 9) ? P.w2[(4 * g + li) * 16 + lb] : 0.f;
+    const cgs_cptr b0c = cgs_to_const(P.b0);
+    const float b2v = cgs_to_const(P.b2)[0];
+    if constexpr (HOIST) {
+        __builtin_amdgcn_sched_barrier(0);
+        mid();
+        fetch_b(0);
+    }
+    __syncthreads();
+
+    MF_STAMP(1);
+    const QuadPos q0 = quad_pos<G>(tid, 0);
+    const int qy_l = q0.qy_l, qx = q0.qx;
+    int pcx[4];
+#pragma unroll
+    for (int dx = 0; dx < 4; ++dx) pcx[dx] = G::pc(2 * qx + dx);
+    float zs1 = 0.f, zs2 = 0.f;
+
+#pragma unroll 1
+    for (int strip = 0; strip < G::STRIPS; ++strip) {
+        const int row0 = strip * G::TH;
+        QuadPos q = q0;
+        q.n = n; q.row0 = row0;
+        MF_STAMP(2 + 10 * strip);
+        commit(row0);
+        __syncthreads();
+        MF_STAMP(3 + 10 * strip);
+        if (strip + 1 < G::STRIPS) fetch(row0 + G::TH);
+
+        frag4 acc[4][4];
+#pragma unroll
+        for (int i = 0; i < 4; ++i)
+#pragma unroll
+            for (int g = 0; g < 4; ++g) acc[i][g] = frag4{b0c[4 * g], b0c[4 * g + 1], b0c[4 * g + 2], b0c[4 * g + 3]};
+        {
+            float4 pt[4][4];
+            read_patch_a<G>(pt, ldsA, 0, q, pcx);
+            mfma_plane<4, 3, 3, 0, 2>(acc, pt, wimg);
+        }
+        MF_STAMP(4 + 10 * strip);
+        static_for<2>([&](auto PL) {
+            constexpr int p = decltype(PL)::value;
+            float4 s[3][3];
+            const int base = (p * G::TRB + qy_l) * G::PWB + qx;
+#pragma unroll
+            for (int j = 0; j < 3; ++j)
+#pragma unroll
+                for (int i = 0; i < 3; ++i) s[j][i] = ldsB[base + j * G::PWB + i];
+            static_for<16>([&](auto T) {
+                constexpr int t = decltype(T)::value, ry = t >> 3, rx = (t >> 2) & 1, c = t & 3;
+                constexpr int abid = rx * 8 + 4 * p + c;
+#pragma unroll
+                for (int pos = 0; pos < 4; ++pos) {
+                    const float x = f4get(s[(pos >> 1) + ry][(pos & 1) + rx], c);
+#pragma unroll
+                    for (int g = 0; g < 4; ++g)
+                        acc[pos][g] = __builtin_amdgcn_mfma_f32_4x4x1f32(wups[pos][g][ry], x, acc[pos][g], 4, abid, 0);
+                }
+            });
+        });
+
+        float hv[4][16];
+        const int y0 = row0 + 2 * qy_l, x0 = 2 * qx;
+#pragma unroll
+        for (int pos = 0; pos < 4; ++pos)
+#pragma unroll
+            for (int c = 0; c < 16; ++c) { const float v = acc[pos][c >> 2][c & 3]; hv[pos][c] = fmaxf(v, 0.01f * v); }
+        MF_STAMP(5 + 10 * strip);
+        __syncthreads();
+        MF_STAMP(6 + 10 * strip);
+        if (P.h) {
+            float4* sw4 = stage4 + wave * 512;
+            const int pp = lane;
+#pragma unroll
+            for (int oy = 0; oy < 2; ++oy) {
+#pragma unroll
+                for (int j = 0; j < 8; ++j) {
+                    const int pos = oy * 2 + (j >> 2), c0 = 4 * (j & 3);
+                    sw4[pp * 8 + (j ^ (pp & 7))] = make_float4(hv[pos][c0], hv[pos][c0 + 1], hv[pos][c0 + 2], hv[pos][c0 + 3]);
+                }
+#pragma unroll
+                for (int k = 0; k < 8; ++k) {
+                    const int i = lane + 64 * k, rp = i >> 3, j = i & 7;
+                    const float4 v = sw4[rp * 8 + (j ^ (rp & 7))];
+                    const int y = row0 + 2 * (2 * wave + (k >> 2)) + oy;
+                    ((float4*)P.h)[((size_t)(n * 64 + y) * 64) * 4 + (rp & 31) * 8 + j] = v;
+                }
+            }
+        }
+        MF_STAMP(7 + 10 * strip);
+        frag4 c2[4][3];
+#pragma unroll
+        for (int i = 0; i < 4; ++i)
+#pragma unroll
+            for (int g = 0; g < 3; ++g) c2[i][g] = frag4{0.f, 0.f, 0.f, 0.f};
+        static_for<16>([&](auto CH) {
+            constexpr int ch = decltype(CH)::value;
+#pragma unroll
+            for (int pos = 0; pos < 4; ++pos)
+#pragma unroll
+                for (int g = 0; g < 3; ++g)
+                    c2[pos][g] = __builtin_amdgcn_mfma_f32_4x4x1f32(w2r[g], hv[pos][ch], c2[pos][g], 4, ch, 0);
+        });
+        MF_STAMP(8 + 10 * strip);
+        float sw[4][4];
+#pragma unroll
+        for (int wy = -1; wy <= 2; ++wy)
+#pragma unroll
+            for (int wx = -1; wx <= 2; ++wx) {
+                float s = 0.f;
+#pragma unroll
+                for (int oy = 0; oy < 2; ++oy)
+#pragma unroll
+                    for (int ox = 0; ox < 2; ++ox) {
+                        const int ky = oy - wy + 1, kx = ox - wx + 1;
+                        if (ky >= 0 && ky <= 2 && kx >= 0 && kx <= 2) {
+                            const int tap = ky * 3 + kx;
+                            s += c2[oy * 2 + ox][tap >> 2][tap & 3];
+                        }
+                    }
+                sw[wy + 1][wx + 1] = s;
+            }
+        float* wown = win + (qy_l + 1) * 16 * kWinPitch + qx;
+#pragma unroll
+        for (int e = 0; e < 16; ++e) wown[e * kWinPitch] = sw[e >> 2][e & 3];
+        __syncthreads();
+        MF_STAMP(9 + 10 * strip);
+        const bool has_top = strip > 0 || qy_l > 0;
+        const float* wtop = win + qy_l * 16 * kWinPitch + qx;
+        float zz[3][2];
+#pragma unroll
+        for (int wy = -1; wy <= 1; ++wy) {
+#pragma unroll
+            for (int wx = 0; wx <= 1; ++wx) {
+                const bool has_side = wx == 0 ? qx > 0 : qx < 31;
+                const int side = has_side ? (wx == 0 ? -1 : 1) : 0;
+                const int wxs = wx == 0 ? 2 : -1;
+                float s = sw[wy + 1][wx + 1];
+                const float a = wown[((wy + 1) * 4 + wxs + 1) * kWinPitch + side];
+                s += has_side ? a : 0.f;
+                if (wy <= 0) {
+                    const float b = wtop[((wy + 3) * 4 + wx + 1) * kWinPitch];
+                    const float c = wtop[((wy + 3) * 4 + wxs + 1) * kWinPitch + side];
+                    s += has_top ? b : 0.f;
+                    s += (has_top && has_side) ? c : 0.f;
+                }
+                zz[wy + 1][wx] = act_fwd<CGS_ACT_SIGMOID>(s + b2v);
+            }
+        }
+        const bool last_row = strip == G::STRIPS - 1 && qy_l == 7;
+#pragma unroll
+        for (int wy = -1; wy <= 1; ++wy) {
+            const int y = y0 + wy;
+            if (wy == 1 ? last_row : y >= 0) {
+                *(float2*)(P.z + (size_t)(n * 64 + y) * 64 + x0) = make_float2(zz[wy + 1][0], zz[wy + 1][1]);
+                zs1 += fabsf(zz[wy + 1][0]) + fabsf(zz[wy + 1][1]);
+                zs2 += zz[wy + 1][0] * zz[wy + 1][0] + zz[wy + 1][1] * zz[wy + 1][1];
+            }
+        }
+        MF_STAMP(10 + 10 * strip);
+        __syncthreads();
+        MF_STAMP(11 + 10 * strip);
+        if (qy_l == 7) {
+#pragma unroll
+            for (int e = 0; e < 16; ++e) win[e * kWinPitch + qx] = sw[e >> 2][e & 3];
+        }
+    }
+    if (P.zpart) {
+        zs1 = wave_sum(zs1); zs2 = wave_sum(zs2);
+        if (lane == 0) { zred[2 * wave] = zs1; zred[2 * wave + 1] = zs2; }
+        __syncthreads();
+        if (tid == 0) {
+            P.zpart[2 * n] = (zred[0] + zred[2]) + (zred[4] + zred[6]);
+            P.zpart[2 * n + 1] = (zred[1] + zred[3]) + (zred[5] + zred[7]);
+        }
+    }
+}
diff --git a/critic-guided-segmentation-of-rewarding-objects-in-first-person-views_amd/csrc/tail.hip b/critic-guided-segmentation-of-rewarding-objects-in-first-person-views_amd/csrc/tail.hip
--- a/critic-guided-segmentation-of-rewarding-objects-in-first-person-views_amd/csrc/tail.hip
+++ b/critic-guided-segmentation-of-rewarding-objects-in-first-person-views_amd/csrc/tail.hip
@@ -4,6 +4,7 @@
 #include "wgrad_dec0.h"
 #include "conv_body.h"
 #include "wgrad_sparse.h"
+#include "mask_fwd_body.h"
 
 namespace {
 
@@ -72,7 +73,9 @@
     int n;
     int nblocks;
     unsigned long long* dbg;
+    const float* m0_w; float* m0_pack;
 };
+__device__ __forceinline__ void mask0_pack_weights(const float* __restrict__ w0, float* __restrict__ pack, int lane);
 
 using X1P = TileP<16, 16, 8, 8, 148>;
 using X2P = TileP<8, 8, 8, 8, 84>;
@@ -88,6 +91,12 @@
     __shared__ float es[32], hs[32];
     if (CGS_KARG_PREFETCH) cgs_kernarg_prefetch<sizeof(TailEncFwdParams) + 2 * sizeof(ConvParams)>();
     const int tid = threadIdx.x, lane = tid & 63, wave = tid >> 6;
+    if constexpr (FUSED && ENC0 == 1) {
+        if ((int)blockIdx.x == P.nblocks) {
+            if (wave == 0) mask0_pack_weights(P.m0_w, P.m0_pack, lane);
+            return;
+        }
+    }
     if (CGS_STAMP_PTR(P.dbg) && tid == 0) CGS_STAMP_PTR(P.dbg)[(size_t)blockIdx.x * 16] = __builtin_amdgcn_s_memtime();
     const int o = tid & 31, kg = tid >> 5;
     int img = blockIdx.x;
@@ -346,15 +355,16 @@
     return CGS_OK;
 }
 
-extern "C" int cgs_critic_fwd_fused(int32_t n, const cgs_tail_enc_weights* w, const void* x, int32_t x_is_mix, const float* w0, const float* b0,
+extern "C" int cgs_critic_fwd_fused_pack(int32_t n, const cgs_tail_enc_weights* w, const void* x, int32_t x_is_mix, const float* w0, const float* b0,
                                     float* e0, uint32_t* am0, const float* w3, const float* b3, float* e1, uint32_t* am1, float* e2, uint32_t* am2,
                                     float* e3, uint32_t* am3, float* e4, float* h1, float* pred, float* o4, cgs_dropout drop_e2,
-                                    cgs_dropout drop_e3, cgs_dropout drop_h1, cgs_stream_t stream) {
+                                    cgs_dropout drop_e3, cgs_dropout drop_h1, const float* w_m0, float* m0_pack, cgs_stream_t stream) {
     if (n < 0 || !w || !x || !w0 || !b0 || !e0 || !am0 || !w3 || !b3 || !e1 || !am1 || !e2 || !am2 || !e3 || !am3 || !e4 || !h1 || !pred) return CGS_ERR_BADARG;
     if (!w->w6 || !w->b6 || !w->w10 || !w->b10 || !w->w14 || !w->b14 || !w->wl1 || !w->bl1 || !w->wl2 || !w->bl2) return CGS_ERR_BADARG;
     if (o4 && (!w->wpw || !w->bpw)) return CGS_ERR_BADARG;
+    if (m0_pack && (!w_m0 || x_is_mix)) return CGS_ERR_BADARG;
     if (n == 0) return CGS_OK;
-    TailEncFwdParams P{*w, e1, e2, am2, e3, am3, e4, h1, pred, o4, drop_e2, drop_e3, drop_h1, n, n, g_tail_stamps ? g_tail_stamps + 0 * 2048 * 16 : nullptr};
+    TailEncFwdParams P{*w, e1, e2, am2, e3, am3, e4, h1, pred, o4, drop_e2, drop_e3, drop_h1, n, n, g_tail_stamps ? g_tail_stamps + 0 * 2048 * 16 : nullptr, w_m0, m0_pack};
     ConvParams PC{}, PC0{};
     PC.src_a = e0; PC.w = w3; PC.bias = b3; PC.out = e1; PC.amask_out = am1; PC.n = n;
     PC0.w = w0; PC0.bias = b0; PC0.out = e0; PC0.amask_out = am0; PC0.n = n;
@@ -368,10 +378,18 @@
     } else {
         PC0.src_a = x;
         if (conv_lds_bytes<FEnc0U8P>() > lds) lds = conv_lds_bytes<FEnc0U8P>();
-        hipLaunchKernelGGL((tail_enc_fwd_kernel<true, 1>), dim3(n), dim3(256), lds, (hipStream_t)stream, P, PC, PC0);
+        hipLaunchKernelGGL((tail_enc_fwd_kernel<true, 1>), dim3(n + (m0_pack ? 1 : 0)), dim3(256), lds, (hipStream_t)stream, P, PC, PC0);
     }
     CGS_HIP_CHECK_LAUNCH();
     return CGS_OK;
+}
+
+extern "C" int cgs_critic_fwd_fused(int32_t n, const cgs_tail_enc_weights* w, const void* x, int32_t x_is_mix, const float* w0, const float* b0,
+                                    float* e0, uint32_t* am0, const float* w3, const float* b3, float* e1, uint32_t* am1, float* e2, uint32_t* am2,
+                                    float* e3, uint32_t* am3, float* e4, float* h1, float* pred, float* o4, cgs_dropout drop_e2,
+                                    cgs_dropout drop_e3, cgs_dropout drop_h1, cgs_stream_t stream) {
+    return cgs_critic_fwd_fused_pack(n, w, x, x_is_mix, w0, b0, e0, am0, w3, b3, e1, am1, e2, am2, e3, am3, e4, h1, pred, o4, drop_e2, drop_e3, drop_h1,
+                                     nullptr, nullptr, stream);
 }
 
 struct TailDecFwdParams {
@@ -416,23 +434,21 @@
 
 using T1F = TileP<16, 16, 16, 16, 292>;
 
-template <bool FUSED, bool H16 = false>
-__global__ void __launch_bounds__(256) __attribute__((amdgpu_waves_per_eu(3, 3))) tail_dec_fwd_kernel(TailDecFwdParams P, ConvParams PC) {
-    static_assert(!H16 || !FUSED, "fp16 operands: the stand-alone inference form");
-    if (CGS_KARG_PREFETCH) cgs_kernarg_prefetch<sizeof(TailDecFwdParams) + sizeof(ConvParams)>();
-    extern __shared__ __attribute__((aligned(16))) float4 dec_conv_smem[];
-    __shared__ __attribute__((aligned(16))) float t1[T1F::FLOATS];
-    __shared__ __attribute__((aligned(16))) float t2[T8x24::FLOATS];
-    __shared__ __attribute__((aligned(16))) float t3[T4x48::FLOATS];
-    __shared__ __attribute__((aligned(16))) float w2s[14 * 64 * 2];
-    static_assert(14 * 64 * 2 >= 216 * 8, "either form fits");
-    __shared__ float part[4][16][16];
+struct DecFwdLds {
+    float4* conv;
+    float* t1; float* t2; float* t3;
+    float* w2s;
+    float (*part)[16][16];
+};
+constexpr int kDecW2sFloats = 14 * 64 * 2;
+static_assert(kDecW2sFloats >= 216 * 8, "either form fits");
+
+template <bool FUSED, bool H16>
+__device__ __forceinline__ void tail_dec_fwd_body(const TailDecFwdParams& P, const ConvParams& PC, const DecFwdLds S) {
+    float4* const dec_conv_smem = S.conv;
+    float* const t1 = S.t1; float* const t2 = S.t2; float* const t3 = S.t3; float* const w2s = S.w2s;
+    float (*const part)[16][16] = S.part;
     const int tid = threadIdx.x, lane = tid & 63, wave = tid >> 6;
-    if ((int)blockIdx.x == P.nblocks) {
-        if (wave == 0) mask0_pack_weights(P.m0_w, P.m0_pack, lane);
-        return;
-    }
-    if constexpr (FUSED) cgs_stagger<8, CGS_STAGGER_DEC_FWD>();
     if (CGS_STAMP_PTR(P.dbg) && tid == 0) CGS_STAMP_PTR(P.dbg)[(size_t)blockIdx.x * 16] = __builtin_amdgcn_s_memtime();
     const int l15 = lane & 15, kq = lane >> 4;
     int img = blockIdx.x;
@@ -592,6 +608,25 @@
         conv3x3_body_pipe<FDec0P>(PC, 2 * (int)blockIdx.x, dec_conv_smem);
     }
     if (CGS_STAMP_PTR(P.dbg) && tid == 0) CGS_STAMP_PTR(P.dbg)[(size_t)blockIdx.x * 16 + 15] = __builtin_amdgcn_s_memtime();
+#undef DEC_FWD_FETCH
+}
+
+template <bool FUSED, bool H16 = false>
+__global__ void __launch_bounds__(256) __attribute__((amdgpu_waves_per_eu(3, 3))) tail_dec_fwd_kernel(TailDecFwdParams P, ConvParams PC) {
+    static_assert(!H16 || !FUSED, "fp16 operands: the stand-alone inference form");
+    if (CGS_KARG_PREFETCH) cgs_kernarg_prefetch<sizeof(TailDecFwdParams) + sizeof(ConvParams)>();
+    extern __shared__ __attribute__((aligned(16))) float4 dec_conv_smem[];
+    __shared__ __attribute__((aligned(16))) float t1[T1F::FLOATS];
+    __shared__ __attribute__((aligned(16))) float t2[T8x24::FLOATS];
+    __shared__ __attribute__((aligned(16))) float t3[T4x48::FLOATS];
+    __shared__ __attribute__((aligned(16))) float w2s[kDecW2sFloats];
+    __shared__ float part[4][16][16];
+    if ((int)blockIdx.x == P.nblocks) {
+        if (threadIdx.x < 64) mask0_pack_weights(P.m0_w, P.m0_pack, threadIdx.x);
+        return;
+    }
+    if constexpr (FUSED) cgs_stagger<8, CGS_STAGGER_DEC_FWD>();
+    tail_dec_fwd_body<FUSED, H16>(P, PC, DecFwdLds{dec_conv_smem, t1, t2, t3, w2s, part});
 }
 
 extern "C" int cgs_tail_dec_fwd_pack(int32_t n, const cgs_tail_dec_weights* w, const float* e1, const float* e2, const float* e3,
@@ -623,6 +658,67 @@
                                                  hipFuncAttributeMaxDynamicSharedMemorySize, (int)(conv_lds_bytes<FDec0P>()));
     if (attr != hipSuccess) return (int)attr;
     hipLaunchKernelGGL(tail_dec_fwd_kernel<true>, dim3(n + (m0_pack ? 1 : 0)), dim3(256), lds, (hipStream_t)stream, P, PC);
+    CGS_HIP_CHECK_LAUNCH();
+    return CGS_OK;
+}
+
+#ifndef CGS_DEC_MASK_HOIST
+#define CGS_DEC_MASK_HOIST 1
+#endif
+#ifndef CGS_STAGGER_DEC_MASK
+#define CGS_STAGGER_DEC_MASK 0
+#endif
+namespace {
+constexpr int kDmConvF4 = (int)(conv_lds_bytes<FDec0P>() / sizeof(float4));
+static_assert(T1F::FLOATS % 4 == 0 && T8x24::FLOATS % 4 == 0 && T4x48::FLOATS % 4 == 0, "16-byte aligned slices");
+constexpr int kDmDecFloats = 4 * kDmConvF4 + T1F::FLOATS + T8x24::FLOATS + T4x48::FLOATS + kDecW2sFloats + 4 * 16 * 16;
+constexpr int kDmMaskFloats = 4 * kMaskStageF4 + kMaskWinFloats + 8;
+constexpr int kDmF4 = ((kDmDecFloats > kDmMaskFloats ? kDmDecFloats : kDmMaskFloats) + 3) / 4;
+unsigned long long* g_dec_mask_stamps = nullptr;
+}
+#ifdef CGS_DEBUG_STAMPS
+extern "C" int dbg_dec_mask_stamps(unsigned long long* stamps) { g_dec_mask_stamps = stamps; return CGS_OK; }
+#endif
+
+__global__ void __launch_bounds__(256, 2) dec_mask_fwd_kernel(TailDecFwdParams P, ConvParams PC, MaskFwdParams M) {
+    if (CGS_KARG_PREFETCH) cgs_kernarg_prefetch<sizeof(TailDecFwdParams) + sizeof(ConvParams) + sizeof(MaskFwdParams)>();
+    __shared__ __attribute__((aligned(16))) float4 lds[kDmF4];
+    float* const f = (float*)lds;
+    float* const t1 = f + 4 * kDmConvF4;
+    float* const t2 = t1 + T1F::FLOATS;
+    float* const t3 = t2 + T8x24::FLOATS;
+    float* const w2s = t3 + T4x48::FLOATS;
+    const DecFwdLds S{lds, t1, t2, t3, w2s, (float (*)[16][16])(w2s + kDecW2sFloats)};
+    float* const win = f + 4 * kMaskStageF4;
+    cgs_stagger<8, CGS_STAGGER_DEC_MASK>();
+    auto phase_d = [&] {
+        tail_dec_fwd_body<true, false>(P, PC, S);
+        __syncthreads();
+    };
+    if constexpr (CGS_DEC_MASK_HOIST) {
+        mask_fwd_body<SRC_U8C3, true, true>(M, lds, win, win + kMaskWinFloats, phase_d);
+    } else {
+        phase_d();
+        mask_fwd_body<SRC_U8C3, false, true>(M, lds, win, win + kMaskWinFloats, [] {});
+    }
+}
+
+extern "C" int cgs_dec_mask_fwd(int32_t n, const cgs_tail_dec_weights* w, const float* e0, const float* e1, const float* e2, const float* e3,
+                                const float* o4, float* o3, float* o2, float* o1, const float* w0, const float* b0, float* o0, int32_t src_a,
+                                const void* x, const float* b_m0, const float* w_m2, const float* b_m2, float* h, float* z, float* zpart,
+                                const float* m0_pack, cgs_stream_t stream) {
+    if (n < 0 || !w || !e0 || !e1 || !e2 || !e3 || !o4 || !o3 || !o2 || !o1 || !w0 || !b0 || !o0) return CGS_ERR_BADARG;
+    if (!x || !b_m0 || !w_m2 || !b_m2 || !h || !z || !zpart || !m0_pack) return CGS_ERR_BADARG;
+    if (!w->w3 || !w->b3 || !w->w2 || !w->b2 || !w->w1 || !w->b1) return CGS_ERR_BADARG;
+    if (src_a != CGS_SRC_U8 && src_a != CGS_SRC_F32) return CGS_ERR_BADARG;
+    if (src_a != CGS_SRC_U8) return CGS_ERR_UNSUPPORTED;
+    if (n == 0) return CGS_OK;
+    if (n > tail_fwd_cap()) return CGS_ERR_UNSUPPORTED;
+    TailDecFwdParams P{*w, e1, e2, e3, o4, o3, o2, o1, n, n, g_tail_stamps ? g_tail_stamps + 1 * 2048 * 16 : nullptr, nullptr, nullptr};
+    ConvParams PC{};
+    PC.src_a = e0; PC.src_b = o1; PC.w = w0; PC.bias = b0; PC.out = o0; PC.n = n;
+    MaskFwdParams M{x, o0, nullptr, b_m0, w_m2, b_m2, h, z, zpart, n, g_dec_mask_stamps, m0_pack};
+    hipLaunchKernelGGL(dec_mask_fwd_kernel, dim3(n), dim3(256), 0, (hipStream_t)stream, P, PC, M);
     CGS_HIP_CHECK_LAUNCH();
     return CGS_OK;
 }
diff --git a/critic-guided-segmentation-of-rewarding-objects-in-first-person-views_amd/engine.py b/critic-guided-segmentation-of-rewarding-objects-in-first-person-views_amd/engine.py
--- a/critic-guided-segmentation-of-rewarding-objects-in-first-person-views_amd/engine.py
+++ b/critic-guided-segmentation-of-rewarding-objects-in-first-person-views_amd/engine.py
@@ -184,8 +184,13 @@
         fm_ptr = self.fm.data_ptr()
         pw = (C.c_void_p(fm_ptr + 4 * self.lm.off("dec_model.4.weight")), C.c_void_p(fm_ptr + 4 * self.lm.off("dec_model.4.bias")),
               self._o4_full)
+        m0 = None
+        if hg.ENC0_MIX_FUSED and hg.dec_mask_fwd_fused(n, self.ab.dtype == torch.uint8) and hg.critic_fwd_whole(False, True):
+            if self.mbuf.get("m0pack") is None:
+                self.mbuf["m0pack"] = torch.empty(40 * 64, device=self.dev, dtype=torch.float32)
+            m0 = (C.c_void_p(fm_ptr + 4 * self.lm.off("masker.0.weight")), self.mbuf["m0pack"])
         hg.critic_forward(self.fc, self.lc, self.ab, 2 * n, drop.shifted(0), out=self._cview(0, 2 * n),
-                          pw=None if self.separate else pw)
+                          pw=None if self.separate else pw, m0=m0)
         sa = self._cview(n, 2 * n)
         if self.separate:
             pws = (pw[0], pw[1], self.mbuf["o4"])
@@ -194,7 +199,7 @@
         else:
             embeds = [sa[f"e{i}"] for i in range(5)]
         hg.masker_forward(self.fm, self.lm, A, embeds, n, out=self.mbuf, o4_done=True,
-                          zpart=self.zsum if hg.ENC0_MIX_FUSED else None)
+                          zpart=self.zsum if hg.ENC0_MIX_FUSED else None, m0pack_done=m0 is not None)
         if hg.ENC0_MIX_FUSED:
             mixsrc = hg.MixInput(A, B, self.mbuf["Z"])
             hg.critic_forward(self.fc, self.lc, mixsrc, nmix, drop.shifted(2 * n), out=self._cview(2 * n, 2 * n + nmix))
diff --git a/critic-guided-segmentation-of-rewarding-objects-in-first-person-views_amd/hourglass.py b/critic-guided-segmentation-of-rewarding-objects-in-first-person-views_amd/hourglass.py
--- a/critic-guided-segmentation-of-rewarding-objects-in-first-person-views_amd/hourglass.py
+++ b/critic-guided-segmentation-of-rewarding-objects-in-first-person-views_amd/hourglass.py
@@ -23,10 +23,19 @@
 DEC_TAIL_DEC0_FUSED = True
 ENC1_TAIL_BWD_FUSED = os.environ.get("CGS_ENC1_TAIL_BWD_FUSED", "1") != "0"
 ENC1_TAIL_BWD_FUSED_MIN_N = int(os.environ.get("CGS_ENC1_TAIL_BWD_FUSED_MIN_N", "224"))
+DEC_MASK_FWD_FUSED = os.environ.get("CGS_DEC_MASK_FWD_FUSED", "1") != "0"
 
 
 def mask_train_fused(n: int) -> bool:
     return MASK_TRAIN_FUSED and n >= MASK_TRAIN_FUSED_MIN_N
+
+
+def critic_fwd_whole(mixin: bool, u8: bool) -> bool:
+    return TAIL_FWD and ENC1_TAIL_FUSED and CRITIC_FWD_FUSED and (mixin or u8)
+
+
+def dec_mask_fwd_fused(n: int, u8: bool) -> bool:
+    return DEC_MASK_FWD_FUSED and TAIL_FWD and DEC_TAIL_DEC0_FUSED and mask_train_fused(n) and u8
 
 
 def enc1_tail_bwd_fused(n: int) -> bool:
@@ -182,7 +191,7 @@
 
 
 def critic_forward(flat: torch.Tensor, lay: Layout, x: torch.Tensor, n: int, drop: DropState = NO_DROP,
-                   out: Optional[Dict[str, torch.Tensor]] = None, pw=None) -> Dict[str, torch.Tensor]:
+                   out: Optional[Dict[str, torch.Tensor]] = None, pw=None, m0=None) -> Dict[str, torch.Tensor]:
     mixin = isinstance(x, MixInput)
     u8 = (not mixin) and x.dtype == torch.uint8
     if not mixin:
@@ -191,7 +200,9 @@
     dev = x.device
     o = out if out is not None else {}
     src = x
-    whole = TAIL_FWD and ENC1_TAIL_FUSED and CRITIC_FWD_FUSED and (mixin or u8)
+    whole = critic_fwd_whole(mixin, u8)
+    if m0 is not None and (mixin or not whole):
+        raise _lib.CgsError("critic_forward: m0 (the mask head's packed weights) rides only in the one-launch form on uint8 frames")
     for i, (key, hw, ca, cb, co, ups, act, pool, site) in enumerate(ENC_LAYERS):
         e = o.get(f"e{i}")
         if e is None:
@@ -218,10 +229,14 @@
         if whole:
             k0, k3 = ENC_LAYERS[0][0], ENC_LAYERS[1][0]
             wp_ = lambda k: C.c_void_p(flat.data_ptr() + 4 * lay.off(k))
-            _lib.call("cgs_critic_fwd_fused", n, C.byref(tw), x.ptr() if mixin else _p(x), int(mixin), wp_(k0 + ".weight"), wp_(k0 + ".bias"),
-                      _p(o["e0"]), _p(o["am0"]), wp_(k3 + ".weight"), wp_(k3 + ".bias"), _p(o["e1"]), _p(o["am1"]), _p(o["e2"]), _p(o["am2"]),
-                      _p(o["e3"]), _p(o["am3"]), _p(o["e4"]), _p(o["h1"]), _p(o["pred"]), _p(pw[2]) if pw else None,
-                      drop.desc(DROP_SITE_E2, True, 128), drop.desc(DROP_SITE_E3, True, 64), drop.desc(DROP_SITE_H1, True, 8), _stream())
+            args = (n, C.byref(tw), x.ptr() if mixin else _p(x), int(mixin), wp_(k0 + ".weight"), wp_(k0 + ".bias"),
+                    _p(o["e0"]), _p(o["am0"]), wp_(k3 + ".weight"), wp_(k3 + ".bias"), _p(o["e1"]), _p(o["am1"]), _p(o["e2"]), _p(o["am2"]),
+                    _p(o["e3"]), _p(o["am3"]), _p(o["e4"]), _p(o["h1"]), _p(o["pred"]), _p(pw[2]) if pw else None,
+                    drop.desc(DROP_SITE_E2, True, 128), drop.desc(DROP_SITE_E3, True, 64), drop.desc(DROP_SITE_H1, True, 8))
+            if m0 is not None:
+                _lib.call("cgs_critic_fwd_fused_pack", *args, m0[0], _p(m0[1]), _stream())
+            else:
+                _lib.call("cgs_critic_fwd_fused", *args, _stream())
             return o
         if ENC1_TAIL_FUSED:
             k3 = ENC_LAYERS[1][0]
@@ -471,7 +486,7 @@
 def masker_forward(flat: torch.Tensor, lay: Layout, x: torch.Tensor, embeds: List[torch.Tensor], n: int,
                    out: Optional[Dict[str, torch.Tensor]] = None, o4_done: bool = False,
                    keep_hm: bool = True, fp16_mask_head: bool = False,
-                   zpart: Optional[torch.Tensor] = None) -> Dict[str, torch.Tensor]:
+                   zpart: Optional[torch.Tensor] = None, m0pack_done: bool = False) -> Dict[str, torch.Tensor]:
     u8 = x.dtype == torch.uint8
     _chk(x, torch.uint8 if u8 else torch.float32, "masker image input")
     _chk_img(x, n, "masker image input")
@@ -500,6 +515,20 @@
             m0pack = o.get("m0pack")
             if m0pack is None:
                 m0pack = o["m0pack"] = torch.empty(40 * 64, device=dev, dtype=torch.float32)
+        if m0pack_done and keep_hm and zpart is not None and dec_mask_fwd_fused(n, u8):
+            assert o.get("m0pack") is not None, "m0pack_done: the caller's critic launch already built out['m0pack']"
+            for k, shp in (("o0", (n, 32, 32, 8)), ("hm", (n, 64, 64, 16)), ("Z", (n, 64, 64))):
+                if o.get(k) is None:
+                    o[k] = torch.empty(shp, device=dev, dtype=torch.float32)
+            wp_ = lambda k: C.c_void_p(fp + 4 * lay.off(k))
+            rc = _lib.load().cgs_dec_mask_fwd(n, C.byref(tw), _p(embeds[0]), _p(embeds[1]), _p(embeds[2]), _p(embeds[3]), _p(o["o4"]),
+                                              _p(o["o3"]), _p(o["o2"]), _p(o["o1"]), wp_("dec_model.0.weight"), wp_("dec_model.0.bias"), _p(o["o0"]),
+                                              _lib.SRC_U8, _p(x), wp_("masker.0.bias"), wp_("masker.2.weight"), wp_("masker.2.bias"),
+                                              _p(o["hm"]), _p(o["Z"]), _p(zpart), _p(o["m0pack"]), _stream())
+            if rc == 0:
+                return o
+            if rc != _lib.ERR_UNSUPPORTED:
+                _lib.check(rc, "cgs_dec_mask_fwd")
         dec0_done = False
         if DEC_TAIL_DEC0_FUSED:
             if o.get("o0") is None:
diff --git a/include/cgs_hip.h b/include/cgs_hip.h
--- a/include/cgs_hip.h
+++ b/include/cgs_hip.h
@@ -135,6 +135,10 @@
                          float* e0, uint32_t* am0, const float* w3, const float* b3, float* e1, uint32_t* am1, float* e2, uint32_t* am2,
                          float* e3, uint32_t* am3, float* e4, float* h1, float* pred, float* o4, cgs_dropout drop_e2, cgs_dropout drop_e3,
                          cgs_dropout drop_h1, cgs_stream_t stream);
+int cgs_critic_fwd_fused_pack(int32_t n, const cgs_tail_enc_weights* w, const void* x, int32_t x_is_mix, const float* w0, const float* b0,
+                              float* e0, uint32_t* am0, const float* w3, const float* b3, float* e1, uint32_t* am1, float* e2, uint32_t* am2,
+                              float* e3, uint32_t* am3, float* e4, float* h1, float* pred, float* o4, cgs_dropout drop_e2, cgs_dropout drop_e3,
+                              cgs_dropout drop_h1, const float* w_m0, float* m0_pack, cgs_stream_t stream);
 int cgs_tail_dec_fwd(int32_t n, const cgs_tail_dec_weights* w, const float* e1, const float* e2, const float* e3,
                      const float* o4, float* o3, float* o2, float* o1, cgs_stream_t stream);
 int cgs_tail_enc_fwd_h16(int32_t n, const cgs_tail_enc_weights* w, const float* e1, float* e2, uint32_t* am2, float* e3,
@@ -206,6 +210,10 @@
 int cgs_tail_dec_fwd_dec0(int32_t n, const cgs_tail_dec_weights* w, const float* e0, const float* e1, const float* e2, const float* e3,
                           const float* o4, float* o3, float* o2, float* o1, const float* w0_hwio, const float* b0, float* o0,
                           const float* w_m0, float* m0_pack, cgs_stream_t stream);
+int cgs_dec_mask_fwd(int32_t n, const cgs_tail_dec_weights* w, const float* e0, const float* e1, const float* e2, const float* e3,
+                     const float* o4, float* o3, float* o2, float* o1, const float* w0_hwio, const float* b0, float* o0, int32_t src_a,
+                     const void* x, const float* b_m0, const float* w_m2, const float* b_m2, float* h, float* z, float* zpart,
+                     const float* m0_pack, cgs_stream_t stream);
 
 int cgs_conv3x3_bwd_weight_slabs(const cgs_conv_desc* d);
 int cgs_conv3x3_bwd_weight(const cgs_conv_desc* d, const void* src_a, const float* src_b,
```

Measured after the change: 1.016 million, median of 6. 1.01x the previous value.
